# OpenVVC/OpenVVC

Hardware: AMD Instinct MI355X
Metric: decoded frames/sec, full rcn back-end decode step (H2D of the recorded picture + MC incl. BDOF/DMVR/affine-PROF/GPM/CIIP + LMCS + inverse transform + ordered intra pass + deblocking + SAO + ALF/CC-ALF + D2H of refined MVs + wait + per-picture digest + publication to the device DPB), 4K 10-bit RA rec (higher is better)
Workload: dtype u16 samples / int16 coefficients / int32 accumulate

## Files before the change

### include/ovvc_hip.h

```cpp
#ifndef OVVC_HIP_H
#define OVVC_HIP_H

#include <stddef.h>
#include <stdint.h>

#ifdef __cplusplus
extern "C" {
#endif

#define OVHIP_ABI_VERSION 9

#define OVHIP_OK        0
#define OVHIP_ENODEV   (-1)
#define OVHIP_ENOMEM   (-2)
#define OVHIP_EINVAL   (-3)
#define OVHIP_ELAUNCH  (-4)
#define OVHIP_EUNSUP   (-5)
#define OVHIP_EREF     (-6)

enum { OVHIP_DST_VII = 0, OVHIP_DCT_VIII = 1, OVHIP_DCT_II = 2 };

typedef struct ovhip_pic {
    uint16_t *y, *cb, *cr;
    int32_t   w, h;
// ... 814 lines not shown
int  ovhip_dpb_post_rows(ovhip_dpb *d, const void *key, int32_t rows, void *event, const volatile uint32_t *abort_word);
int  ovhip_dpb_rows_tag(ovhip_dpb *d, const void *key, uint64_t tag, int dev, int32_t need_rows, int block, int pin, ovhip_pic *pic, void **event);
int  ovhip_dpb_wait_copy(ovhip_dpb *d, int dev, void *event);
int  ovhip_dpb_unpin(ovhip_dpb *d, const void *key);
int  ovhip_dpb_release(ovhip_dpb *d, const void *key);
int  ovhip_dpb_lookup(ovhip_dpb *d, const void *key, int *home_dev, ovhip_pic *pic);
void ovhip_dpb_shutdown(ovhip_dpb *d);
int  ovhip_dpb_get_stats(ovhip_dpb *d, ovhip_dpb_stats *out);

typedef struct ovhip_frame ovhip_frame;

enum { OVHIP_OUT_NONE = 0,
       OVHIP_OUT_DIGEST = 1,
       OVHIP_OUT_PLANES = 2,
       OVHIP_OUT_PACKED = 3 };
typedef struct ovhip_frame_output {
    int32_t  mode;
    ovhip_window window;
    uint16_t *y, *cb, *cr; int32_t stride_y, stride_c;
    void    *packed;
    uint8_t  digest[16];
} ovhip_frame_output;

enum { OVHIP_FE_BEGIN = 1, OVHIP_FE_REF, OVHIP_FE_DMVR_ROWS, OVHIP_FE_DMVR_BEGIN, OVHIP_FE_DMVR_COLLECT, OVHIP_FE_SUBMIT, OVHIP_FE_FAIL,
       OVHIP_FE_BAND  };
typedef struct ovhip_frame_event {
    uint32_t op; int32_t frame;
    uint64_t key, tag;
    int64_t  a, b, result;
} ovhip_frame_event;
void ovhip_frame_set_trace(void (*sink)(void *user, const ovhip_frame_event *ev), void *user);

int  ovhip_frame_create(ovhip_dpb *dpb, int dev, int32_t w, int32_t h, ovhip_frame **out);
void ovhip_frame_destroy(ovhip_frame *f);
ovhip_ctx      *ovhip_frame_ctx(ovhip_frame *f);
ovhip_job      *ovhip_frame_job(ovhip_frame *f);
ovhip_recorder *ovhip_frame_recorder(ovhip_frame *f);
int  ovhip_frame_begin(ovhip_frame *f, const void *key);
int  ovhip_frame_ref(ovhip_frame *f, const void *ref_key);
int  ovhip_frame_begin_tag(ovhip_frame *f, const void *key, uint64_t tag);
int  ovhip_frame_ref_tag(ovhip_frame *f, const void *ref_key, uint64_t tag);
int  ovhip_frame_ref_at(ovhip_frame *f, int slot, const void *ref_key);
int64_t ovhip_frame_dmvr_rows(ovhip_frame *f);
int  ovhip_frame_refs_ready(ovhip_frame *f);
int64_t ovhip_frame_dmvr_rows_begin(ovhip_frame *f, int32_t log2_ctu_s);
int64_t ovhip_frame_dmvr_rows_begin_upto(ovhip_frame *f, int32_t log2_ctu_s, size_t upto_units);
int64_t ovhip_frame_dmvr_rows_collect(ovhip_frame *f);
int  ovhip_frame_submit(ovhip_frame *f, ovhip_job *job, const ovhip_pic *intra, const ovhip_job_params *params, ovhip_frame_output *out);
int  ovhip_frame_set_band_mode(ovhip_frame *f, int on);
int  ovhip_frame_band(ovhip_frame *f, const ovhip_job_params *params, int32_t row_end, int32_t last, ovhip_frame_output *out);
int  ovhip_frame_band_upto(ovhip_frame *f, const ovhip_job_params *params, int32_t row_end, const ovhip_band_counts *upto, int32_t block);
int  ovhip_frame_band_stats(const ovhip_frame *f, int32_t *n_bands, int32_t *n_deferred);
int  ovhip_frame_set_output_scale(ovhip_frame *f, int32_t out_w, int32_t out_h, const ovhip_scale_info *info);
int  ovhip_frame_set_film_grain(ovhip_frame *f, const ovhip_fg_params *params, int32_t poc);
int  ovhip_frame_set_picture_hash(ovhip_frame *f, int method, int n_planes, const ovhip_pic_hash_value *expected);
int  ovhip_frame_picture_hash(const ovhip_frame *f, ovhip_pic_hash_value *computed);
int  ovhip_frame_set_rgb_output(ovhip_frame *f, const ovhip_rgb_format *fmt, const ovhip_window *win, void *d_dst, size_t dst_bytes);
int  ovhip_frame_set_surface_output(ovhip_frame *f, const ovhip_surface_format *fmt, const ovhip_window *win, void *d_dst, size_t dst_bytes);
int  ovhip_frame_set_mvfield_output(ovhip_frame *f, const ovhip_mvfield_format *fmt, void *d_vec, size_t vec_bytes, void *d_info, size_t info_bytes);
int  ovhip_frame_fail(ovhip_frame *f, int status);
const char *ovhip_frame_last_error(const ovhip_frame *f);

typedef struct ovhip_calllog ovhip_calllog;
ovhip_calllog *ovhip_calllog_create(void);
void   ovhip_calllog_destroy(ovhip_calllog *log);
void   ovhip_calllog_reset(ovhip_calllog *log);
const void *ovhip_calllog_data(const ovhip_calllog *log, size_t *bytes);
void   ovhip_rec_set_calllog(ovhip_recorder *rec, ovhip_calllog *log);
int64_t ovhip_calllog_replay(const void *data, size_t bytes, ovhip_recorder *rec);

#define OVHIP_STREAM_MAX_REFS 8
typedef struct ovhip_stream_content {
    const void *calllog; size_t calllog_bytes;
    ovhip_job_params params;
    uint32_t n_ref_slots;
} ovhip_stream_content;

typedef struct ovhip_stream_pic {
    uint32_t content;
    uint32_t job;
    int32_t  poc;
    uint16_t device;
    uint16_t n_refs;
    uint32_t refs[OVHIP_STREAM_MAX_REFS];
    int32_t  owner;
    uint32_t send_mask;
} ovhip_stream_pic;

typedef struct ovhip_stream_xfer {
    void *user;
    int (*send)(void *user, uint32_t idx, const ovhip_pic *pic, int dst_rank);
    int (*recv)(void *user, uint32_t idx, const ovhip_pic *pic, int src_rank);
} ovhip_stream_xfer;

typedef struct ovhip_rccl ovhip_rccl;
int  ovhip_rccl_unique_id(uint8_t out[128]);
int  ovhip_rccl_create(ovhip_rccl **out, const uint8_t unique_id[128], int rank, int world, int hip_device);
void ovhip_rccl_destroy(ovhip_rccl *r);
const ovhip_stream_xfer *ovhip_rccl_xfer(ovhip_rccl *r);
const char *ovhip_rccl_last_error(const ovhip_rccl *r);
int  ovhip_rccl_stats(const ovhip_rccl *r, uint64_t out[4]);
int  ovhip_rccl_self_exchange(ovhip_rccl *r, const ovhip_pic *src, const ovhip_pic *dst);

enum { OVHIP_STREAM_RECORD = 1,
       OVHIP_STREAM_DIGESTS = 2,
       OVHIP_STREAM_RESIDENT = 4,
       OVHIP_STREAM_KEEP = 8,
       OVHIP_STREAM_HOLD_ALL = 32,
       OVHIP_STREAM_FILE_MD5 = 16 };

typedef struct ovhip_stream_cfg {
    int32_t w, h;
    uint32_t flags;
    int32_t threads_per_device;
    int32_t output;
    ovhip_window window;
    uint32_t extra_stages;
    int32_t rank;
    const ovhip_stream_xfer *xfer;
    int32_t intra_lookahead;
    int32_t ahead_own_queue;
} ovhip_stream_cfg;

typedef struct ovhip_stream_result {
    double   seconds;
    uint64_t n_decoded, n_second_passes, n_received, n_sent;
    uint64_t out_frames, out_bytes;
    uint8_t  out_md5[16];
    double   record_seconds;
    double   host_seconds[5];
    int32_t  status;
    char     error[192];
    double  *trace;
} ovhip_stream_result;

typedef struct ovhip_stream ovhip_stream;
int  ovhip_stream_create(ovhip_stream **out, ovhip_dpb *dpb, const ovhip_stream_cfg *cfg, const ovhip_stream_content *contents,
                         uint32_t n_contents, ovhip_job *const *jobs, uint32_t n_jobs);
void ovhip_stream_destroy(ovhip_stream *s);
int  ovhip_stream_run(ovhip_stream *s, const ovhip_stream_pic *pics, uint32_t n_total, uint32_t first, uint32_t n, uint32_t flags,
                      uint8_t *digests, ovhip_stream_result *res);
ovhip_frame *ovhip_stream_frame(ovhip_stream *s, int dev, int thread);
int  ovhip_stream_queue_info(const ovhip_stream *s, int *moved, int *sharing);
int  ovhip_stream_set_output_scale(ovhip_stream *s, int32_t out_w, int32_t out_h, const ovhip_scale_info *info);
int  ovhip_stream_set_film_grain(ovhip_stream *s, const ovhip_fg_params *params);
int  ovhip_stream_set_picture_hashes(ovhip_stream *s, int method, int n_planes, const ovhip_pic_hash_value *expected);
int  ovhip_stream_picture_hashes(const ovhip_stream *s, ovhip_pic_hash_value *computed, uint32_t *n_mismatch, int32_t *first_mismatch);
int  ovhip_stream_set_rgb_output(ovhip_stream *s, const ovhip_rgb_format *fmt, const ovhip_window *win, void *d_base, size_t bytes_per_picture, uint32_t n_slots);
int  ovhip_stream_set_surface_output(ovhip_stream *s, const ovhip_surface_format *fmt, const ovhip_window *win, void *d_base, size_t bytes_per_picture, uint32_t n_slots);
int  ovhip_stream_set_mvfield_output(ovhip_stream *s, const ovhip_mvfield_format *fmt, void *d_vec_base, size_t vec_bytes_per_picture,
                                     void *d_info_base, size_t info_bytes_per_picture, uint32_t n_slots);
const void *ovhip_stream_key(const ovhip_stream *s, uint32_t idx);
int  ovhip_job_test_abort_next_flow(ovhip_job *job);

#ifdef __cplusplus
}
#endif
#endif
```

### openvvc_amd/capi.py

```python
from __future__ import annotations

import ctypes as C
import os
from pathlib import Path

import numpy as np

_PKG = Path(__file__).resolve().parent
LIB_PATH = _PKG / os.environ.get("OVVC_HIP_LIB_NAME", "libovvc_hip.so")

OVHIP_ABI_VERSION = 9
OVHIP_OK, OVHIP_ENODEV, OVHIP_ENOMEM, OVHIP_EINVAL, OVHIP_ELAUNCH, OVHIP_EUNSUP, OVHIP_EREF = 0, -1, -2, -3, -4, -5, -6
DST_VII, DCT_VIII, DCT_II = 0, 1, 2
TB_TR, TB_DC, TB_TS, TB_TS_RAW = 0, 1, 2, 3
TB_FLAG_RASTER = 0x80
RES_ADD, RES_SUB, RES_ADD_HALF, RES_SUB_HALF, RES_SCALE = 0, 1, 2, 3, 4
MC_HPEL_FILT, MC_FILT_4x4, MC_NO_LUMA, MC_NO_CHROMA, MC_LMCS, MC_BDOF, MC_DMVR = 1, 2, 4, 8, 16, 32, 64
PU_BDOF, PU_DMVR, PU_GPM = 1, 2, 4
MC_GPM = 128


class Pic(C.Structure):
    _fields_ = [("y", C.c_void_p), ("cb", C.c_void_p), ("cr", C.c_void_p),
                ("w", C.c_int32), ("h", C.c_int32), ("stride_y", C.c_int32), ("stride_c", C.c_int32)]
# ... 489 lines not shown
    p = Path(path) if path else LIB_PATH
    if not p.exists():
        raise RuntimeError(f"{p} not built: run `python -c 'import __graft_entry__ as g; g.build()'` "
                           "(the HIP engine has no CPU fallback)")
    try:
        import torch
    except Exception:
        pass
    lib = C.CDLL(str(p))
    vp, u32, i32 = C.c_void_p, C.c_uint32, C.c_int32
    P = C.POINTER
    sigs = {
        "ovhip_abi_version": (C.c_int, []),
        "ovhip_rec_create": (vp, [i32, i32]),
        "ovhip_rec_destroy": (None, [vp]),
        "ovhip_rec_reset": (None, [vp]),
        "ovhip_rec_tu": (C.c_int, [vp, P(TuState), P(TuDesc)]),
        "ovhip_rec_pu": (C.c_int, [vp, P(PuDesc)]),
        "ovhip_rec_set_ref_scale": (C.c_int, [vp, i32, P(RefScale)]),
        "ovhip_rec_refusal": (C.c_char_p, [vp]),
        "ovhip_rec_rpr_units": (vp, [vp, P(C.c_size_t)]),
        "ovhip_mc_rpr_launch": (C.c_int, [vp, P(Pic), P(Pic), u32, vp, u32, vp, P(Pic)]),
        "ovhip_rec_set_rpr_tools": (C.c_int, [vp, u32]),
        "ovhip_rec_aff_rpr_units": (vp, [vp, P(C.c_size_t)]),
        "ovhip_mca_rpr_launch": (C.c_int, [vp, P(Pic), P(Pic), u32, vp, u32, vp, vp]),
        "ovhip_rec_dbf_ctu": (C.c_int, [vp, vp]),
        "ovhip_rec_dbf_row": (C.c_int, [vp, vp, C.c_size_t]),
        "ovhip_rec_dbf_mv_prepass_view": (C.c_int, [vp, vp, vp, vp]),
        "ovhip_rec_cu_inter": (C.c_int, [vp, vp, vp]),
        "ovhip_rec_dbf_planes": (C.c_int, [vp, P(DbfPlanes)]),
        "ovhip_dbf_launch": (C.c_int, [vp, P(Pic), P(DbfPlanes)]),
        "ovhip_sao_launch": (C.c_int, [vp, P(Pic), P(Pic), vp, i32]),
        "ovhip_alf_launch": (C.c_int, [vp, P(Pic), P(Pic), P(AlfPic)]),
        "ovhip_rec_tb_cmds": (vp, [vp, P(C.c_size_t)]),
        "ovhip_rec_coefs": (vp, [vp, P(C.c_size_t)]),
        "ovhip_rec_mc_units": (vp, [vp, P(C.c_size_t)]),
        "ovhip_rec_mcx_units": (vp, [vp, P(C.c_size_t)]),
        "ovhip_rec_affine_cu": (C.c_int, [vp, P(AffineDesc)]),
        "ovhip_rec_transform_tree": (C.c_int, [vp, P(TuState), P(TtDesc)]),
        "ovhip_rec_lmcs_region": (C.c_int, [vp, C.c_int32, C.c_int32, u32, u32]),
        "ovhip_dbf_compact": (C.c_int64, [P(DbfPlanes), C.c_int, vp, C.c_size_t]),
        "ovhip_rec_dbf_mv_prepass": (C.c_int, [vp, P(DbfMvCtx)]),
        "ovhip_dbf_launch_edges": (C.c_int, [vp, P(Pic), vp, u32, vp, u32, C.c_int32, C.c_int32]),
        "ovhip_rec_ciip": (C.c_int, [vp, C.c_int32, C.c_int32, C.c_int32, C.c_int32, C.c_int32, C.c_int32]),
        "ovhip_rec_ciip_units": (vp, [vp, P(C.c_size_t)]),
        "ovhip_ciip_launch": (C.c_int, [vp, P(Pic), P(Pic), vp, u32]),
        "ovhip_rec_lmcs_regions": (vp, [vp, P(C.c_size_t)]),
        "ovhip_rec_tb_cmds_split": (vp, [vp, C.c_size_t * 4, P(C.c_size_t)]),
        "ovhip_itx_launch_classes": (C.c_int, [vp, P(Pic), vp, u32, u32, vp, vp]),
        "ovhip_itx_launch_chroma_lmcs": (C.c_int, [vp, P(Pic), vp, u32, u32, vp, vp, vp]),
        "ovhip_lmcs_build": (C.c_int, [P(LmcsData), P(LmcsLuts)]),
        "ovhip_lmcs_scale_launch": (C.c_int, [vp, P(Pic), vp, u32, P(LmcsLuts), vp]),
        "ovhip_lmcs_inverse_launch": (C.c_int, [vp, P(Pic), vp]),
        "ovhip_rec_aff_units": (vp, [vp, P(C.c_size_t)]),
        "ovhip_rec_aff_side": (vp, [vp, P(C.c_size_t)]),
        "ovhip_ctx_create": (C.c_int, [P(vp), C.c_int, vp]),
        "ovhip_ctx_destroy": (None, [vp]),
        "ovhip_ctx_sync": (C.c_int, [vp]),
        "ovhip_ctx_shares_queue": (C.c_int, [vp, vp]),
        "ovhip_ctx_new_stream": (C.c_int, [vp]),
        "ovhip_ctx_fork": (C.c_int, [vp, C.c_int]),
        "ovhip_ctx_join": (C.c_int, [vp]),
        "ovhip_last_error": (C.c_char_p, [vp]),
        "ovhip_ctx_stream": (vp, [vp]),
        "ovhip_malloc": (C.c_int, [vp, C.c_size_t, P(vp)]),
        "ovhip_free": (C.c_int, [vp, vp]),
        "ovhip_h2d": (C.c_int, [vp, vp, vp, C.c_size_t]),
        "ovhip_d2h": (C.c_int, [vp, vp, vp, C.c_size_t]),
        "ovhip_pic_alloc": (C.c_int, [vp, i32, i32, P(Pic)]),
        "ovhip_pic_free": (C.c_int, [vp, P(Pic)]),
        "ovhip_pic_upload": (C.c_int, [vp, P(Pic), vp, vp, vp, i32, i32]),
        "ovhip_pic_download": (C.c_int, [vp, P(Pic), vp, vp, vp, i32, i32]),
        "ovhip_itx_launch": (C.c_int, [vp, P(Pic), vp, u32, vp, vp]),
        "ovhip_mc_launch": (C.c_int, [vp, P(Pic), P(Pic), u32, vp, u32, vp, P(Pic)]),
        "ovhip_ciip_weight": (C.c_int, [C.c_int32, C.c_int32]),
        "ovhip_mcx_launch": (C.c_int, [vp, P(Pic), P(Pic), u32, vp, u32, vp, vp]),
        "ovhip_mca_launch": (C.c_int, [vp, P(Pic), P(Pic), u32, vp, u32, vp, vp]),
        "ovhip_mcxa_launch": (C.c_int, [vp, P(Pic), P(Pic), u32, vp, u32, vp, vp, u32, vp, vp]),
        "ovhip_rec_create_ex": (vp, [i32, i32, vp]),
        "ovhip_rec_set_dense_dbf_planes": (None, [vp, C.c_int]),
        "ovhip_rec_dbf_edges": (vp, [vp, C.c_int, P(C.c_size_t), P(DbfOffsets)]),
        "ovhip_dbf_launch_edges_ex": (C.c_int, [vp, P(Pic), vp, u32, vp, u32, P(DbfOffsets)]),
        "ovhip_dmvr_search_launch": (C.c_int, [vp, P(Pic), P(Pic), u32, vp, u32, vp]),
        "ovhip_rec_append_raw": (C.c_int, [vp, C.c_int, vp, C.c_size_t]),
        "ovhip_itx_launch_classes_res": (C.c_int, [vp, P(Pic), P(Pic), vp, u32, u32, vp, vp]),
        "ovhip_intra_level_launch": (C.c_int, [vp, P(Pic), P(Pic), vp, u32, vp, vp, vp, i32, u32]),
        "ovhip_intra_level_geom": (u32, [vp, C.c_size_t]),
        "ovhip_intra_sync_words": (C.c_size_t, [i32, i32, i32]),
        "ovhip_intra_flow_words": (C.c_size_t, [i32, i32]),
        "ovhip_intra_flow_items": (C.c_size_t, [vp, C.c_size_t, vp, C.c_size_t]),
        "ovhip_intra_flow_launch": (C.c_int, [vp, P(Pic), P(Pic), vp, u32, vp, u32, vp, vp, vp, i32, vp, u32, vp, i32, i32]),
        "ovhip_intra_ctu_launch": (C.c_int, [vp, P(Pic), P(Pic), vp, vp, u32, vp, vp, vp, i32, vp, u32, vp]),
        "ovhip_rec_itask_levels": (u32, [vp]),
        "ovhip_rec_isp_cu": (C.c_int, [vp, vp, vp]),
        "ovhip_isp_geometry": (None, [i32, i32, i32, P(i32), P(i32), P(i32), P(i32)]),
        "ovhip_job_bind": (C.c_int, [vp, vp]),
        "ovhip_rec_set_ctu_size": (C.c_int, [vp, i32]),
        "ovhip_rec_itasks_by_ctu": (vp, [vp, i32, P(C.c_size_t), P(vp), P(C.c_size_t)]),
        "ovhip_rec_tu_intra": (C.c_int, [vp, P(TuState), P(TuDesc), P(ITask), P(ITask)]),
        "ovhip_rec_itasks": (vp, [vp, P(C.c_size_t)]),
        "ovhip_rec_ibc_check": (C.c_int, [vp, P(IbcDesc)]),
        "ovhip_rec_tu_ibc": (C.c_int, [vp, P(TuState), P(TuDesc), P(IbcDesc)]),
        "ovhip_rec_ibc_tasks": (C.c_size_t, [vp]),
        "ovhip_rec_itasks_sorted": (vp, [vp, P(C.c_size_t), P(P(C.c_uint32)), P(C.c_uint32)]),
        "ovhip_rec_set_dbf_offsets": (C.c_int, [vp, P(DbfOffsets), C.c_int]),
        "ovhip_job_create": (C.c_int, [vp, i32, i32, P(vp)]),
        "ovhip_job_destroy": (None, [vp]),
        "ovhip_job_recorder": (vp, [vp]),
        "ovhip_job_begin": (C.c_int, [vp]),
        "ovhip_job_flush": (C.c_int, [vp, P(Pic), P(Pic), u32, P(Pic), P(JobParams)]),
        "ovhip_frame_band": (C.c_int, [vp, P(JobParams), i32, i32, P(FrameOutput)]),
        "ovhip_frame_set_band_mode": (C.c_int, [vp, C.c_int]),
        "ovhip_frame_band_upto": (C.c_int, [vp, P(JobParams), i32, P(BandCounts), i32]),
        "ovhip_frame_dmvr_rows_begin_upto": (C.c_int64, [vp, i32, C.c_size_t]),
        "ovhip_job_dmvr_rows_begin_upto": (C.c_int64, [vp, P(Pic), u32, i32, C.c_size_t]),
        "ovhip_frame_band_stats": (C.c_int, [vp, P(i32), P(i32)]),
        "ovhip_dpb_post_rows": (C.c_int, [vp, vp, i32, vp, vp]),
        "ovhip_dpb_rows_tag": (C.c_int, [vp, vp, C.c_uint64, C.c_int, i32, C.c_int, C.c_int, P(Pic), P(vp)]),
        "ovhip_job_band": (C.c_int, [vp, P(Pic), P(Pic), u32, P(JobParams), P(BandCounts), i32, i32]),
        "ovhip_job_band_active": (C.c_int, [vp]),
        "ovhip_job_band_busy": (C.c_int, [vp]),
        "ovhip_job_band_progress": (C.c_int, [vp, P(i32), P(vp), P(vp)]),
        "ovhip_rec_counts": (None, [vp, P(BandCounts)]),
        "ovhip_sao_launch_rows": (C.c_int, [vp, P(Pic), P(Pic), vp, i32, i32, i32]),
        "ovhip_alf_launch_rows": (C.c_int, [vp, P(Pic), P(Pic), P(AlfPic), i32, i32]),
        "ovhip_job_wait": (C.c_int, [vp]),
        "ovhip_job_refined_mvs": (vp, [vp, P(C.c_size_t)]),
        "ovhip_job_dmvr_rows": (C.c_int64, [vp, P(Pic), u32]),
        "ovhip_job_dmvr_rows_begin": (C.c_int64, [vp, P(Pic), u32, i32]),
        "ovhip_job_dmvr_rows_collect": (C.c_int64, [vp]),
        "ovhip_job_last_stats": (C.c_int, [vp, P(JobStats)]),
        "ovhip_job_time_stage": (C.c_int, [vp, C.c_int]),
        "ovhip_job_stage_time": (C.c_int, [vp, P(C.c_double), P(C.c_uint64)]),
        "ovhip_lmcs_scale_prepare_launch": (C.c_int, [vp, P(Pic), vp, u32, vp, vp, vp, u32, vp, u32]),
        "ovhip_lmcs_inverse_untag_launch": (C.c_int, [vp, P(Pic), vp, vp, u32]),
        "ovhip_intra_flow_untag_launch": (C.c_int, [vp, P(Pic), vp, u32, i32]),
        "ovhip_tmvp_cells_launch": (C.c_int, [vp, vp, u32, vp, i32, i32, vp]),
        "ovhip_job_tmvp_cells": (vp, [vp, P(C.c_size_t)]),
        "ovhip_output_bytes": (C.c_size_t, [i32, i32, P(Window)]),
        "ovhip_output_rows": (C.c_size_t, [i32, i32, P(Window)]),
        "ovhip_output_pack_launch": (C.c_int, [vp, P(Pic), P(Window), vp]),
        "ovhip_output_row_md5_launch": (C.c_int, [vp, P(Pic), P(Window), vp]),
        "ovhip_output_bands": (C.c_size_t, [i32, i32, P(Window)]),
        "ovhip_output_tree_md5_launch": (C.c_int, [vp, P(Pic), P(Window), vp]),
        "ovhip_pic_output": (C.c_int, [vp, P(Pic), P(Window), vp]),
        "ovhip_pic_digest": (C.c_int, [vp, P(Pic), P(Window), vp]),
        "ovhip_md5_init": (None, [P(Md5State)]),
        "ovhip_md5_update": (None, [P(Md5State), vp, C.c_size_t]),
        "ovhip_md5_final": (None, [P(Md5State), vp]),
        "ovhip_d2d": (C.c_int, [vp, vp, vp, C.c_size_t]),
        "ovhip_host_alloc": (vp, [C.c_size_t]),
        "ovhip_host_free": (None, [vp]),
        "ovhip_job_test_abort_next_flow": (C.c_int, [vp]),
        "ovhip_dpb_create": (C.c_int, [P(vp), P(C.c_int), C.c_int]),
        "ovhip_dpb_create_ex": (C.c_int, [P(vp), C.c_int, P(DpbOps)]),
        "ovhip_dpb_destroy": (None, [vp]),
        "ovhip_dpb_n_devices": (C.c_int, [vp]),
        "ovhip_dpb_device": (C.c_int, [vp, C.c_int]),
        "ovhip_dpb_begin": (C.c_int, [vp, vp, C.c_int, i32, i32, P(Pic)]),
        "ovhip_dpb_want": (C.c_int, [vp, vp, C.c_int]),
        "ovhip_dpb_begin_tag": (C.c_int, [vp, vp, C.c_uint64, C.c_int, i32, i32, P(Pic)]),
        "ovhip_dpb_want_tag": (C.c_int, [vp, vp, C.c_uint64, C.c_int]),
        "ovhip_dpb_acquire_tag": (C.c_int, [vp, vp, C.c_uint64, C.c_int, P(Pic), P(vp)]),
        "ovhip_dpb_publish": (C.c_int, [vp, vp, C.c_int]),
        "ovhip_dpb_acquire": (C.c_int, [vp, vp, C.c_int, P(Pic), P(vp)]),
        "ovhip_dpb_wait_copy": (C.c_int, [vp, C.c_int, vp]),
        "ovhip_dpb_poll_tag": (C.c_int, [vp, vp, C.c_uint64]),
        "ovhip_frame_refs_ready": (C.c_int, [vp]),
        "ovhip_dpb_set_unknown_key_timeout": (None, [vp, C.c_int]),
        "ovhip_dpb_unpin": (C.c_int, [vp, vp]),
        "ovhip_dpb_release": (C.c_int, [vp, vp]),
        "ovhip_dpb_lookup": (C.c_int, [vp, vp, P(C.c_int), P(Pic)]),
        "ovhip_dpb_shutdown": (None, [vp]),
        "ovhip_dpb_get_stats": (C.c_int, [vp, P(DpbStats)]),
        "ovhip_frame_create": (C.c_int, [vp, C.c_int, i32, i32, P(vp)]),
        "ovhip_frame_destroy": (None, [vp]),
        "ovhip_frame_ctx": (vp, [vp]),
        "ovhip_frame_job": (vp, [vp]),
        "ovhip_frame_recorder": (vp, [vp]),
        "ovhip_frame_begin": (C.c_int, [vp, vp]),
        "ovhip_frame_ref": (C.c_int, [vp, vp]),
        "ovhip_frame_set_trace": (None, [vp, vp]),
        "ovhip_rccl_unique_id": (C.c_int, [vp]),
        "ovhip_rccl_create": (C.c_int, [P(vp), vp, C.c_int, C.c_int, C.c_int]),
        "ovhip_rccl_destroy": (None, [vp]),
        "ovhip_rccl_xfer": (vp, [vp]),
        "ovhip_rccl_last_error": (C.c_char_p, [vp]),
        "ovhip_rccl_stats": (C.c_int, [vp, P(C.c_uint64)]),
        "ovhip_rccl_self_exchange": (C.c_int, [vp, P(Pic), P(Pic)]),
        "ovhip_frame_begin_tag": (C.c_int, [vp, vp, C.c_uint64]),
        "ovhip_frame_ref_tag": (C.c_int, [vp, vp, C.c_uint64]),
        "ovhip_frame_ref_at": (C.c_int, [vp, C.c_int, vp]),
        "ovhip_frame_dmvr_rows": (C.c_int64, [vp]),
        "ovhip_frame_dmvr_rows_begin": (C.c_int64, [vp, i32]),
        "ovhip_frame_dmvr_rows_collect": (C.c_int64, [vp]),
        "ovhip_frame_submit": (C.c_int, [vp, vp, P(Pic), P(JobParams), P(FrameOutput)]),
        "ovhip_frame_fail": (C.c_int, [vp, C.c_int]),
        "ovhip_frame_last_error": (C.c_char_p, [vp]),
        "ovhip_calllog_create": (vp, []),
        "ovhip_calllog_destroy": (None, [vp]),
        "ovhip_calllog_reset": (None, [vp]),
        "ovhip_calllog_data": (vp, [vp, P(C.c_size_t)]),
        "ovhip_rec_set_calllog": (None, [vp, vp]),
        "ovhip_calllog_replay": (C.c_int64, [vp, C.c_size_t, vp]),
        "ovhip_stream_create": (C.c_int, [P(vp), vp, P(StreamCfg), P(StreamContent), u32, P(vp), u32]),
        "ovhip_stream_destroy": (None, [vp]),
        "ovhip_stream_run": (C.c_int, [vp, P(StreamPic), u32, u32, u32, u32, vp, P(StreamResult)]),
        "ovhip_stream_frame": (vp, [vp, C.c_int, C.c_int]),
        "ovhip_stream_queue_info": (C.c_int, [vp, P(C.c_int), P(C.c_int)]),
        "ovhip_stream_key": (vp, [vp, u32]),
        "ovhip_output_scale_check": (C.c_int, [i32, i32, P(ScaleInfo), i32, i32, P(i32 * 4)]),
        "ovhip_output_scale_launch": (C.c_int, [vp, P(Pic), P(ScaleInfo), P(Pic)]),
        "ovhip_pic_output_scaled": (C.c_int, [vp, P(Pic), P(ScaleInfo), i32, i32, P(Window), vp]),
        "ovhip_pic_digest_scaled": (C.c_int, [vp, P(Pic), P(ScaleInfo), i32, i32, P(Window), vp]),
        "ovhip_ctx_scratch_bytes": (C.c_size_t, [vp]),
        "ovhip_frame_set_output_scale": (C.c_int, [vp, i32, i32, P(ScaleInfo)]),
        "ovhip_stream_set_output_scale": (C.c_int, [vp, i32, i32, P(ScaleInfo)]),
        "ovhip_frame_set_film_grain": (C.c_int, [vp, P(FgParams), i32]),
        "ovhip_stream_set_film_grain": (C.c_int, [vp, P(FgParams)]),
        "ovhip_fg_derive": (C.c_int, [P(FgParams), P(FgModel), P(FgParams)]),
        "ovhip_fg_database": (vp, []),
        "ovhip_fg_seed": (u32, [i32, i32, C.c_int]),
        "ovhip_fg_prng": (u32, [u32]),
        "ovhip_fg_stripe_seeds": (None, [u32, i32, i32, P(u32)]),
        "ovhip_film_grain_launch": (C.c_int, [vp, P(Pic), P(FgModel), i32, i32, P(Pic)]),
        "ovhip_pic_output_grain": (C.c_int, [vp, P(Pic), P(FgModel), i32, P(Window), vp]),
        "ovhip_pic_digest_grain": (C.c_int, [vp, P(Pic), P(FgModel), i32, P(Window), vp]),
        "ovhip_pic_hash_host": (C.c_int, [C.c_int, C.c_int, vp, vp, vp, i32, i32, i32, i32, P(PicHashValue)]),
        "ovhip_pic_hash_parse_sei": (C.c_int, [vp, C.c_size_t, P(PicHashValue)]),
        "ovhip_pic_hash_equal": (C.c_int, [P(PicHashValue), P(PicHashValue)]),
        "ovhip_pic_hash_launch": (C.c_int, [vp, P(Pic), C.c_int, C.c_int, vp]),
        "ovhip_pic_hash": (C.c_int, [vp, P(Pic), C.c_int, C.c_int, P(PicHashValue)]),
        "ovhip_frame_set_picture_hash": (C.c_int, [vp, C.c_int, C.c_int, P(PicHashValue)]),
        "ovhip_frame_picture_hash": (C.c_int, [vp, P(PicHashValue)]),
        "ovhip_stream_set_picture_hashes": (C.c_int, [vp, C.c_int, C.c_int, P(PicHashValue)]),
        "ovhip_stream_picture_hashes": (C.c_int, [vp, P(PicHashValue), P(u32), P(i32)]),
        "ovhip_rgb_bytes": (C.c_size_t, [i32, i32, P(Window), P(RgbFormat)]),
        "ovhip_rgb_coefs": (C.c_int, [P(RgbFormat), P(i32), P(i32)]),
        "ovhip_rgb_host": (C.c_int, [vp, vp, vp, i32, i32, i32, i32, P(Window), P(RgbFormat), vp, C.c_size_t]),
        "ovhip_rgb_launch": (C.c_int, [vp, P(Pic), P(Window), P(RgbFormat), vp, C.c_size_t]),
        "ovhip_pic_output_rgb": (C.c_int, [vp, P(Pic), P(Window), P(RgbFormat), vp, C.c_size_t]),
        "ovhip_frame_set_rgb_output": (C.c_int, [vp, P(RgbFormat), P(Window), vp, C.c_size_t]),
        "ovhip_stream_set_rgb_output": (C.c_int, [vp, P(RgbFormat), P(Window), vp, C.c_size_t, u32]),
        "ovhip_surface_bytes": (C.c_size_t, [i32, i32, P(Window), P(SurfaceFormat)]),
        "ovhip_surface_host": (C.c_int, [vp, vp, vp, i32, i32, i32, i32, P(Window), P(SurfaceFormat), vp, C.c_size_t]),
        "ovhip_surface_launch": (C.c_int, [vp, P(Pic), P(Window), P(SurfaceFormat), vp, C.c_size_t]),
        "ovhip_pic_output_surface": (C.c_int, [vp, P(Pic), P(Window), P(SurfaceFormat), vp, C.c_size_t]),
        "ovhip_frame_set_surface_output": (C.c_int, [vp, P(SurfaceFormat), P(Window), vp, C.c_size_t]),
        "ovhip_stream_set_surface_output": (C.c_int, [vp, P(SurfaceFormat), P(Window), vp, C.c_size_t, u32]),
        "ovhip_mvfield_bytes": (C.c_size_t, [i32, i32, P(MvfieldFormat), P(C.c_size_t)]),
        "ovhip_mvfield_host": (C.c_int, [i32, i32, P(MvfieldSrc), P(MvfieldFormat), vp, C.c_size_t, vp, C.c_size_t]),
        "ovhip_mvfield_launch": (C.c_int, [vp, i32, i32, P(MvfieldSrc), P(MvfieldFormat), vp, C.c_size_t, vp, C.c_size_t]),
        "ovhip_job_mvfield": (C.c_int, [vp, P(MvfieldFormat), vp, C.c_size_t, vp, C.c_size_t]),
        "ovhip_frame_set_mvfield_output": (C.c_int, [vp, P(MvfieldFormat), vp, C.c_size_t, vp, C.c_size_t]),
        "ovhip_stream_set_mvfield_output": (C.c_int, [vp, P(MvfieldFormat), vp, C.c_size_t, vp, C.c_size_t, u32]),
    }
    ab_build = "OVVC_HIP_LIB_NAME" in os.environ
    for name, (res, args) in sigs.items():
        if ab_build and not hasattr(lib, name):
            continue
        fn = getattr(lib, name)
        fn.restype, fn.argtypes = res, args
    if lib.ovhip_abi_version() != OVHIP_ABI_VERSION and not ab_build:
        raise RuntimeError("libovvc_hip.so ABI version mismatch")
    if path is None:
        _lib = lib
    return lib


EXPORTED_SYMBOLS = [
    "ovhip_abi_version", "ovhip_rec_create", "ovhip_rec_destroy", "ovhip_rec_reset", "ovhip_rec_tu",
    "ovhip_rec_pu", "ovhip_rec_cu_inter", "ovhip_rec_dbf_row", "ovhip_rec_dbf_mv_prepass_view", "ovhip_rec_dbf_ctu", "ovhip_rec_dbf_planes", "ovhip_dbf_launch", "ovhip_sao_launch", "ovhip_alf_launch", "ovhip_rec_tb_cmds", "ovhip_rec_coefs", "ovhip_rec_mc_units", "ovhip_rec_mcx_units", "ovhip_mcx_launch", "ovhip_rec_affine_cu", "ovhip_rec_transform_tree", "ovhip_rec_lmcs_region", "ovhip_dbf_compact", "ovhip_rec_dbf_mv_prepass", "ovhip_dbf_launch_edges", "ovhip_rec_ciip", "ovhip_ciip_weight", "ovhip_rec_ciip_units", "ovhip_ciip_launch", "ovhip_rec_lmcs_regions", "ovhip_rec_tb_cmds_split", "ovhip_itx_launch_classes", "ovhip_itx_launch_chroma_lmcs", "ovhip_lmcs_build", "ovhip_lmcs_scale_launch", "ovhip_lmcs_inverse_launch", "ovhip_rec_aff_units", "ovhip_rec_aff_side", "ovhip_mca_launch", "ovhip_mcxa_launch", "ovhip_ctx_create",
    "ovhip_ctx_destroy", "ovhip_ctx_sync", "ovhip_ctx_shares_queue", "ovhip_ctx_new_stream", "ovhip_ctx_fork", "ovhip_ctx_join", "ovhip_last_error", "ovhip_ctx_stream", "ovhip_malloc",
    "ovhip_free", "ovhip_h2d", "ovhip_d2h", "ovhip_pic_alloc", "ovhip_pic_free", "ovhip_pic_upload",
    "ovhip_pic_download", "ovhip_itx_launch", "ovhip_mc_launch",
    "ovhip_rec_set_ref_scale", "ovhip_rec_refusal", "ovhip_rec_rpr_units", "ovhip_mc_rpr_launch",
    "ovhip_rec_set_rpr_tools", "ovhip_rec_aff_rpr_units", "ovhip_mca_rpr_launch",
    "ovhip_rec_create_ex", "ovhip_rec_set_dense_dbf_planes", "ovhip_rec_dbf_edges", "ovhip_dbf_launch_edges_ex",
    "ovhip_dmvr_search_launch", "ovhip_rec_append_raw", "ovhip_rec_set_dbf_offsets", "ovhip_rec_tu_intra", "ovhip_rec_itasks", "ovhip_rec_itasks_sorted", "ovhip_itx_launch_classes_res", "ovhip_intra_level_launch", "ovhip_intra_level_geom", "ovhip_intra_sync_words", "ovhip_intra_ctu_launch", "ovhip_intra_flow_words", "ovhip_intra_flow_items", "ovhip_intra_flow_launch",
    "ovhip_rec_itask_levels", "ovhip_rec_isp_cu", "ovhip_isp_geometry", "ovhip_rec_itasks_by_ctu", "ovhip_rec_set_ctu_size", "ovhip_job_bind", "ovhip_job_create", "ovhip_job_destroy", "ovhip_job_recorder", "ovhip_job_begin",
    "ovhip_frame_band", "ovhip_frame_band_upto", "ovhip_frame_dmvr_rows_begin_upto", "ovhip_job_dmvr_rows_begin_upto", "ovhip_frame_set_band_mode", "ovhip_frame_band_stats", "ovhip_dpb_post_rows", "ovhip_dpb_rows_tag",
    "ovhip_job_band", "ovhip_job_band_active", "ovhip_job_band_busy", "ovhip_job_band_reserve", "ovhip_job_reserve_for_picture", "ovhip_rec_reserve_for_picture", "ovhip_job_band_progress", "ovhip_rec_counts", "ovhip_sao_launch_rows", "ovhip_alf_launch_rows",
    "ovhip_job_flush", "ovhip_job_wait", "ovhip_job_refined_mvs", "ovhip_job_dmvr_rows", "ovhip_job_dmvr_rows_begin", "ovhip_job_dmvr_rows_collect", "ovhip_job_last_stats", "ovhip_job_time_stage", "ovhip_job_stage_time",
    "ovhip_output_bytes", "ovhip_output_rows", "ovhip_output_pack_launch", "ovhip_output_row_md5_launch", "ovhip_output_bands", "ovhip_output_tree_md5_launch", "ovhip_pic_output", "ovhip_pic_digest",
    "ovhip_md5_init", "ovhip_md5_update", "ovhip_md5_final", "ovhip_tmvp_cells_launch", "ovhip_job_tmvp_cells", "ovhip_intra_flow_untag_launch", "ovhip_lmcs_inverse_untag_launch", "ovhip_lmcs_scale_prepare_launch",
    "ovhip_host_alloc", "ovhip_host_free", "ovhip_d2d", "ovhip_job_test_abort_next_flow",
    "ovhip_dpb_create", "ovhip_dpb_create_ex", "ovhip_dpb_destroy", "ovhip_dpb_n_devices", "ovhip_dpb_device", "ovhip_dpb_begin", "ovhip_dpb_want",
    "ovhip_dpb_publish", "ovhip_dpb_acquire", "ovhip_dpb_wait_copy", "ovhip_dpb_poll_tag", "ovhip_frame_refs_ready", "ovhip_dpb_set_unknown_key_timeout", "ovhip_dpb_unpin", "ovhip_dpb_release", "ovhip_dpb_lookup", "ovhip_dpb_shutdown",
    "ovhip_dpb_get_stats", "ovhip_dpb_begin_tag", "ovhip_dpb_want_tag", "ovhip_dpb_acquire_tag", "ovhip_frame_begin_tag", "ovhip_frame_ref_tag", "ovhip_frame_set_trace",
    "ovhip_rccl_unique_id", "ovhip_rccl_create", "ovhip_rccl_destroy", "ovhip_rccl_xfer", "ovhip_rccl_last_error", "ovhip_rccl_stats", "ovhip_rccl_self_exchange",
    "ovhip_frame_create", "ovhip_frame_destroy", "ovhip_frame_ctx", "ovhip_frame_job", "ovhip_frame_recorder", "ovhip_frame_begin", "ovhip_frame_ref",
    "ovhip_frame_ref_at", "ovhip_frame_dmvr_rows", "ovhip_frame_dmvr_rows_begin", "ovhip_frame_dmvr_rows_collect", "ovhip_frame_submit", "ovhip_frame_fail", "ovhip_frame_last_error",
    "ovhip_calllog_create", "ovhip_calllog_destroy", "ovhip_calllog_reset", "ovhip_calllog_data", "ovhip_rec_set_calllog", "ovhip_calllog_replay",
    "ovhip_stream_create", "ovhip_stream_destroy", "ovhip_stream_run", "ovhip_stream_frame", "ovhip_stream_key", "ovhip_stream_queue_info",
    "ovhip_output_scale_check", "ovhip_output_scale_launch", "ovhip_pic_output_scaled", "ovhip_pic_digest_scaled",
    "ovhip_frame_set_output_scale", "ovhip_stream_set_output_scale", "ovhip_ctx_scratch_bytes",
    "ovhip_rec_ibc_check", "ovhip_rec_tu_ibc", "ovhip_rec_ibc_tasks",
    "ovhip_frame_set_film_grain", "ovhip_stream_set_film_grain", "ovhip_fg_derive", "ovhip_fg_database", "ovhip_fg_seed", "ovhip_fg_prng", "ovhip_fg_stripe_seeds", "ovhip_film_grain_launch", "ovhip_pic_output_grain", "ovhip_pic_digest_grain",
    "ovhip_pic_hash_host", "ovhip_pic_hash_parse_sei", "ovhip_pic_hash_equal", "ovhip_pic_hash_launch", "ovhip_pic_hash",
    "ovhip_frame_set_picture_hash", "ovhip_frame_picture_hash", "ovhip_stream_set_picture_hashes", "ovhip_stream_picture_hashes",
    "ovhip_rgb_bytes", "ovhip_rgb_coefs", "ovhip_rgb_host", "ovhip_rgb_launch", "ovhip_pic_output_rgb", "ovhip_frame_set_rgb_output", "ovhip_stream_set_rgb_output",
    "ovhip_surface_bytes", "ovhip_surface_host", "ovhip_surface_launch", "ovhip_pic_output_surface", "ovhip_frame_set_surface_output", "ovhip_stream_set_surface_output",
    "ovhip_mvfield_bytes", "ovhip_mvfield_host", "ovhip_mvfield_launch", "ovhip_job_mvfield", "ovhip_frame_set_mvfield_output", "ovhip_stream_set_mvfield_output",
]


def rpr_units(lib, rec) -> list:
    n = C.c_size_t(0)
    ptr = lib.ovhip_rec_rpr_units(rec, C.byref(n))
    if not ptr or not n.value:
        return []
    raw = C.string_at(ptr, n.value * C.sizeof(RprUnit))
    return [RprUnit.from_buffer_copy(raw, i * C.sizeof(RprUnit)) for i in range(n.value)]


def aff_rpr_units(lib, rec) -> list:
    n = C.c_size_t(0)
    ptr = lib.ovhip_rec_aff_rpr_units(rec, C.byref(n))
    if not ptr or not n.value:
        return []
    raw = C.string_at(ptr, n.value * C.sizeof(AffRprUnit))
    return [AffRprUnit.from_buffer_copy(raw, i * C.sizeof(AffRprUnit)) for i in range(n.value)]


def set_ref_scale(lib, rec, slot: int, scale_hor: int | None = None, scale_ver: int | None = None, ref_w: int = 0, ref_h: int = 0,
                  col_hor: int = 0, col_ver: int = 0) -> int:
    if scale_hor is None:
        return lib.ovhip_rec_set_ref_scale(rec, slot, None)
    sc = RefScale(scale_hor, scale_ver if scale_ver is not None else scale_hor, ref_w, ref_h, col_hor, col_ver)
    return lib.ovhip_rec_set_ref_scale(rec, slot, C.byref(sc))


class Recorder:

    def __init__(self, pic_w: int, pic_h: int):
        self.lib = load()
        self.h = self.lib.ovhip_rec_create(pic_w, pic_h)
        if not self.h:
            raise MemoryError("ovhip_rec_create")
        self._keep = []

    def close(self):
        if self.h:
            self.lib.ovhip_rec_destroy(self.h)
            self.h = None

    def __del__(self):
        try:
            self.close()
        except Exception:
            pass

    def reset(self):
        self.lib.ovhip_rec_reset(self.h)

    def start_calllog(self):
        self._log = self.lib.ovhip_calllog_create()
        self.lib.ovhip_rec_set_calllog(self.h, self._log)

    def take_calllog(self) -> np.ndarray:
        n = C.c_size_t()
        p = self.lib.ovhip_calllog_data(self._log, C.byref(n))
        if not p and n.value:
            raise MemoryError("call log")
        out = np.frombuffer((C.c_char * n.value).from_address(p), dtype=np.uint8).copy() if n.value else np.zeros(0, np.uint8)
        self.lib.ovhip_rec_set_calllog(self.h, None)
        self.lib.ovhip_calllog_destroy(self._log)
        self._log = None
        return out

    def replay(self, log: np.ndarray) -> int:
        n = self.lib.ovhip_calllog_replay(log.ctypes.data, log.nbytes, self.h)
        if n < 0:
            raise ValueError(f"ovhip_calllog_replay -> {n}")
        return int(n)

    def tu(self, st: TuState, d: TuDesc) -> int:
        r = self.lib.ovhip_rec_tu(self.h, C.byref(st), C.byref(d))
        if r < 0:
            raise ValueError(f"ovhip_rec_tu -> {r}")
        return r

    def tu_intra(self, st: TuState, d: TuDesc, task_l: "ITask | None", task_c: "ITask | None") -> int:
        r = self.lib.ovhip_rec_tu_intra(self.h, C.byref(st), C.byref(d), C.byref(task_l) if task_l is not None else None,
                                        C.byref(task_c) if task_c is not None else None)
        if r < 0:
            raise ValueError(f"ovhip_rec_tu_intra -> {r}")
        return r

    def ibc_check(self, cu: IbcDesc) -> int:
        return self.lib.ovhip_rec_ibc_check(self.h, C.byref(cu))

    def tu_ibc(self, st: TuState, d: TuDesc, cu: IbcDesc) -> int:
        return self.lib.ovhip_rec_tu_ibc(self.h, C.byref(st), C.byref(d), C.byref(cu))

    def ibc_tasks(self) -> int:
        return int(self.lib.ovhip_rec_ibc_tasks(self.h))

    def refusal(self) -> str:
        return (self.lib.ovhip_rec_refusal(self.h) or b"").decode()

    def itasks(self) -> np.ndarray:
        return self._arr(self.lib.ovhip_rec_itasks, ITASK_DTYPE)

    def itasks_sorted(self):
        n, nl, ls = C.c_size_t(), C.c_uint32(), C.POINTER(C.c_uint32)()
        p = self.lib.ovhip_rec_itasks_sorted(self.h, C.byref(n), C.byref(ls), C.byref(nl))
        if not n.value:
            return np.zeros(0, ITASK_DTYPE), np.zeros(1, np.uint32)
        t = np.frombuffer((C.c_char * (n.value * 32)).from_address(p), dtype=ITASK_DTYPE).copy()
        return t, np.array([ls[i] for i in range(nl.value + 1)], np.uint32)

    def itasks_by_ctu(self, log2_ctu: int = 7):
        n, nc, cp = C.c_size_t(), C.c_size_t(), C.c_void_p()
        p = self.lib.ovhip_rec_itasks_by_ctu(self.h, log2_ctu, C.byref(n), C.byref(cp), C.byref(nc))
        if not n.value:
            return np.zeros(0, ITASK_DTYPE), np.zeros(0, ICTU_DTYPE)
        t = np.frombuffer((C.c_char * (n.value * 32)).from_address(p), dtype=ITASK_DTYPE).copy()
        c = np.frombuffer((C.c_char * (nc.value * 16)).from_address(cp.value), dtype=ICTU_DTYPE).copy()
        return t, c

    def transform_tree(self, st: "TuState", d: TtDesc, infos: bytes, res_cb: np.ndarray, res_cr: np.ndarray, res_y: np.ndarray) -> int:
        ib = (C.c_char * len(infos)).from_buffer_copy(infos)
        keep = [np.ascontiguousarray(a, dtype=np.int16) for a in (res_cb, res_cr, res_y)]
        d.tu_info = C.addressof(ib)
        for k in range(3):
            d.residual[k] = keep[k].ctypes.data
        r = self.lib.ovhip_rec_transform_tree(self.h, C.byref(st), C.byref(d))
        d.tu_info = None
        if r < 0:
            raise ValueError(f"ovhip_rec_transform_tree -> {r}")
        return r

    def isp_cu(self, st: TuState, d: IspDesc) -> int:
        r = self.lib.ovhip_rec_isp_cu(self.h, C.byref(st), C.byref(d))
        if r < 0:
            raise ValueError(f"ovhip_rec_isp_cu -> {r}")
        return r

# ... 126 lines not shown
```

### openvvc_amd/csrc/kernels_itx.hip

```cpp
#include "ovvc_common.hip.h"
#include <stdlib.h>
#define OVT_ATTR __device__
#include "vvc_tables.h"

#ifndef OV_WPE_ITX
#define OV_WPE_ITX 8
#endif
#if OV_WPE_ITX > 0
#define OV_OCC_ITX __attribute__((amdgpu_waves_per_eu(OV_WPE_ITX)))
#else
#define OV_OCC_ITX
#endif

namespace {

constexpr int core_ks(int log2n)   { const int n = 1 << log2n, K = n < 32 ? n : 32; return K < 8 ? 8 : K; }
constexpr int core_size(int log2n) { return (1 << log2n) * core_ks(log2n); }
constexpr int core_off(int type, int log2n)
{
    int off = 0;
    for (int t = 0; t < 3; ++t)
        for (int l = (t == 2 ? 1 : 2); l <= (t == 2 ? 6 : 5); ++l) {
            if (t == type && l == log2n) return off;
            off += core_size(l);
        }
    return off;
}
constexpr int CORE_TOTAL = core_off(3, 0);
struct CoreT16 { int16_t v[CORE_TOTAL]; };
constexpr CoreT16 build_cores()
{
    CoreT16 t{};
    const int8_t *const tabs[3][7] = {
        { nullptr, nullptr, ovt_dst7_4, ovt_dst7_8, ovt_dst7_16, ovt_dst7_32, nullptr },
        { nullptr, nullptr, ovt_dct8_4, ovt_dct8_8, ovt_dct8_16, ovt_dct8_32, nullptr },
        { nullptr, ovt_dct2_2, ovt_dct2_4, ovt_dct2_8, ovt_dct2_16, ovt_dct2_32, ovt_dct2_64 } };
    for (int ty = 0; ty < 3; ++ty)
        for (int l = 1; l <= 6; ++l) {
            if (!tabs[ty][l]) continue;
            const int n = 1 << l, K = n < 32 ? n : 32, KS = core_ks(l), off = core_off(ty, l);
            for (int j = 0; j < n; ++j)
                for (int k = 0; k < K; ++k) t.v[off + j * KS + k] = tabs[ty][l][k * n + j];
        }
    return t;
}
__device__ const CoreT16 __attribute__((aligned(16))) g_cores = build_cores();

constexpr uint64_t core_lut(int type)
{
    uint64_t v = 0;
    for (int l = (type == 2 ? 1 : 2); l <= (type == 2 ? 6 : 5); ++l)
        v |= (uint64_t)((core_off(type, l) - core_off(type, type == 2 ? 1 : 2)) / 16) << (8 * l);
    return v;
}
static_assert(core_lut(0) == core_lut(1) && (core_off(2, 6) - core_off(2, 1)) / 16 < 256 && core_off(1, 2) % 16 == 0 && core_off(2, 1) % 16 == 0,
              "core offsets must fit the byte table");
__device__ __forceinline__ const int16_t *tr_core(int type, int log2n)
{
    const uint64_t lut = type == 2 ? core_lut(2) : core_lut(0);
    const int base = type == 2 ? core_off(2, 1) : type == 1 ? core_off(1, 2) : 0;
    return g_cores.v + base + 16 * (int)((lut >> (8 * log2n)) & 0xff);
}
__device__ __forceinline__ int tile_stride(int K) { return K < 8 ? 8 : K + (K >= 16 ? 4 : 0); }
constexpr int tile_stride_c(int K) { return K < 8 ? 8 : K + (K >= 16 ? 4 : 0); }

__device__ __forceinline__ int dequant1(int c, int scale, int shift, int neg)
{
    if (neg) return ov_clip3((int)((uint32_t)c * (uint32_t)(scale << shift)), -32767, 32767);
    return ov_clip3(((int)((uint32_t)c * (uint32_t)scale) + ((1 << shift) >> 1)) >> shift, -32767, 32767);
}

__device__ __forceinline__ int nb_rows_of(uint64_t map)
{
    uint32_t m = (uint32_t)map | (uint32_t)(map >> 32);
    m |= m >> 16; m |= m >> 8;
    m = (m & 0xff) | 1;
    return (32 - __clz((int)m)) << 2;
}
__device__ __forceinline__ int nb_cols_of(uint64_t map)
{
    return (8 - (__clzll((long long)(map | 1)) >> 3)) << 2;
}

__device__ __forceinline__ int residual1(int pix, int r, int mode, int scale)
{
    const int neg = -(mode & 1);
    int v = ((r ^ neg) - neg) >> ((mode >> 1) & 1);
    if (mode & OVHIP_RES_STORE) return ov_clip16(v) & 0xffff;
    if (mode & OVHIP_RES_SCALE) {
        int sign = v & (1 << 15);
        int a = ov_clip_bd(abs(v));
        a = (a * scale + (1 << 10)) >> 11;
        v = ov_clip3(sign ? -a : a, -(1 << 15), 1 << 15);
    }
    return ov_clip_bd(pix + v);
}

struct ResDelta { long long d[3]; };

struct ResidualSink {
    uint16_t *dst; int stride; int mode;
    uint16_t *dst2; int stride2; int mode2;
    int scale;
};
typedef short short2v __attribute__((ext_vector_type(2)));

template <bool FINAL, int NT, int NK4>
__device__ __forceinline__ void tr_pass_lds_n(const int16_t *src, int sstride, const int16_t *core, int cstride, int log2n,
                                               int kmax, int lines, int shift, int16_t *dst, int dstride, int lane,
                                               const ResidualSink &sink)
{
    const int n = 1 << log2n;
    const int ntask = lines << log2n;
    const int rnd = 1 << (shift - 1);
    const int nk4 = (kmax + 3) >> 2;
    for (int t = lane; t < ntask; t += NT) {
        const int j = t & (n - 1), i = t >> log2n;
        int old = 0, old2 = 0;
        if (FINAL) {
            old = sink.dst[i * sink.stride + j];
            if (sink.dst2) old2 = sink.dst2[i * sink.stride2 + j];
        }
        const int2 *sp = reinterpret_cast<const int2 *>(src + i * sstride);
        const int2 *cp = reinterpret_cast<const int2 *>(core + j * cstride);
        int acc = 0;
        if (NK4 > 0) {
            int2 a[NK4 > 0 ? NK4 : 1], m[NK4 > 0 ? NK4 : 1];
#pragma unroll
            for (int k4 = 0; k4 < NK4; ++k4) { a[k4] = sp[k4]; m[k4] = cp[k4]; }
#pragma unroll
            for (int k4 = 0; k4 < NK4; ++k4) {
                acc = __builtin_amdgcn_sdot2(__builtin_bit_cast(short2v, a[k4].x), __builtin_bit_cast(short2v, m[k4].x), acc, false);
                acc = __builtin_amdgcn_sdot2(__builtin_bit_cast(short2v, a[k4].y), __builtin_bit_cast(short2v, m[k4].y), acc, false);
            }
        } else
        for (int k4 = 0; k4 < nk4; ++k4) {
            const int2 a = sp[k4], m = cp[k4];
            acc = __builtin_amdgcn_sdot2(__builtin_bit_cast(short2v, a.x), __builtin_bit_cast(short2v, m.x), acc, false);
            acc = __builtin_amdgcn_sdot2(__builtin_bit_cast(short2v, a.y), __builtin_bit_cast(short2v, m.y), acc, false);
        }
        const int r = ov_clip16((acc + rnd) >> shift);
        if (!FINAL) {
            dst[j * dstride + i] = (int16_t)r;
        } else {
            sink.dst[i * sink.stride + j] = (uint16_t)residual1(old, r, sink.mode, sink.scale);
            if (sink.dst2) sink.dst2[i * sink.stride2 + j] = (uint16_t)residual1(old2, r, sink.mode2, sink.scale);
        }
    }
}

template <bool FINAL, int NT>
__device__ __forceinline__ void tr_pass_lds(const int16_t *src, int sstride, const int16_t *core, int cstride, int log2n,
                                             int kmax, int lines, int shift, int16_t *dst, int dstride, int lane,
                                             const ResidualSink &sink)
{
    const int nk4 = (kmax + 3) >> 2;
    if (nk4 == 1)      tr_pass_lds_n<FINAL, NT, 1>(src, sstride, core, cstride, log2n, kmax, lines, shift, dst, dstride, lane, sink);
    else if (nk4 == 2) tr_pass_lds_n<FINAL, NT, 2>(src, sstride, core, cstride, log2n, kmax, lines, shift, dst, dstride, lane, sink);
    else if (nk4 == 4) tr_pass_lds_n<FINAL, NT, 4>(src, sstride, core, cstride, log2n, kmax, lines, shift, dst, dstride, lane, sink);
    else               tr_pass_lds_n<FINAL, NT, 0>(src, sstride, core, cstride, log2n, kmax, lines, shift, dst, dstride, lane, sink);
}

template <int NT>
__device__ __forceinline__ void lmcs_inverse_rows(const ovhip_pic &pic, const uint16_t *__restrict__ lut, uint32_t e, uint32_t n_extra,
                                                  uint16_t *s_lut)
{
    for (int i = threadIdx.x; i < 512; i += NT) reinterpret_cast<uint32_t *>(s_lut)[i] = reinterpret_cast<const uint32_t *>(lut)[i];
    __syncthreads();
    const int nvx = pic.w >> 3, tail = pic.w & 7;
    for (int y = (int)e; y < pic.h; y += (int)n_extra) {
        uint16_t *row = pic.y + (size_t)y * pic.stride_y;
        for (int v = threadIdx.x; v < nvx; v += NT) {
            uint4 q = *reinterpret_cast<uint4 *>(row + 8 * v);
            uint32_t *d = reinterpret_cast<uint32_t *>(&q);
#pragma unroll
            for (int k = 0; k < 4; ++k) d[k] = s_lut[d[k] & 1023] | ((uint32_t)s_lut[(d[k] >> 16) & 1023] << 16);
            *reinterpret_cast<uint4 *>(row + 8 * v) = q;
        }
        if ((int)threadIdx.x < tail) row[8 * nvx + threadIdx.x] = s_lut[row[8 * nvx + threadIdx.x] & 1023];
    }
}

#define ITX_LDS_BIG   8064
#define ITX_LDS_SLICE 2048

__device__ __forceinline__ ResidualSink make_sink(const ovhip_pic &pic, const ResDelta &rd, const ovhip_tb_cmd &c, const int16_t *__restrict__ lmcs_scales)
{
    ResidualSink sink;
    sink.dst = ov_plane(pic, c.plane, sink.stride) + c.y * sink.stride + c.x;
    sink.mode = c.res_mode;
    sink.dst2 = nullptr; sink.stride2 = 0; sink.mode2 = c.res_mode2;
    if (c.plane2 != 0xff) sink.dst2 = ov_plane(pic, c.plane2, sink.stride2) + c.y * sink.stride2 + c.x;
    if (c.res_mode & OVHIP_RES_STORE) {
        const long long d1 = c.plane == 0 ? rd.d[0] : (c.plane == 1 ? rd.d[1] : rd.d[2]);
        sink.dst = reinterpret_cast<uint16_t *>(reinterpret_cast<char *>(sink.dst) + d1);
        if (sink.dst2) {
            const long long d2 = c.plane2 == 0 ? rd.d[0] : (c.plane2 == 1 ? rd.d[1] : rd.d[2]);
            sink.dst2 = reinterpret_cast<uint16_t *>(reinterpret_cast<char *>(sink.dst2) + d2);
        }
    }
    sink.scale = (c.res_mode & OVHIP_RES_SCALE_IDX) ? lmcs_scales[c.c_scale] : c.c_scale;
    return sink;
}

template <int NT>
__device__ __forceinline__ void block_sync()
{
    if (NT == 64) {
        __builtin_amdgcn_fence(__ATOMIC_RELEASE, "wavefront");
        __builtin_amdgcn_wave_barrier();
        __builtin_amdgcn_fence(__ATOMIC_ACQUIRE, "wavefront");
    } else __syncthreads();
}

template <int NT, int LW = -1, int LH = -1, bool PLAIN = false>
__device__ __forceinline__ void itx_block(const ovhip_pic &pic, const ResDelta &rd, const ovhip_tb_cmd &c, bool valid, const int16_t *__restrict__ arena,
                                          const int16_t *__restrict__ lmcs_scales, int ablate, int lane, int16_t *lds)
{
    const int log2_w = LW >= 0 ? LW : c.log2_w, log2_h = LH >= 0 ? LH : c.log2_h;
    const int tb_w = 1 << log2_w, tb_h = 1 << log2_h;
    const int kind = PLAIN ? (int)OVHIP_TB_TR : (c.kind & 0x3f);
    const bool raster = PLAIN ? false : (bool)(c.kind & OVHIP_TB_FLAG_RASTER), bdpcm = PLAIN ? false : (bool)(c.kind & OVHIP_TB_FLAG_BDPCM);
    if (PLAIN) ablate = 0;
    const int cw = min(tb_w, 32), ch = min(tb_h, 32);
    const int16_t *src = arena + c.coef_off;

    if (NT == 64 && kind == OVHIP_TB_DC && !ablate) {
        if (!valid) return;
        const bool have = raster || (c.sig_sb_map & 1);
        const int lvl = have ? (int)src[0] : 0;
        const int c0 = (!have || bdpcm) ? lvl : dequant1(lvl, c.dq_scale, c.dq_shift, c.dq_neg);
        const int flat_val = ov_clip16(((((int)(int16_t)c0 + 1) >> 1) + (1 << (14 - OV_BD - 1))) >> (14 - OV_BD));
        const ResidualSink sink = make_sink(pic, rd, c, lmcs_scales);
        for (int i0 = lane; i0 < tb_w * tb_h; i0 += 4 * NT) {
            int old[4], old2[4];
#pragma unroll
            for (int q = 0; q < 4; ++q) {
                const int i = i0 + NT * q;
                if (i < tb_w * tb_h) {
                    const int x = i & (tb_w - 1), y = i >> log2_w;
                    old[q] = sink.dst[y * sink.stride + x];
                    old2[q] = sink.dst2 ? (int)sink.dst2[y * sink.stride2 + x] : 0;
                }
            }
#pragma unroll
            for (int q = 0; q < 4; ++q) {
                const int i = i0 + NT * q;
                if (i < tb_w * tb_h) {
                    const int x = i & (tb_w - 1), y = i >> log2_w;
                    sink.dst[y * sink.stride + x] = (uint16_t)residual1(old[q], flat_val, sink.mode, sink.scale);
                    if (sink.dst2) sink.dst2[y * sink.stride2 + x] = (uint16_t)residual1(old2[q], flat_val, sink.mode2, sink.scale);
                }
            }
        }
        return;
    }

    const int l2nx = max(min(log2_w, 5) - 2, 0), nx = 1 << l2nx, ny = ch >> 2;
    const int sx = lane & (nx - 1), sy = lane >> l2nx, bit = sy * 8 + sx;
    const bool descan = !raster && !(ablate & 2) && cw >= 4 && lane < nx * ny;
    const bool sig = descan && ((c.sig_sb_map >> bit) & 1);
    int4 v0 = make_int4(0, 0, 0, 0), v1 = v0;
    if (valid && sig) {
        const int rank = __popcll(c.sig_sb_map & ((1ull << bit) - 1));
        const int4 *p = reinterpret_cast<const int4 *>(src + rank * 16);
        v0 = p[0]; v1 = p[1];
    }
    const int kv = min(tb_h, 32), kh = min(tb_w, 32);
    const bool one_d = kind == OVHIP_TB_TR && (log2_w == 0 || log2_h == 0);
    const bool is_tr = kind == OVHIP_TB_TR && !one_d;
    const int cs = tile_stride(ch);
    const int msv = tile_stride(kv), msh = tile_stride(kh);
    const int n_coef = (max(cw * cs, is_tr ? 0 : tb_w * tb_h) + 7) & ~7, n_tmp = (tb_h * msh + 7) & ~7, n_mv = (tb_h * msv + 7) & ~7;
    int16_t *const s_coef = lds, *const s_tmp = lds + n_coef, *const s_mv = s_tmp + n_tmp, *const s_mh = s_mv + n_mv;
    if (valid && is_tr && !(ablate & 1)) {
        const int l2cv = kv >= 32 ? 2 : kv >= 16 ? 1 : 0, l2ch = kh >= 32 ? 2 : kh >= 16 ? 1 : 0;
        const int nv = tb_h << l2cv, nh = tb_w << l2ch;
        const uint4 *mv4 = reinterpret_cast<const uint4 *>(tr_core(c.tr_v, log2_h));
        const uint4 *mh4 = reinterpret_cast<const uint4 *>(tr_core(c.tr_h, log2_w));
        for (int i = lane; i < max(nv, nh); i += NT) {
            uint4 a = make_uint4(0, 0, 0, 0), b = a;
            if (i < nv) a = mv4[i];
            if (i < nh) b = mh4[i];
            if (i < nv) {
                uint2 *d = reinterpret_cast<uint2 *>(s_mv + (i >> l2cv) * msv + ((i & ((1 << l2cv) - 1)) << 3));
                d[0] = make_uint2(a.x, a.y); d[1] = make_uint2(a.z, a.w);
            }
            if (i < nh) {
                uint2 *d = reinterpret_cast<uint2 *>(s_mh + (i >> l2ch) * msh + ((i & ((1 << l2ch) - 1)) << 3));
                d[0] = make_uint2(b.x, b.y); d[1] = make_uint2(b.z, b.w);
            }
        }
    }

    if (!valid || (ablate & 2)) {
    } else if (raster) {
        if (is_tr) {
            for (int i = lane; i < tb_w * tb_h; i += NT) {
                const int x = i & (tb_w - 1), y = i >> log2_w;
                if (y < ch && x < cw) s_coef[x * cs + y] = (int16_t)dequant1(src[i], c.dq_scale, c.dq_shift, c.dq_neg);
                if (tb_h < 4 && y == 0 && x < cw) { s_coef[x * cs + 2] = 0; s_coef[x * cs + 3] = 0; }
            }
        } else {
            for (int i = lane; i < tb_w * tb_h; i += NT)
                s_coef[i] = (kind == OVHIP_TB_TS_RAW || bdpcm) ? src[i] : (int16_t)dequant1(src[i], c.dq_scale, c.dq_shift, c.dq_neg);
        }
    } else if (descan) {
        const int w[8] = { v0.x, v0.y, v0.z, v0.w, v1.x, v1.y, v1.z, v1.w };
        int o[4][4];
#pragma unroll
        for (int r = 0; r < 4; ++r)
#pragma unroll
            for (int q = 0; q < 4; ++q) {
                const int word = w[r * 2 + (q >> 1)];
                const int cv = (q & 1) ? (word >> 16) : (int)(int16_t)(word & 0xffff);
                o[r][q] = (bdpcm || !sig) ? cv : dequant1(cv, c.dq_scale, c.dq_shift, c.dq_neg);
            }
#pragma unroll
        for (int a = 0; a < 4; ++a) {
            uint2 pk;
            if (is_tr) {
                pk.x = (uint32_t)(o[0][a] & 0xffff) | ((uint32_t)o[1][a] << 16);
                pk.y = (uint32_t)(o[2][a] & 0xffff) | ((uint32_t)o[3][a] << 16);
                *reinterpret_cast<uint2 *>(s_coef + (sx * 4 + a) * cs + sy * 4) = pk;
            } else {
                pk.x = (uint32_t)(o[a][0] & 0xffff) | ((uint32_t)o[a][1] << 16);
                pk.y = (uint32_t)(o[a][2] & 0xffff) | ((uint32_t)o[a][3] << 16);
                *reinterpret_cast<uint2 *>(s_coef + (sy * 4 + a) * cw + sx * 4) = pk;
            }
        }
    }
    block_sync<NT>();

    const ResidualSink sink = make_sink(pic, rd, c, lmcs_scales);

    if (ablate & 4) valid = false;
    const bool tr = valid && is_tr, lf = !PLAIN && tr && (c.lfnst & 1), bd = valid && !is_tr && bdpcm;
    int nb_row = 0, nb_col = 0;
    if (tr) {
        if (raster) {
            const int l2sw = log2_w > 2 ? 3 : 1;
            nb_col = kv;
            nb_row = (nb_rows_of(c.sig_sb_map) >> 2) << l2sw;
        } else {
            nb_row = nb_rows_of(c.sig_sb_map);
            nb_col = nb_cols_of(c.sig_sb_map);
        }
    }
    const bool is8 = log2_w >= 3 && log2_h >= 3;
    const int nout = is8 ? 48 : 16;
    int out = 0;
    if (lf) {
        const int set = (c.lfnst >> 1) & 3, idx = (c.lfnst >> 3) & 1;
        const int8_t *m = is8 ? ovt_lfnst_8x8[set][idx] : ovt_lfnst_4x4[set][idx];
        const int nin = is8 ? 16 : (min(log2_w, 5) == min(log2_h, 5) ? 8 : 16);
        if (lane < nout) {
            const uint64_t scan = 0xfbe7ad369c258140ull;
            int s = 0;
            for (int j = 0; j < nin; ++j) {
                const int pos = (int)((scan >> (4 * j)) & 0xf);
                s += (int)s_coef[(pos & 3) * cs + (pos >> 2)] * (int)m[lane + j * nout];
            }
            out = ov_clip3((s + 64) >> 7, -(1 << 15), 1 << 15);
        }
    } else if (bd) {
        if (c.tr_h == 0) {
            if (lane < tb_h) {
                int acc = s_coef[lane * tb_w];
                for (int x = 1; x < tb_w; ++x) { acc = ov_clip3(acc + s_coef[lane * tb_w + x], -(1 << 15), (1 << 15) - 1); s_coef[lane * tb_w + x] = (int16_t)acc; }
            }
        } else if (lane < tb_w) {
            int acc = s_coef[lane];
            for (int y = 1; y < tb_h; ++y) { acc = ov_clip3(acc + s_coef[y * tb_w + lane], -(1 << 15), (1 << 15) - 1); s_coef[y * tb_w + lane] = (int16_t)acc; }
        }
    }
    if (!PLAIN) block_sync<NT>();
    if (lf) {
        const int tr_flag = (c.lfnst >> 4) & 1;
        if (lane < nout) {
            int r, q;
            if (!is8)           { r = lane >> 2; q = lane & 3; }
            else if (lane < 32) { r = lane >> 3; q = lane & 7; }
            else                { r = 4 + ((lane - 32) >> 2); q = lane & 3; }
            if (tr_flag) { int t = r; r = q; q = t; }
            s_coef[q * cs + r] = (int16_t)out;
        }
        nb_row = 4 << (int)is8;
        nb_col = max(nb_col, nb_row);
    } else if (bd && kind == OVHIP_TB_TS) {
        for (int i = lane; i < tb_w * tb_h; i += NT) s_coef[i] = (int16_t)dequant1(s_coef[i], c.dq_scale, c.dq_shift, c.dq_neg);
    }
    if (!PLAIN) block_sync<NT>();
    const int ts = tile_stride(kh);
    if (tr) {
        nb_row = min(nb_row, tb_w);
        const int k1 = min(nb_col, kv);
        if ((nb_row & 3) && lane < tb_h)
            for (int e = nb_row; e < ((nb_row + 3) & ~3); ++e) s_tmp[lane * ts + e] = 0;
        tr_pass_lds<false, NT>(s_coef, cs, s_mv, msv, log2_h, k1, nb_row, 7, s_tmp, ts, lane, sink);
    }
    if (valid && one_d) {
        const int l2n = log2_w == 0 ? log2_h : log2_w, n = 1 << l2n, kmax = min(n, 32), ks = core_ks(l2n);
        const int16_t *core = tr_core(log2_w == 0 ? c.tr_v : c.tr_h, l2n);
        if (lane < n) {
            int acc = 0;
            for (int k = 0; k < kmax; ++k) acc += (int)s_coef[k] * (int)core[lane * ks + k];
            s_tmp[lane] = (int16_t)ov_clip16((acc + (1 << (20 - OV_BD))) >> (20 - OV_BD + 1));
        }
    }
    block_sync<NT>();
    if (tr) {
        const int k2 = min(nb_row, kh);
        tr_pass_lds<true, NT>(s_tmp, ts, s_mh, msh, log2_w, k2, tb_h, 20 - OV_BD, nullptr, 0, lane, sink);
        return;
    }
    if (!valid) return;

    const bool flat = kind == OVHIP_TB_DC;
    const int flat_val = ov_clip16(((((int)s_coef[0] + 1) >> 1) + (1 << (14 - OV_BD - 1))) >> (14 - OV_BD));
    for (int i0 = lane; i0 < tb_w * tb_h; i0 += 4 * NT) {
        int old[4], old2[4];
#pragma unroll
        for (int q = 0; q < 4; ++q) {
            const int i = i0 + NT * q;
            if (i < tb_w * tb_h) {
                const int x = i & (tb_w - 1), y = i >> log2_w;
                old[q] = sink.dst[y * sink.stride + x];
                old2[q] = sink.dst2 ? (int)sink.dst2[y * sink.stride2 + x] : 0;
            }
        }
#pragma unroll
        for (int q = 0; q < 4; ++q) {
            const int i = i0 + NT * q;
            if (i < tb_w * tb_h) {
                const int x = i & (tb_w - 1), y = i >> log2_w;
                const int r = flat ? flat_val : one_d ? (int)s_tmp[i] : (int)s_coef[y * tb_w + x];
                sink.dst[y * sink.stride + x] = (uint16_t)residual1(old[q], r, sink.mode, sink.scale);
                if (sink.dst2) sink.dst2[y * sink.stride2 + x] = (uint16_t)residual1(old2[q], r, sink.mode2, sink.scale);
            }
        }
    }
}

template <int K>
__device__ __forceinline__ int itx_dot(const int16_t *a, const int16_t *b, int kmax)
{
    int acc = 0;
    if (K == 4) {
        const uint2 x = *reinterpret_cast<const uint2 *>(a), y = *reinterpret_cast<const uint2 *>(b);
        acc = __builtin_amdgcn_sdot2(__builtin_bit_cast(short2v, x.x), __builtin_bit_cast(short2v, y.x), acc, false);
        acc = __builtin_amdgcn_sdot2(__builtin_bit_cast(short2v, x.y), __builtin_bit_cast(short2v, y.y), acc, false);
    } else {
#pragma unroll
        for (int k = 0; k < K; k += 8) {
            if (k < kmax) {
                const uint4 x = *reinterpret_cast<const uint4 *>(a + k), y = *reinterpret_cast<const uint4 *>(b + k);
                acc = __builtin_amdgcn_sdot2(__builtin_bit_cast(short2v, x.x), __builtin_bit_cast(short2v, y.x), acc, false);
                acc = __builtin_amdgcn_sdot2(__builtin_bit_cast(short2v, x.y), __builtin_bit_cast(short2v, y.y), acc, false);
                acc = __builtin_amdgcn_sdot2(__builtin_bit_cast(short2v, x.z), __builtin_bit_cast(short2v, y.z), acc, false);
                acc = __builtin_amdgcn_sdot2(__builtin_bit_cast(short2v, x.w), __builtin_bit_cast(short2v, y.w), acc, false);
            }
        }
    }
    return acc;
}

template <int LW, int LH>
__device__ __forceinline__ void itx_tiny(const ovhip_pic &pic, const ResDelta &rd, const ovhip_tb_cmd *__restrict__ cmds, uint32_t i, bool valid,
                                         const int16_t *__restrict__ arena, const int16_t *__restrict__ lmcs_scales, int16_t *s , int l)
{
    constexpr int W = 1 << LW, H = 1 << LH, N = W * H;
    static_assert(N <= 64 && W <= 8 && H <= 8, "a block is at most one wave: its fences are the wave's (tried with 16-point shapes behind workgroup barriers: slower)");
    const ovhip_tb_cmd c = cmds[valid ? i : 0];
    const int r = l >> LW, q = l & (W - 1);
    const int bit = (r >> 2) * 8 + (q >> 2);
    const bool sig = (c.sig_sb_map >> bit) & 1;
    const int rank = __popcll(c.sig_sb_map & ((1ull << bit) - 1));
    const int16_t *src = arena + c.coef_off + rank * 16 + (r & 3) * 4 + (q & 3);
    const int co = sig ? dequant1((int)src[0], c.dq_scale, c.dq_shift, c.dq_neg) : 0;
    s[q * H + r] = (int16_t)co;
    block_sync<64>();
    int acc = itx_dot<H>(s + q * H, tr_core(c.tr_v, LH) + r * 8, H);
    s[N + r * W + q] = (int16_t)ov_clip16((acc + 64) >> 7);
    block_sync<64>();
    acc = itx_dot<W>(s + N + r * W, tr_core(c.tr_h, LW) + q * 8, W);
    int res = ov_clip16((acc + (1 << (20 - OV_BD - 1))) >> (20 - OV_BD));
    if (c.kind == OVHIP_TB_DC) {
        res = ov_clip16(((((int)s[0] + 1) >> 1) + (1 << (14 - OV_BD - 1))) >> (14 - OV_BD));
    }
    if (!valid) return;
    const ResidualSink sink = make_sink(pic, rd, c, lmcs_scales);
    const int old = sink.dst[r * sink.stride + q];
    const int old2 = sink.dst2 ? (int)sink.dst2[r * sink.stride2 + q] : 0;
    sink.dst[r * sink.stride + q] = (uint16_t)residual1(old, res, sink.mode, sink.scale);
    if (sink.dst2) sink.dst2[r * sink.stride2 + q] = (uint16_t)residual1(old2, res, sink.mode2, sink.scale);
}

struct TinyCounts { uint32_t n[4]; };

__global__ __launch_bounds__(256) OV_OCC_ITX void k_itx_all(ovhip_pic pic, const ovhip_tb_cmd *__restrict__ cmds, uint32_t n_large,
                                                  uint32_t n_small, const int16_t *__restrict__ arena,
                                                  const int16_t *__restrict__ lmcs_scales, int ablate,
                                                  const uint16_t *__restrict__ lmcs_inv_lut, uint32_t n_extra, ResDelta rd, TinyCounts tc)
{
    __shared__ __attribute__((aligned(16))) int16_t lds[ITX_LDS_BIG > 4 * ITX_LDS_SLICE ? ITX_LDS_BIG : 4 * ITX_LDS_SLICE];
    const uint32_t n_tiny = tc.n[0] + tc.n[1] + tc.n[2] + tc.n[3];
    const uint32_t gq = (tc.n[0] + 3) >> 2, g0 = (tc.n[1] + 7) >> 3, g1 = (tc.n[2] + 7) >> 3, g2 = (tc.n[3] + 15) >> 4, n_tg = gq + g0 + g1 + g2;
    const uint32_t n_wave = n_small - n_tiny;
    const uint32_t b = blockIdx.x, n_quads = (n_wave + 3) >> 2;
    if (b < n_large) {
        itx_block<256>(pic, rd, cmds[ov_xcd_slot(b, n_large)], true, arena, lmcs_scales, ablate, threadIdx.x, lds);
    } else if (b < n_large + n_quads) {
        const int w = __builtin_amdgcn_readfirstlane(threadIdx.x >> 6);
        const uint32_t i = ov_xcd_slot(b - n_large, n_quads) * 4 + w;
        const bool valid = i < n_wave;
        const ovhip_tb_cmd &c = cmds[n_large + (valid ? i : 0)];
        int16_t *const slice = lds + w * ITX_LDS_SLICE;
        const int lane = threadIdx.x & 63;
        const bool plain = valid && !ablate && (c.kind & 0x3f) == OVHIP_TB_TR && !(c.kind & (OVHIP_TB_FLAG_RASTER | OVHIP_TB_FLAG_BDPCM)) && !(c.lfnst & 1);
        const int shape = plain ? (c.log2_w << 3 | c.log2_h) : -1;
#define ITX_SHAPE(lw, lh) case (lw) << 3 | (lh): itx_block<64, lw, lh, true>(pic, rd, c, true, arena, lmcs_scales, 0, lane, slice); break;
        switch (shape) {
        ITX_SHAPE(2, 2) ITX_SHAPE(3, 2) ITX_SHAPE(2, 3) ITX_SHAPE(3, 3) ITX_SHAPE(4, 2) ITX_SHAPE(2, 4) ITX_SHAPE(4, 3) ITX_SHAPE(3, 4)
        ITX_SHAPE(4, 4) ITX_SHAPE(5, 2) ITX_SHAPE(2, 5) ITX_SHAPE(5, 3) ITX_SHAPE(3, 5)
        default: itx_block<64>(pic, rd, c, valid, arena, lmcs_scales, ablate, lane, slice);
        }
#undef ITX_SHAPE
    } else if (b < n_large + n_quads + n_tg) {
        uint32_t g = b - n_large - n_quads;
        const ovhip_tb_cmd *base = cmds + n_large + n_wave;
        if (g < gq) {
            const uint32_t blk = threadIdx.x >> 6, i = ov_xcd_slot(g, gq) * 4 + blk;
            itx_tiny<3, 3>(pic, rd, base, i, i < tc.n[0], arena, lmcs_scales, lds + 128 * blk, (int)(threadIdx.x & 63));
        } else if ((g -= gq) < g0) {
            const uint32_t blk = threadIdx.x >> 5, i = ov_xcd_slot(g, g0) * 8 + blk;
            itx_tiny<2, 3>(pic, rd, base + tc.n[0], i, i < tc.n[1], arena, lmcs_scales, lds + 64 * blk, (int)(threadIdx.x & 31));
        } else if ((g -= g0) < g1) {
            const uint32_t blk = threadIdx.x >> 5, i = ov_xcd_slot(g, g1) * 8 + blk;
            itx_tiny<3, 2>(pic, rd, base + tc.n[0] + tc.n[1], i, i < tc.n[2], arena, lmcs_scales, lds + 64 * blk, (int)(threadIdx.x & 31));
        } else {
            g -= g1;
            const uint32_t blk = threadIdx.x >> 4, i = ov_xcd_slot(g, g2) * 16 + blk;
            itx_tiny<2, 2>(pic, rd, base + tc.n[0] + tc.n[1] + tc.n[2], i, i < tc.n[3], arena, lmcs_scales, lds + 32 * blk, (int)(threadIdx.x & 15));
        }
    } else {
        lmcs_inverse_rows<256>(pic, lmcs_inv_lut, b - n_large - n_quads - n_tg, n_extra, reinterpret_cast<uint16_t *>(lds));
    }
}

}

static int itx_ablate()
{
    static int cfg_ablate = -1;
#ifdef OVHIP_TUNING
    if (cfg_ablate < 0) { const char *a = getenv("OVHIP_ITX_ABLATE"); cfg_ablate = a ? atoi(a) : 0; }
#else
    cfg_ablate = 0;
#endif
    return cfg_ablate;
}

static int itx_launch(ovhip_ctx *ctx, const ovhip_pic *dst, const ovhip_tb_cmd *d_cmds, uint32_t n_large, uint32_t n_small,
                      const int16_t *d_coefs, const int16_t *d_lmcs_scales, const uint16_t *d_bwd_lut, const ovhip_pic *res = nullptr,
                      const uint32_t *tiny3 = nullptr)
{
    TinyCounts tc = { { tiny3 ? tiny3[0] : 0u, tiny3 ? tiny3[1] : 0u, tiny3 ? tiny3[2] : 0u, tiny3 ? tiny3[3] : 0u } };
    if ((uint64_t)tc.n[0] + tc.n[1] + tc.n[2] + tc.n[3] > n_small) return ov_fail(ctx, OVHIP_EINVAL, "itx launch: more tiny blocks than small ones", hipSuccess);
    ResDelta rd = { { 0, 0, 0 } };
    if (res) {
        if (res->w != dst->w || res->h != dst->h || res->stride_y != dst->stride_y || res->stride_c != dst->stride_c)
            return ov_fail(ctx, OVHIP_EINVAL, "itx launch: the residual picture must have the picture's geometry", hipSuccess);
        rd.d[0] = (char *)res->y - (char *)dst->y; rd.d[1] = (char *)res->cb - (char *)dst->cb; rd.d[2] = (char *)res->cr - (char *)dst->cr;
    }
    const uint32_t n_extra = d_bwd_lut ? (uint32_t)(dst->h + 3) / 4 : 0;
    if (itx_ablate()) tc.n[0] = tc.n[1] = tc.n[2] = tc.n[3] = 0;
    const uint32_t n_tiny = tc.n[0] + tc.n[1] + tc.n[2] + tc.n[3];
    const uint32_t grid = n_large + (n_small - n_tiny + 3) / 4 + (tc.n[0] + 3) / 4 + (tc.n[1] + 7) / 8 + (tc.n[2] + 7) / 8 + (tc.n[3] + 15) / 16 + n_extra;
    if (!grid) return OVHIP_OK;
    hipLaunchKernelGGL(k_itx_all, dim3(grid), dim3(256), 0, ctx->stream, *dst, d_cmds, n_large, n_small, d_coefs,
                       d_lmcs_scales, itx_ablate(), d_bwd_lut, n_extra, rd, tc);
    OV_LAUNCH_CHECK(ctx, "k_itx_all");
    return OVHIP_OK;
}

extern "C" int ovhip_itx_launch_classes(ovhip_ctx *ctx, const ovhip_pic *dst, const ovhip_tb_cmd *d_cmds,
                                        uint32_t n_large, uint32_t n_small, const int16_t *d_coefs,
                                        const int16_t *d_lmcs_scales)
{
    if (!ctx || !dst) return OVHIP_EINVAL;
    OV_DEVICE(ctx);
    if (!n_large && !n_small) return OVHIP_OK;
    if (!d_cmds || !d_coefs) return ov_fail(ctx, OVHIP_EINVAL, "ovhip_itx_launch: null buffer", hipSuccess);
    return itx_launch(ctx, dst, d_cmds, n_large, n_small, d_coefs, d_lmcs_scales, nullptr);
}

extern "C" int ovhip_itx_launch_classes_res(ovhip_ctx *ctx, const ovhip_pic *dst, const ovhip_pic *res, const ovhip_tb_cmd *d_cmds,
                                            uint32_t n_large, uint32_t n_small, const int16_t *d_coefs,
                                            const int16_t *d_lmcs_scales)
{
    if (!ctx || !dst || !res) return OVHIP_EINVAL;
    OV_DEVICE(ctx);
    if ((n_large + n_small) && (!d_cmds || !d_coefs))
        return ov_fail(ctx, OVHIP_EINVAL, "ovhip_itx_launch_classes_res: null commands / coefficients", hipSuccess);
    return itx_launch(ctx, dst, d_cmds, n_large, n_small, d_coefs, d_lmcs_scales, nullptr, res);
}

extern "C" int ovhip_itx_launch_chroma_lmcs(ovhip_ctx *ctx, const ovhip_pic *dst, const ovhip_tb_cmd *d_cmds,
                                            uint32_t n_large, uint32_t n_small, const int16_t *d_coefs,
                                            const int16_t *d_lmcs_scales, const uint16_t *d_bwd_lut)
{
    if (!ctx || !dst || !d_bwd_lut) return OVHIP_EINVAL;
    OV_DEVICE(ctx);
    if ((n_large || n_small) && (!d_cmds || !d_coefs)) return ov_fail(ctx, OVHIP_EINVAL, "ovhip_itx_launch_chroma_lmcs: null buffer", hipSuccess);
    if ((dst->stride_y & 7) || ((uintptr_t)dst->y & 15))
        return ov_fail(ctx, OVHIP_EINVAL, "ovhip_itx_launch_chroma_lmcs: luma plane must be 16-byte aligned with stride % 8 == 0", hipSuccess);
    return itx_launch(ctx, dst, d_cmds, n_large, n_small, d_coefs, d_lmcs_scales, d_bwd_lut);
}

extern "C" int ovhip_itx_launch_ex_(ovhip_ctx *ctx, const ovhip_pic *dst, const ovhip_pic *res, const ovhip_tb_cmd *d_cmds,
                                    uint32_t n_large, uint32_t n_small, const uint32_t tiny3[4], const int16_t *d_coefs,
                                    const int16_t *d_lmcs_scales, const uint16_t *d_bwd_lut)
{
    if (!ctx || !dst) return OVHIP_EINVAL;
    OV_DEVICE(ctx);
    if (!n_large && !n_small && !d_bwd_lut) return OVHIP_OK;
    if ((n_large || n_small) && (!d_cmds || !d_coefs)) return ov_fail(ctx, OVHIP_EINVAL, "ovhip_itx_launch_ex_: null buffer", hipSuccess);
    if (d_bwd_lut && ((dst->stride_y & 7) || ((uintptr_t)dst->y & 15)))
        return ov_fail(ctx, OVHIP_EINVAL, "ovhip_itx_launch_ex_: luma plane must be 16-byte aligned with stride % 8 == 0", hipSuccess);
    return itx_launch(ctx, dst, d_cmds, n_large, n_small, d_coefs, d_lmcs_scales, d_bwd_lut, res, tiny3);
}

extern "C" int ovhip_itx_launch(ovhip_ctx *ctx, const ovhip_pic *dst, const ovhip_tb_cmd *d_cmds,
                                uint32_t n_cmds, const int16_t *d_coefs, const int16_t *d_lmcs_scales)
{
    return ovhip_itx_launch_classes(ctx, dst, d_cmds, n_cmds, 0, d_coefs, d_lmcs_scales);
}
```

### openvvc_amd/csrc/kernels_lmcs.hip

```cpp
#include "ovvc_common.hip.h"
#include "flow_state.hip.h"
#include "lmcs_wnd.hip.h"

namespace {

#ifndef LMCS_ROWS
#define LMCS_ROWS 4
#endif

__global__ __launch_bounds__(64) void k_lmcs_scale(ovhip_pic pic, const ovhip_lmcs_region *__restrict__ regs, uint32_t n,
                                                   LmcsWnd wnd, int16_t *__restrict__ scales, const ovhip_itask *__restrict__ tasks,
                                                   uint32_t n_tasks, FlowState fs, unsigned epoch)
{
    const uint32_t bid = blockIdx.x;
    if (bid >= n) {
        const uint32_t ti = (bid - n) * 4 + (threadIdx.x >> 4);
        if (ti < n_tasks) flow_prepare_task(tasks[ti], fs, epoch, threadIdx.x & 15);
        return;
    }
    const ovhip_lmcs_region g = regs[bid];
    if (g.ordered) return;
    const int lane = threadIdx.x;
    const uint16_t *src = pic.y + (size_t)g.y * pic.stride_y + g.x;
    const int na = 4 * g.n_abv, nl = 4 * g.n_lft;
    const long oa = g.n_abv ? (long)min(lane, na - 1) - pic.stride_y : 0;
    const long ol = g.n_lft ? (long)min(lane, nl - 1) * pic.stride_y - 1 : 0;
    const int va = src[oa], vl = src[ol];
    int sum = (g.n_abv ? va : 0) + (g.n_lft ? vl : 0);
#pragma unroll
    for (int m = 32; m; m >>= 1) sum += __shfl_xor(sum, m);
    if (lane == 0) scales[bid] = (int16_t)lmcs_scale_of_sum(wnd, sum, g.n_abv, g.n_lft);
}

typedef uint32_t lm_u2 __attribute__((ext_vector_type(2), aligned(4)));

#define UNTAG_TASKS_PER_WG 4
__device__ __forceinline__ void untag_chroma_tasks(const ovhip_pic &pic, const ovhip_itask *__restrict__ tasks, uint32_t n, uint32_t wg)
{
    const uint32_t ti = wg * UNTAG_TASKS_PER_WG + (threadIdx.x >> 6);
    if (ti >= n) return;
    const ovhip_itask t = tasks[ti];
    if (t.kind == OVHIP_IT_REGION || t.kind == OVHIP_IT_LUMA || t.kind == OVHIP_IT_IBC_L) return;
    const int lane = threadIdx.x & 63;
    const int l2w = t.log2_w, w = 1 << l2w, npx = w << t.log2_h, stride = pic.stride_c;
    const bool res_only = t.kind == OVHIP_IT_RES_C;
    const bool on0 = !res_only || (t.flags & OVHIP_IF_RES_CB), on1 = !res_only || (t.flags & OVHIP_IF_RES_CR);
    uint16_t *const d0 = pic.cb + t.y * stride + t.x, *const d1 = pic.cr + t.y * stride + t.x;
    if (w >= 4) {
        for (int base = 0; base < npx; base += 1024) {
            lm_u2 v0[4], v1[4];
#pragma unroll
            for (int k = 0; k < 4; ++k) {
                const int p = base + 4 * lane + 256 * k;
                const int o = (p >> l2w) * stride + (p & (w - 1));
                if (p < npx && on0) v0[k] = *reinterpret_cast<const lm_u2 *>(d0 + o);
                if (p < npx && on1) v1[k] = *reinterpret_cast<const lm_u2 *>(d1 + o);
            }
#pragma unroll
            for (int k = 0; k < 4; ++k) {
                const int p = base + 4 * lane + 256 * k;
                const int o = (p >> l2w) * stride + (p & (w - 1));
                if (p < npx && on0) { lm_u2 v = v0[k]; v[0] &= 0x03ff03ffu; v[1] &= 0x03ff03ffu; *reinterpret_cast<lm_u2 *>(d0 + o) = v; }
                if (p < npx && on1) { lm_u2 v = v1[k]; v[0] &= 0x03ff03ffu; v[1] &= 0x03ff03ffu; *reinterpret_cast<lm_u2 *>(d1 + o) = v; }
            }
        }
    } else if (w == 2) {
        for (int p = 2 * lane; p < npx; p += 128) {
            const int o = (p >> l2w) * stride + (p & (w - 1));
            uint32_t a = 0, b = 0;
            if (on0) a = *reinterpret_cast<const uint32_t *>(d0 + o);
            if (on1) b = *reinterpret_cast<const uint32_t *>(d1 + o);
            if (on0) *reinterpret_cast<uint32_t *>(d0 + o) = a & 0x03ff03ffu;
            if (on1) *reinterpret_cast<uint32_t *>(d1 + o) = b & 0x03ff03ffu;
        }
    } else {
        for (int p = lane; p < npx; p += 64) {
            const int o = (p >> l2w) * stride + (p & (w - 1));
            if (on0) d0[o] = d0[o] & 0x3ff;
            if (on1) d1[o] = d1[o] & 0x3ff;
        }
    }
}

__global__ __launch_bounds__(256) void k_lmcs_inverse(ovhip_pic pic, const uint16_t *__restrict__ lut, uint32_t rows_y,
                                                      const ovhip_itask *__restrict__ tasks, uint32_t n_tasks)
{
    const uint32_t untag_y = gridDim.y - rows_y;
    if (blockIdx.y < untag_y) { untag_chroma_tasks(pic, tasks, n_tasks, blockIdx.y * gridDim.x + blockIdx.x); return; }
    const uint32_t by = blockIdx.y - untag_y;

    __shared__ uint16_t s_lut[1024];
    const int nvx = pic.w >> 3;
    const int tail = pic.w & 7;
    const int y00 = (int)by * LMCS_ROWS, v00 = blockIdx.x * 256 + threadIdx.x;
    uint4 q0[LMCS_ROWS];
    const bool first = y00 < pic.h && v00 < nvx;
    if (first) {
#pragma unroll
        for (int r = 0; r < LMCS_ROWS; ++r) q0[r] = *reinterpret_cast<const uint4 *>(pic.y + (size_t)min(y00 + r, pic.h - 1) * pic.stride_y + 8 * v00);
    }
    for (int i = threadIdx.x; i < 512; i += 256) reinterpret_cast<uint32_t *>(s_lut)[i] = reinterpret_cast<const uint32_t *>(lut)[i];
    __syncthreads();
    for (int y0 = y00; y0 < pic.h; y0 += rows_y * LMCS_ROWS) {
        for (int v = v00; v < nvx; v += gridDim.x * 256) {
            uint4 q[LMCS_ROWS];
            if (y0 == y00 && v == v00) {
#pragma unroll
                for (int r = 0; r < LMCS_ROWS; ++r) q[r] = q0[r];
            } else {
#pragma unroll
                for (int r = 0; r < LMCS_ROWS; ++r) q[r] = *reinterpret_cast<const uint4 *>(pic.y + (size_t)min(y0 + r, pic.h - 1) * pic.stride_y + 8 * v);
            }
#pragma unroll
            for (int r = 0; r < LMCS_ROWS; ++r) {
                if (y0 + r >= pic.h) break;
                uint32_t *d = reinterpret_cast<uint32_t *>(&q[r]);
#pragma unroll
                for (int k = 0; k < 4; ++k) d[k] = s_lut[d[k] & 1023] | ((uint32_t)s_lut[(d[k] >> 16) & 1023] << 16);
                *reinterpret_cast<uint4 *>(pic.y + (size_t)(y0 + r) * pic.stride_y + 8 * v) = q[r];
            }
        }
        if (tail && blockIdx.x == 0 && threadIdx.x < tail)
            for (int r = 0; r < LMCS_ROWS && y0 + r < pic.h; ++r) {
                uint16_t *row = pic.y + (size_t)(y0 + r) * pic.stride_y;
                row[8 * nvx + threadIdx.x] = s_lut[row[8 * nvx + threadIdx.x] & 1023];
            }
    }
}

}

static int lmcs_scale_launch(ovhip_ctx *ctx, const ovhip_pic *pic, const ovhip_lmcs_region *d_regions, uint32_t n_regions, const ovhip_lmcs_luts *luts,
                             int16_t *d_scales, const ovhip_itask *d_tasks, uint32_t n_tasks, uint32_t *d_state, uint32_t epoch)
{
    if (!ctx || !pic || !luts) return OVHIP_EINVAL;
    OV_DEVICE(ctx);
    if (!n_regions && !n_tasks) return OVHIP_OK;
    if (n_regions && (!d_regions || !d_scales)) return ov_fail(ctx, OVHIP_EINVAL, "ovhip_lmcs_scale_launch: null buffer", hipSuccess);
    if (n_tasks && (!d_tasks || !d_state || !epoch)) return ov_fail(ctx, OVHIP_EINVAL, "ovhip_lmcs_scale_prepare_launch: bad arguments", hipSuccess);
    const LmcsWnd w = lmcs_wnd_of(luts);
    FlowState fs;
    memset(&fs, 0, sizeof(fs));
    if (n_tasks) fs = flow_state_of(d_state, pic->w, pic->h);
    hipLaunchKernelGGL(k_lmcs_scale, dim3(n_regions + (n_tasks + 3) / 4), dim3(64), 0, ctx->stream, *pic, d_regions, n_regions, w, d_scales, d_tasks, n_tasks, fs, epoch);
    OV_LAUNCH_CHECK(ctx, n_tasks ? "k_lmcs_scale (+ flow state words)" : "k_lmcs_scale");
    return OVHIP_OK;
}

extern "C" int ovhip_lmcs_scale_launch(ovhip_ctx *ctx, const ovhip_pic *pic, const ovhip_lmcs_region *d_regions,
                                       uint32_t n_regions, const ovhip_lmcs_luts *luts, int16_t *d_scales)
{
    return lmcs_scale_launch(ctx, pic, d_regions, n_regions, luts, d_scales, nullptr, 0, nullptr, 0);
}

extern "C" int ovhip_lmcs_scale_prepare_launch(ovhip_ctx *ctx, const ovhip_pic *pic, const ovhip_lmcs_region *d_regions, uint32_t n_regions,
                                               const ovhip_lmcs_luts *luts, int16_t *d_scales, const ovhip_itask *d_tasks, uint32_t n_tasks,
                                               uint32_t *d_state, uint32_t epoch)
{
    return lmcs_scale_launch(ctx, pic, d_regions, n_regions, luts, d_scales, d_tasks, n_tasks, d_state, epoch);
}

static int lmcs_inverse_launch(ovhip_ctx *ctx, const ovhip_pic *pic, const uint16_t *d_bwd_lut, const ovhip_itask *d_tasks, uint32_t n_tasks, const char *who)
{
    if (!ctx || !pic || !d_bwd_lut) return OVHIP_EINVAL;
    OV_DEVICE(ctx);
    if ((pic->stride_y & 7) || ((uintptr_t)pic->y & 15))
        return ov_fail(ctx, OVHIP_EINVAL, "ovhip_lmcs_inverse_launch: luma plane must be 16-byte aligned with stride % 8 == 0", hipSuccess);
    const int nvx = pic->w >> 3;
    const int row_groups = (pic->h + LMCS_ROWS - 1) / LMCS_ROWS;
    const uint32_t gx = (nvx + 255) / 256 > 0 ? (nvx + 255) / 256 : 1, rows_y = row_groups < 4096 ? row_groups : 4096;
    const uint32_t untag_wgs = d_tasks ? (n_tasks + UNTAG_TASKS_PER_WG - 1) / UNTAG_TASKS_PER_WG : 0;
    hipLaunchKernelGGL(k_lmcs_inverse, dim3(gx, rows_y + (untag_wgs + gx - 1) / gx), dim3(256), 0, ctx->stream, *pic, d_bwd_lut, rows_y, d_tasks, d_tasks ? n_tasks : 0u);
    OV_LAUNCH_CHECK(ctx, who);
    return OVHIP_OK;
}

extern "C" int ovhip_lmcs_inverse_launch(ovhip_ctx *ctx, const ovhip_pic *pic, const uint16_t *d_bwd_lut)
{
    return lmcs_inverse_launch(ctx, pic, d_bwd_lut, nullptr, 0, "k_lmcs_inverse");
}

extern "C" int ovhip_lmcs_inverse_untag_launch(ovhip_ctx *ctx, const ovhip_pic *pic, const uint16_t *d_bwd_lut, const ovhip_itask *d_tasks, uint32_t n_tasks)
{
    if (n_tasks && !d_tasks) return OVHIP_EINVAL;
// ... 3 lines not shown
```

### openvvc_amd/csrc/lmcs_wnd.hip.h

```cpp
#pragma once
#include "ovvc_common.hip.h"

struct LmcsWnd { uint16_t bnd[17]; int min_idx, max_idx, crs_offset; };

static inline LmcsWnd lmcs_wnd_of(const ovhip_lmcs_luts *luts)
{
    LmcsWnd wnd;
    memset(&wnd, 0, sizeof(wnd));
    if (luts) { memcpy(wnd.bnd, luts->wnd_bnd, sizeof(wnd.bnd)); wnd.min_idx = luts->min_idx; wnd.max_idx = luts->max_idx; wnd.crs_offset = luts->crs_offset; }
    return wnd;
}

__device__ __forceinline__ int lmcs_scale_of_sum(const LmcsWnd &wnd, int sum, bool has_abv, bool has_lft)
{
    const int nb_units = (has_abv ? 16 : 0) + (has_lft ? 16 : 0);
    int log2_nb = 0;
    for (int v = nb_units; v; v >>= 1) ++log2_nb;
    const int avg = log2_nb ? (sum + (1 << log2_nb)) >> (log2_nb + 1) : 512;
    int idx = wnd.min_idx;
    for (; idx < wnd.max_idx; ++idx)
        if (avg < wnd.bnd[idx + 1]) break;
    idx = min(idx, 15);
    const int wnd_sz = (int)wnd.bnd[idx + 1] - (int)wnd.bnd[idx];
    return wnd_sz == 0 ? 1 << 11 : (1 << (OV_BD - 4 + 11)) / (wnd_sz + wnd.crs_offset);
}
```

### openvvc_amd/csrc/ovvc_picture.hip

```cpp
#include "ovvc_job.hip.h"

extern "C" int ovhip_dmvr_search_launch(ovhip_ctx *ctx, const ovhip_pic *geom, const ovhip_pic *refs, uint32_t n_refs,
                                        const ovhip_mc_unit *d_units, uint32_t n_units, int32_t *d_mv_out);

namespace {

static const ovhip_pic *same_size_refs(const ovhip_pic *geom, const ovhip_pic *refs, uint32_t n_refs, ovhip_pic *out)
{
    if (!refs || n_refs > 16) return refs;
    bool any = false;
    for (uint32_t i = 0; i < n_refs; ++i) {
        const bool same = refs[i].w == geom->w && refs[i].h == geom->h && refs[i].stride_y == geom->stride_y && refs[i].stride_c == geom->stride_c;
        out[i] = same ? refs[i] : *geom;
        any |= !same;
    }
    return any ? out : refs;
}

__global__ __launch_bounds__(256) void k_store_host(uint4 *__restrict__ dst, const uint4 *__restrict__ src, size_t n)
{
    const size_t i = (size_t)blockIdx.x * 256 + threadIdx.x;
    if (i < n) dst[i] = src[i];
}

int store_host(ovhip_ctx *ctx, void *dst_host, const void *src_dev, size_t bytes)
{
    const size_t n = (bytes + 15) / 16;
    if (!n) return OVHIP_OK;
    hipLaunchKernelGGL(k_store_host, dim3((unsigned)((n + 255) / 256)), dim3(256), 0, ctx->stream, (uint4 *)dst_host, (const uint4 *)src_dev, n);
    OV_LAUNCH_CHECK(ctx, "k_store_host");
    return OVHIP_OK;
}

double host_now_us()
{
    timespec t;
    clock_gettime(CLOCK_MONOTONIC, &t);
    return 1e6 * (double)t.tv_sec + 1e-3 * (double)t.tv_nsec;
}

int grow_trace() { static int on = -1; if (on < 0) on = getenv("OVVC_HIP_GROW_TRACE") != nullptr; return on; }

int h2d(ovhip_job *j, hipStream_t st, int k, const void *host, size_t bytes)
{
    if (!bytes) return OVHIP_OK;
    if (j->resident) return j->dev[k].cap >= bytes ? OVHIP_OK : ov_fail(j->ctx, OVHIP_EINVAL, "resident flush before a full one", hipSuccess);
    int r = dev_reserve(j, k, bytes);
    if (r) return r;
    OV_HIP(j->ctx, hipMemcpyAsync(j->dev[k].p, host, bytes, hipMemcpyHostToDevice, st));
    j->st.h2d_bytes += bytes; j->st.n_h2d++;
    return OVHIP_OK;
}

extern "C" const ovhip_tb_cmd *ovhip_rec_tb_cmds_split_tiny_(ovhip_recorder *r, size_t counts[4], size_t tiny[4][4], size_t *n);
extern "C" int ovhip_itx_launch_ex_(ovhip_ctx *ctx, const ovhip_pic *dst, const ovhip_pic *res, const ovhip_tb_cmd *d_cmds, uint32_t n_large,
                                    uint32_t n_small, const uint32_t tiny3[4], const int16_t *d_coefs, const int16_t *d_lmcs_scales, const uint16_t *d_bwd_lut);

extern "C" int ovhip_sao_launch_rows(ovhip_ctx *ctx, const ovhip_pic *dst, const ovhip_pic *src, const ovhip_sao_ctu *d_params, int32_t log2_ctu_s, int32_t row0, int32_t row1);
extern "C" int ovhip_alf_launch_rows(ovhip_ctx *ctx, const ovhip_pic *dst, const ovhip_pic *src, const ovhip_alf_pic *alf, int32_t row0, int32_t row1);

#ifndef OVHIP_PACK_LIMIT
#define OVHIP_PACK_LIMIT (1 << 20)
#endif

int t_collect(ovhip_job *j, int k)
{
    if (!j->t_pending[k]) return OVHIP_OK;
    float ms = 0.f;
    OV_HIP(j->ctx, hipEventSynchronize(j->t_ev[k][1]));
    OV_HIP(j->ctx, hipEventElapsedTime(&ms, j->t_ev[k][0], j->t_ev[k][1]));
    j->t_sum_ms += ms; j->t_count++;
    j->t_pending[k] = 0;
    return OVHIP_OK;
}

struct StageTimer {
    ovhip_job *j; int k;
    StageTimer(ovhip_job *job, int stage) : j(job), k(-1)
    {
        if (!j || j->t_stage != stage) return;
        k = j->t_next; j->t_next = (j->t_next + 1) % 32;
        if (t_collect(j, k) != OVHIP_OK || hipEventRecord(j->t_ev[k][0], j->ctx->stream) != hipSuccess) k = -1;
    }
    ~StageTimer()
    {
        if (k >= 0 && hipEventRecord(j->t_ev[k][1], j->ctx->stream) == hipSuccess) j->t_pending[k] = 1;
    }
};

int copy_rows(ovhip_ctx *ctx, const ovhip_pic *d, const ovhip_pic *s, int32_t r0, int32_t r1)
{
    uint16_t *dp[3] = { d->y, d->cb, d->cr };
    uint16_t *sp[3] = { s->y, s->cb, s->cr };
    for (int p = 0; p < 3; ++p) {
        const size_t ds = p ? d->stride_c : d->stride_y, ss = p ? s->stride_c : s->stride_y;
        const int32_t a = p ? r0 / 2 : r0, b = p ? r1 / 2 : r1;
        OV_HIP(ctx, hipMemcpy2DAsync(dp[p] + a * ds, ds * 2, sp[p] + a * ss, ss * 2, (size_t)(p ? d->w / 2 : d->w) * 2, b - a,
                                     hipMemcpyDeviceToDevice, ctx->stream));
    }
    return OVHIP_OK;
}

int tmvp_cells(ovhip_job *j, const ovhip_mc_unit *d_units, const int32_t *d_mv, size_t first, size_t n, int log2_ctu)
{
    ovhip_tmvp_cell *d_cells = (ovhip_tmvp_cell *)j->dev[B_TMVP].p + 4 * first;
    CHK(ovhip_tmvp_cells_launch(j->ctx, d_units, (uint32_t)(n - first), d_mv, log2_ctu, (j->w + (1 << log2_ctu) - 1) >> log2_ctu, d_cells));
    CHK(store_host(j->ctx, j->tmvp_host + 4 * first, d_cells, 4 * (n - first) * sizeof(ovhip_tmvp_cell)));
    j->n_tmvp = 4 * n;
    return OVHIP_OK;
}

}

enum { UP_DEVS = 64, UP_MAX = 8 };
static pthread_mutex_t g_up_mtx = PTHREAD_MUTEX_INITIALIZER;
static hipStream_t g_up[UP_DEVS][UP_MAX];
static unsigned g_up_next[UP_DEVS];
static int g_up_n = -1;
static int upload_stream_count();
static hipStream_t upload_stream_for(ovhip_job *j)
{
    const int n = upload_stream_count(), dev = j->ctx->device;
    if (n <= 0 || dev < 0 || dev >= UP_DEVS || j->t_stage >= 0) return nullptr;
    pthread_mutex_lock(&g_up_mtx);
    const unsigned k = g_up_next[dev]++ % (unsigned)n;
    if (!g_up[dev][k] && hipStreamCreateWithFlags(&g_up[dev][k], hipStreamNonBlocking) != hipSuccess) g_up[dev][k] = nullptr;
    hipStream_t st = g_up[dev][k];
    pthread_mutex_unlock(&g_up_mtx);
    return st;
}

static int upload_stream_count()
{
    if (__atomic_load_n(&g_up_n, __ATOMIC_RELAXED) < 0) {
        const char *e = getenv("OVVC_HIP_UPLOAD_STREAMS"); const int n = e ? atoi(e) : 2;
        __atomic_store_n(&g_up_n, n < 0 ? 0 : n > UP_MAX ? UP_MAX : n, __ATOMIC_RELAXED);
    }
    return __atomic_load_n(&g_up_n, __ATOMIC_RELAXED);
}

extern "C" int ovhip_upload_streams_clear_of_(ovhip_ctx *keep_clear)
{
    if (!keep_clear) return OVHIP_EINVAL;
    const int n = upload_stream_count(), dev = keep_clear->device;
    if (n <= 0 || dev < 0 || dev >= UP_DEVS) return 0;
    OV_DEVICE(keep_clear);
    int sharing = 0;
    for (int k = 0; k < n; ++k) {
        pthread_mutex_lock(&g_up_mtx);
        if (!g_up[dev][k] && hipStreamCreateWithFlags(&g_up[dev][k], hipStreamNonBlocking) != hipSuccess) g_up[dev][k] = nullptr;
        hipStream_t st = g_up[dev][k];
        pthread_mutex_unlock(&g_up_mtx);
        if (!st) continue;
        for (int tries = 0; tries < 12; ++tries) {
            ovhip_ctx tmp; memset(&tmp, 0, sizeof(tmp)); tmp.device = dev; tmp.stream = st;
            const int q = ovhip_ctx_shares_queue(keep_clear, &tmp);
            if (q != 1) { st = q == 0 ? st : nullptr; break; }
            hipStream_t fresh = nullptr;
            if (hipStreamCreateWithFlags(&fresh, hipStreamNonBlocking) != hipSuccess) { st = nullptr; break; }
            st = fresh;
            if (tries == 11) st = nullptr;
        }
        if (!st) { ++sharing; continue; }
        pthread_mutex_lock(&g_up_mtx);
        g_up[dev][k] = st;
        pthread_mutex_unlock(&g_up_mtx);
    }
    return sharing;
}

void *pinned_alloc(void *user, size_t bytes)
{
    (void)user;
    void *p = nullptr;
    const double t0 = grow_trace() ? host_now_us() : 0.0;
    const bool ok = hipHostMalloc(&p, bytes ? bytes : 16, hipHostMallocDefault) == hipSuccess;
    if (grow_trace()) fprintf(stderr, "grow: pinned %zu bytes at %.3f ms, took %.3f ms\n", bytes, 1e-3 * t0, 1e-3 * (host_now_us() - t0));
    return ok ? p : nullptr;
}
void pinned_free(void *user, void *p) { (void)user; if (p) (void)hipHostFree(p); }

int dev_reserve(ovhip_job *j, int k, size_t bytes)
{
    DevBuf &b = j->dev[k];
    if (bytes <= b.cap) return OVHIP_OK;
    size_t nc = b.cap ? b.cap : (size_t)1 << 16;
    while (nc < bytes) nc *= 2;
    const double t0 = grow_trace() ? host_now_us() : 0.0;
    if (b.p) OV_HIP(j->ctx, hipFree(b.p));
    b.p = nullptr; b.cap = 0;
    hipError_t e = hipMalloc(&b.p, nc);
    if (grow_trace()) fprintf(stderr, "grow: device buffer %d to %zu bytes at %.3f ms, took %.3f ms\n", k, nc, 1e-3 * t0, 1e-3 * (host_now_us() - t0));
    if (e != hipSuccess) return ov_fail(j->ctx, OVHIP_ENOMEM, "hipMalloc(job buffer)", e);
    b.cap = nc;
    return OVHIP_OK;
}

int pinned_reserve(ovhip_job *j, void **p, size_t *cap, size_t bytes)
{
    if (bytes <= *cap) return OVHIP_OK;
    size_t nc = *cap ? *cap : 4096;
    while (nc < bytes) nc *= 2;
    void *q = pinned_alloc(nullptr, nc);
    if (!q) return ov_fail(j->ctx, OVHIP_ENOMEM, "hipHostMalloc", hipSuccess);
    if (*p) { memcpy(q, *p, *cap); pinned_free(nullptr, *p); }
    *p = q; *cap = nc;
    return OVHIP_OK;
}

int state_words(ovhip_job *j, uint32_t **words, size_t n)
{
    if (*words) return OVHIP_OK;
    OV_HIP(j->ctx, hipMalloc((void **)words, n * sizeof(uint32_t)));
    OV_HIP(j->ctx, hipMemsetAsync(*words, 0, n * sizeof(uint32_t), j->ctx->stream));
    return OVHIP_OK;
}

int ordered_arm(ovhip_job *j, uint32_t **words, size_t n)
{
    CHK(state_words(j, words, n));
    if (!j->abort_host) {
        j->abort_host = (uint32_t *)pinned_alloc(nullptr, 64);
        if (!j->abort_host) return ov_fail(j->ctx, OVHIP_ENOMEM, "pinned abort word", hipSuccess);
        *j->abort_host = 0;
    }
    if (++j->epoch >= 0x7ffffff0u) j->epoch = 1;
    return OVHIP_OK;
}

int flow_widest(const ovhip_itask *sorted, const uint32_t *items, size_t n_items)
{
    size_t widest = 0, run = 0;
    for (size_t q = 0; q < n_items; ++q) {
        run = (q && sorted[flow_item_unpack(items[q]).task].level == sorted[flow_item_unpack(items[q - 1]).task].level) ? run + 1 : 1;
        if (run > widest) widest = run;
    }
    return (int)((2 * widest + 63) & ~(size_t)63);
}


enum { FLOW_DEVS = 64, FLOW_DECAY = 512 };
static int g_flow_shift[FLOW_DEVS], g_flow_clean[FLOW_DEVS];
int flow_shift_of(int device)
{
    const int s = __atomic_load_n(&g_flow_shift[device & (FLOW_DEVS - 1)], __ATOMIC_RELAXED);
    return s < 0 ? 0 : s > 4 ? 4 : s;
}

int flow_worker_count(const ovhip_ctx *ctx, uint32_t asked, const ovhip_itask *sorted, const uint32_t *items, size_t n_items, bool in_band)
{
    const int most = (6 * ctx->num_cus) >> flow_shift_of(ctx->device);
    int n = asked ? (int)asked : flow_widest(sorted, items, n_items);
    if (in_band || !asked) n = n >= most ? most : (n < 64 ? 64 : n);
    if (in_band) return ((n < 64 ? 64 : n) + 63) & ~63;
    return n < 1 ? 1 : n;
}

void flow_launch_abandoned(ovhip_job *j)
{
    const int fd = j->ctx->device & (FLOW_DEVS - 1);
    if (!j->test_abort_seen) {
        if (__atomic_load_n(&g_flow_shift[fd], __ATOMIC_RELAXED) < 4) __atomic_fetch_add(&g_flow_shift[fd], 1, __ATOMIC_RELAXED);
        __atomic_store_n(&g_flow_clean[fd], 0, __ATOMIC_RELAXED);
    }
    j->test_abort_seen = 0;
    j->flow_launched = 0;
}

void flow_launch_clean(ovhip_job *j)
{
    if (!j->flow_launched) return;
    const int fd = j->ctx->device & (FLOW_DEVS - 1);
    j->flow_launched = 0;
    if (__atomic_load_n(&g_flow_shift[fd], __ATOMIC_RELAXED) > 0 && __atomic_add_fetch(&g_flow_clean[fd], 1, __ATOMIC_RELAXED) == FLOW_DECAY) {
        __atomic_store_n(&g_flow_clean[fd], 0, __ATOMIC_RELAXED);
        int cur = __atomic_load_n(&g_flow_shift[fd], __ATOMIC_RELAXED);
        while (cur > 0 && !__atomic_compare_exchange_n(&g_flow_shift[fd], &cur, cur - 1, true, __ATOMIC_RELAXED, __ATOMIC_RELAXED)) {}
    }
}

static int g_band_flow_inflight[FLOW_DEVS];
int band_flow_take(ovhip_ctx *ctx, int want)
{
    const int fd = ctx->device & (FLOW_DEVS - 1), cap = 12 * ctx->num_cus;
    int cur = __atomic_load_n(&g_band_flow_inflight[fd], __ATOMIC_RELAXED);
    for (;;) {
        int give = cap - cur < want ? cap - cur : want;
        give &= ~63;
        if (give < 64) return 0;
        if (__atomic_compare_exchange_n(&g_band_flow_inflight[fd], &cur, cur + give, true, __ATOMIC_RELAXED, __ATOMIC_RELAXED)) return give;
    }
}
void band_flow_give(ovhip_ctx *ctx, int n) { if (n) __atomic_fetch_sub(&g_band_flow_inflight[ctx->device & (FLOW_DEVS - 1)], n, __ATOMIC_RELAXED); }

int band_flow_reclaim(ovhip_ctx *ctx, int *charge, hipEvent_t ev_recon, int wait)
{
    if (!*charge) return 1;
    if (wait) (void)hipEventSynchronize(ev_recon);
    else if (hipEventQuery(ev_recon) != hipSuccess) { (void)hipGetLastError(); return 0; }
    band_flow_give(ctx, *charge);
    *charge = 0;
    return 1;
}

void chain_bind(Chain &c, const Placement &p, const ovhip_band_counts &first, const ovhip_band_counts &n, uint32_t n_rpr, uint32_t n_affr)
{
    c.d_mc = (const ovhip_mc_unit *)p.at[B_MC]; c.n_mc = n.n_mc; c.d_mcx = (const ovhip_mc_unit *)p.at[B_MCX]; c.n_mcx = n.n_mcx;
    c.d_aff = (const ovhip_aff_unit *)p.at[B_AFF]; c.n_aff = n.n_aff; c.d_side = (const int32_t *)p.at[B_SIDE] - first.n_side;
    c.d_rpr = (const ovhip_rpr_unit *)p.at[B_RPR]; c.n_rpr = n_rpr; c.d_affr = (const ovhip_aff_rpr_unit *)p.at[B_AFFR]; c.n_affr = n_affr;
    c.d_tb = (const ovhip_tb_cmd *)p.at[B_TB]; c.d_coef = (const int16_t *)p.at[B_COEF] - first.n_coef;
    c.d_reg = (const ovhip_lmcs_region *)p.at[B_REG] - first.n_reg; c.reg0 = first.n_reg; c.n_reg = n.n_reg;
    c.d_it = (const ovhip_itask *)p.at[B_ITASK]; c.n_it = n.n_itask; c.d_items = (const uint32_t *)p.at[B_IITEM];
}

int chain_predict(const Chain &c, const ovhip_pic *refs_same, const ovhip_pic *refs, uint32_t n_refs, const ovhip_pic *intra, int32_t *d_mv)
{
    ovhip_job *j = c.j;
    {
        StageTimer t_(c.timer, OVHIP_TIME_MC);
        CHK(ovhip_mc_launch(j->ctx, c.dst, refs_same, n_refs, c.d_mc, c.n_mc, c.d_fwd, intra));
        if (c.n_rpr) CHK(ovhip_mc_rpr_launch(j->ctx, c.dst, refs, n_refs, c.d_rpr, c.n_rpr, c.d_fwd, intra));
    }
    j->st.n_launches += (c.n_mc != 0) + (c.n_rpr != 0);
    if (c.n_mcx || c.n_aff) {
        StageTimer t_(c.timer, OVHIP_TIME_MCXA);
        CHK(ovhip_mcxa_launch(j->ctx, c.dst, refs_same, n_refs, c.d_mcx, c.n_mcx, d_mv, c.d_aff, c.n_aff, c.d_side, c.d_fwd));
        j->st.n_launches++;
    }
    if (c.n_affr) {
        StageTimer t_(c.timer, OVHIP_TIME_MCXA);
        CHK(ovhip_mca_rpr_launch(j->ctx, c.dst, refs, n_refs, c.d_affr, c.n_affr, c.d_side, c.d_fwd));
        j->st.n_launches++;
    }
    return OVHIP_OK;
}

int chain_residual(Chain &c, const uint16_t *d_bwd)
{
    ovhip_job *j = c.j;
    ovhip_ctx *ctx = j->ctx;
    const uint32_t t_luma[4] = { (uint32_t)c.tiny[1][0], (uint32_t)c.tiny[1][1], (uint32_t)c.tiny[1][2], (uint32_t)c.tiny[1][3] };
    const uint32_t t_chroma[4] = { (uint32_t)c.tiny[3][0], (uint32_t)c.tiny[3][1], (uint32_t)c.tiny[3][2], (uint32_t)c.tiny[3][3] };
    if (c.cls[0] + c.cls[1]) {
        StageTimer t_(c.timer, OVHIP_TIME_ITX_LUMA);
        CHK(ovhip_itx_launch_ex_(ctx, c.dst, c.res, c.d_tb, (uint32_t)c.cls[0], (uint32_t)c.cls[1], t_luma, c.d_coef, nullptr, nullptr));
        j->st.n_launches++;
    }
    if (c.n_reg) {
        if (!c.luts) return ov_fail(ctx, OVHIP_EINVAL, "chroma-scale regions recorded without LMCS tables", hipSuccess);
        StageTimer t_(c.timer, OVHIP_TIME_LMCS_SCALE);
        if (c.n_items) {
            CHK(ovhip_lmcs_scale_prepare_launch(ctx, c.dst, c.d_reg + c.reg0, c.n_reg, c.luts, c.d_scales + c.reg0, c.d_it, c.n_it, j->d_flow, j->epoch));
            c.prepared = 1;
        } else CHK(ovhip_lmcs_scale_launch(ctx, c.dst, c.d_reg + c.reg0, c.n_reg, c.luts, c.d_scales + c.reg0));
        j->st.n_launches++;
    }
    const ovhip_tb_cmd *d_tbc = c.d_tb + c.cls[0] + c.cls[1];
    StageTimer t_(c.timer, OVHIP_TIME_ITX_CHROMA);
    if (d_bwd && c.cls[3]) {
        CHK(ovhip_itx_launch_ex_(ctx, c.dst, nullptr, d_tbc, (uint32_t)c.cls[2], (uint32_t)c.cls[3], t_chroma, c.d_coef, c.d_scales, d_bwd));
        j->st.n_launches++;
        return OVHIP_OK;
    }
    if (c.cls[2] + c.cls[3]) {
        CHK(ovhip_itx_launch_ex_(ctx, c.dst, c.res, d_tbc, (uint32_t)c.cls[2], (uint32_t)c.cls[3], t_chroma, c.d_coef, c.d_scales, nullptr));
        j->st.n_launches++;
    }
    if (d_bwd) { CHK(ovhip_lmcs_inverse_launch(ctx, c.dst, d_bwd)); j->st.n_launches++; }
    return OVHIP_OK;
}

int chain_ordered(const Chain &c, int n_workers)
{
    ovhip_job *j = c.j;
    if (c.n_items) {
        CHK(ovhip_intra_flow_launch(j->ctx, c.dst, c.res, c.d_it, c.n_it, c.d_items, c.n_items, c.d_reg, c.luts, c.d_scales, c.log2_ctu,
                                    j->d_flow, j->epoch, j->abort_host, (c.prepared ? 0 : 1) | (c.ibc ? OVHIP_FLOW_IBC : 0), n_workers));
        j->st.n_launches += 1 + !c.prepared;
        return OVHIP_OK;
    }
    for (uint32_t l = 0; l < c.n_lv; ++l) {
        const uint32_t a = c.lv_start[l], b = c.lv_start[l + 1];
        if (b > a) {
            CHK(ovhip_intra_level_launch(j->ctx, c.dst, c.res, c.d_it + a, b - a, c.d_reg, c.luts, c.d_scales, c.log2_ctu,
                                         ovhip_intra_level_geom(c.h_it + a, b - a)));
            j->st.n_launches++;
        }
    }
    return OVHIP_OK;
}

int chain_unmap(ovhip_job *j, const ovhip_pic *dst, int32_t row0, int32_t row1, const uint16_t *d_bwd, const ovhip_itask *d_it, uint32_t n_tagged)
{
    if (d_bwd) {
        ovhip_pic view = *dst;
        view.y = dst->y + (size_t)row0 * dst->stride_y; view.h = row1 - row0;
        CHK(ovhip_lmcs_inverse_untag_launch(j->ctx, &view, d_bwd, d_it, n_tagged));
    } else if (n_tagged) CHK(ovhip_intra_flow_untag_launch(j->ctx, dst, d_it, n_tagged, 1));
    else return OVHIP_OK;
    j->st.n_launches++;
    return OVHIP_OK;
}

int chain_deblock(const Chain &c, const ovhip_dbf_edge *d_ev, uint32_t n_ev, const ovhip_dbf_edge *d_eh, uint32_t n_eh, const ovhip_dbf_offsets *offs)
{
    StageTimer t_(c.timer, OVHIP_TIME_DBF);
    CHK(ovhip_dbf_launch_edges_ex(c.j->ctx, c.dst, d_ev, n_ev, d_eh, n_eh, offs));
    c.j->st.n_launches += (n_ev != 0) + (n_eh != 0);
    return OVHIP_OK;
}

int chain_filters(const Chain &c, const ovhip_sao_ctu *d_sao, const ovhip_alf_pic *alf, int32_t s0, int32_t s1, int32_t a0, int32_t a1)
{
    ovhip_job *j = c.j;
    if (s1 > s0) {
        if (d_sao) {
            StageTimer t_(c.timer, OVHIP_TIME_SAO);
            CHK(ovhip_sao_launch_rows(j->ctx, &j->tmp, c.dst, d_sao, c.log2_ctu, s0, s1));
            j->st.n_launches++;
        } else if (alf) CHK(copy_rows(j->ctx, &j->tmp, c.dst, s0, s1));
    }
    if (a1 > a0) {
        if (alf) {
            StageTimer t_(c.timer, OVHIP_TIME_ALF);
            CHK(ovhip_alf_launch_rows(j->ctx, c.dst, &j->tmp, alf, a0, a1));
            j->st.n_launches++;
        } else if (d_sao) CHK(copy_rows(j->ctx, c.dst, &j->tmp, a0, a1));
    }
    return OVHIP_OK;
}

namespace {

struct Gathered {
    Switches sw; size_t n_ctu;
    double t0;
    const ovhip_tb_cmd *tb; size_t cls[4], tiny[4][4];
    const int16_t *coef; const ovhip_mc_unit *mc, *mcx; const ovhip_aff_unit *aff; const int32_t *side; const ovhip_lmcs_region *reg;
    const ovhip_ciip_unit *ciip; const ovhip_rpr_unit *rpr; const ovhip_aff_rpr_unit *affr;
    const ovhip_itask *it; const ovhip_ictu *ictu; const uint32_t *lv_start; uint32_t n_lv;
    const ovhip_dbf_edge *ev, *eh; ovhip_dbf_offsets offs;
    ovhip_band_counts n;
    size_t n_ciip, n_rpr, n_affr, n_ictu;
    size_t n_items;
    bool ibc;
    int by_ctu; bool ordered, flow;
};

int flush_gather(ovhip_job *j, const ovhip_pic *dst, const ovhip_pic *intra, const ovhip_job_params *pr, Gathered &g)
{
    ovhip_ctx *ctx = j->ctx;
    if ((dst->w != j->w || dst->h != j->h)) return ov_fail(ctx, OVHIP_EINVAL, "ovhip_job_flush: picture size differs from the job's", hipSuccess);
    { const int64_t c_ = ovhip_job_dmvr_rows_collect(j); if (c_ < 0) return (int)c_; }
    g = Gathered{};
    g.sw = switches_of(pr);
    const uint32_t stages = g.sw.stages;
    const int log2_ctu = g.sw.log2_ctu;
    if (log2_ctu < 5 || log2_ctu > 7) return ov_fail(ctx, OVHIP_EINVAL, "ovhip_job_flush: log2_ctu_s", hipSuccess);
    g.n_ctu = (size_t)((j->w + (1 << log2_ctu) - 1) >> log2_ctu) * ((j->h + (1 << log2_ctu) - 1) >> log2_ctu);
    memset(&j->st, 0, sizeof(j->st));
    j->st.n_ordered_retries = j->n_retries;
    g.t0 = host_now_us();
    j->resident = (stages & OVHIP_STAGE_RESIDENT) && pr->stages;
    ovhip_recorder *rec = j->rec;

    size_t n_tb = 0, n_coef = 0, n_mc = 0, n_mcx = 0, n_aff = 0, n_side = 0, n_reg = 0, n_ev = 0, n_eh = 0;
    g.tb = ovhip_rec_tb_cmds_split_tiny_(rec, g.cls, g.tiny, &n_tb);
    if (!g.tb && n_tb) return ov_fail(ctx, OVHIP_ENOMEM, "ovhip_rec_tb_cmds_split", hipSuccess);
    g.coef = ovhip_rec_coefs(rec, &n_coef);
    g.mc = ovhip_rec_mc_units(rec, &n_mc);
    g.mcx = ovhip_rec_mcx_units(rec, &n_mcx);
    g.aff = ovhip_rec_aff_units(rec, &n_aff);
    g.side = ovhip_rec_aff_side(rec, &n_side);
    g.reg = ovhip_rec_lmcs_regions(rec, &n_reg);
    g.ciip = ovhip_rec_ciip_units(rec, &g.n_ciip);
    if (g.n_ciip && !intra)
        return ov_fail(ctx, OVHIP_EUNSUP, "ovhip_job_flush: CIIP blend units recorded but no picture with their intra prediction", hipSuccess);
    g.rpr = ovhip_rec_rpr_units(rec, &g.n_rpr);
    g.affr = ovhip_rec_aff_rpr_units(rec, &g.n_affr);
    size_t n_it = 0;
    const int want_ctu = pr->stages && (stages & OVHIP_STAGE_INTRA_CTU);
    g.ibc = ovhip_rec_ibc_tasks(rec) != 0;
    g.by_ctu = want_ctu && !g.ibc;
    int by_flow = !want_ctu && !(pr->stages && (stages & OVHIP_STAGE_INTRA_LEVELS));
    if (j->resident && by_flow && !j->flow_on_device) by_flow = 0;
    g.it = !g.by_ctu ? ovhip_rec_itasks_sorted(rec, &n_it, &g.lv_start, &g.n_lv)
                     : ovhip_rec_itasks_by_ctu(rec, log2_ctu, &n_it, &g.ictu, &g.n_ictu);
    if (by_flow && n_it) {
        g.n_items = ovhip_intra_flow_items_(g.it, n_it, j->items_host, j->items_cap / sizeof(uint32_t));
        if (g.n_items > j->items_cap / sizeof(uint32_t)) {
            CHK(pinned_reserve(j, (void **)&j->items_host, &j->items_cap, g.n_items * sizeof(uint32_t)));
            g.n_items = ovhip_intra_flow_items_(g.it, n_it, j->items_host, g.n_items);
        }
    }
    if (!g.it && ovhip_rec_itask_levels(rec)) return ov_fail(ctx, OVHIP_ENOMEM, "ovhip_job_flush: sorting the ordered tasks", hipSuccess);
    if (g.by_ctu) g.n_lv = ovhip_rec_itask_levels(rec);
    if (!(stages & OVHIP_STAGE_INTRA)) { n_it = 0; g.n_lv = 0; g.n_ictu = 0; }
    g.ordered = n_it != 0;
    g.flow = (stages & OVHIP_STAGE_INTRA) && g.n_items;
    if (g.ordered && !j->res.y) CHK(ovhip_pic_alloc(ctx, j->w, j->h, &j->res));
    if (g.ordered && (dst->stride_y != j->res.stride_y || dst->stride_c != j->res.stride_c))
        return ov_fail(ctx, OVHIP_EUNSUP, "ovhip_job_flush: pictures with ordered tasks need tight planes (stride = width)", hipSuccess);
    g.ev = ovhip_rec_dbf_edges(rec, 0, &n_ev, &g.offs);
    g.eh = ovhip_rec_dbf_edges(rec, 1, &n_eh, nullptr);
    g.n = ovhip_band_counts{ (uint32_t)n_tb, (uint32_t)n_coef, (uint32_t)n_mc, (uint32_t)n_mcx, (uint32_t)n_aff, (uint32_t)n_side, (uint32_t)n_reg,
                             (uint32_t)n_it, (uint32_t)n_ev, (uint32_t)n_eh };
    j->st.n_itasks = g.n.n_itask; j->st.n_ilevels = g.n_lv;
    j->st.n_tb = g.n.n_tb; j->st.n_mc = g.n.n_mc; j->st.n_mcx = g.n.n_mcx; j->st.n_aff = g.n.n_aff;
    j->st.n_edges_v = g.n.n_edge_v; j->st.n_edges_h = g.n.n_edge_h; j->st.n_regions = g.n.n_reg;
    if (g.sw.alf_on && alf_tables_missing(pr)) return ov_fail(ctx, OVHIP_EINVAL, "ovhip_job_flush: ALF tables missing", hipSuccess);
    return OVHIP_OK;
}

struct Small { const void *host; size_t bytes; int buf; size_t at; };

int stage_uploads(ovhip_job *j, hipStream_t ust, const Gathered &g, size_t block_bytes, const Small *small, size_t n_small, const void **packed)
{
// ... 286 lines not shown
    if (!j || !n_units) return nullptr;
    *n_units = j->n_mv;
    return j->mv_host;
}

const ovhip_tmvp_cell *ovhip_job_tmvp_cells(ovhip_job *j, size_t *n_entries)
{
    if (!j || !n_entries) return nullptr;
    *n_entries = j->n_tmvp;
    return j->tmvp_host;
}

int ovhip_job_last_stats(const ovhip_job *j, ovhip_job_stats *out)
{
    if (!j || !out) return OVHIP_EINVAL;
    *out = j->st;
    return OVHIP_OK;
}

int ovhip_job_time_stage(ovhip_job *j, int stage)
{
    if (!j || stage < -1 || stage >= OVHIP_TIME_COUNT) return OVHIP_EINVAL;
    OV_DEVICE(j->ctx);
    for (int k = 0; k < 32; ++k) {
        CHK(t_collect(j, k));
        for (int q = 0; q < 2 && stage >= 0; ++q)
            if (!j->t_ev[k][q]) OV_HIP(j->ctx, hipEventCreate(&j->t_ev[k][q]));
    }
    j->t_stage = stage; j->t_sum_ms = 0.0; j->t_count = 0;
    return OVHIP_OK;
}

int ovhip_job_stage_time(ovhip_job *j, double *sum_ms, uint64_t *count)
{
    if (!j || !sum_ms || !count) return OVHIP_EINVAL;
    OV_DEVICE(j->ctx);
    for (int k = 0; k < 32; ++k) CHK(t_collect(j, k));
    *sum_ms = j->t_sum_ms; *count = j->t_count;
    return OVHIP_OK;
}

int64_t ovhip_job_dmvr_rows_collect(ovhip_job *j)
{
    if (!j) return OVHIP_EINVAL;
    if (j->rows_pending) {
        ovhip_ctx *ctx = j->ctx;
        OV_DEVICE(ctx);
        hipError_t e = hipEventSynchronize(j->ev_rows);
        j->rows_pending = 0;
        if (e != hipSuccess) return ov_fail(ctx, OVHIP_ELAUNCH, "hipEventSynchronize(dmvr rows)", e);
        if (j->rows_end > j->n_mv) j->n_mv = j->rows_end;
    }
    return (int64_t)j->rows_end;
}

int64_t ovhip_job_dmvr_rows_begin_upto(ovhip_job *j, const ovhip_pic *refs, uint32_t n_refs, int32_t log2_ctu_s, size_t upto);
int64_t ovhip_job_dmvr_rows_begin(ovhip_job *j, const ovhip_pic *refs, uint32_t n_refs, int32_t log2_ctu_s)
{
    return ovhip_job_dmvr_rows_begin_upto(j, refs, n_refs, log2_ctu_s, (size_t)-1);
}

int64_t ovhip_job_dmvr_rows_begin_upto(ovhip_job *j, const ovhip_pic *refs, uint32_t n_refs, int32_t log2_ctu_s, size_t upto)
{
    if (!j) return OVHIP_EINVAL;
    const int64_t c = ovhip_job_dmvr_rows_collect(j);
    if (c < 0) return c;
    ovhip_ctx *ctx = j->ctx;
    OV_DEVICE(ctx);
    size_t n = 0;
    const ovhip_mc_unit *u = ovhip_rec_mcx_units(j->rec, &n);
    if (n > upto) n = upto;
    const size_t first = j->dmvr_first;
    if (n <= first) return (int64_t)first;
    int any = 0;
    for (size_t i = first; i < n && !any; ++i) any = (u[i].flags & OVHIP_MC_DMVR) != 0;
    if (any) {
        CHK(pinned_reserve(j, (void **)&j->mv_host, &j->mv_cap, n * 16));
        if (log2_ctu_s) CHK(pinned_reserve(j, (void **)&j->tmvp_host, &j->tmvp_cap, 4 * n * sizeof(ovhip_tmvp_cell)));
        if (j->dev[B_MCX].cap < n * sizeof(ovhip_mc_unit) || j->dev[B_MV].cap < n * 16 ||
            (log2_ctu_s && j->dev[B_TMVP].cap < 4 * n * sizeof(ovhip_tmvp_cell))) {
            const size_t ub = (size_t)((j->w + 7) / 8) * ((j->h + 7) / 8);
            CHK(dev_reserve(j, B_MCX, (ub > n ? ub : n) * sizeof(ovhip_mc_unit)));
            CHK(dev_reserve(j, B_MV, (ub > n ? ub : n) * 16));
            if (log2_ctu_s) CHK(dev_reserve(j, B_TMVP, 4 * (ub > n ? ub : n) * sizeof(ovhip_tmvp_cell)));
        }
        char *d_units = (char *)j->dev[B_MCX].p + first * sizeof(ovhip_mc_unit);
        int32_t *d_mv = (int32_t *)j->dev[B_MV].p + 4 * first;
        OV_HIP(ctx, hipMemcpyAsync(d_units, u + first, (n - first) * sizeof(ovhip_mc_unit), hipMemcpyHostToDevice, ctx->stream));
        ovhip_pic geom = j->tmp, same[16];
        CHK(ovhip_dmvr_search_launch(ctx, &geom, same_size_refs(&geom, refs, n_refs, same), n_refs, (const ovhip_mc_unit *)d_units,
                                     (uint32_t)(n - first), d_mv));
        CHK(store_host(ctx, j->mv_host + 4 * first, d_mv, (n - first) * 16));
        if (log2_ctu_s) CHK(tmvp_cells(j, (const ovhip_mc_unit *)d_units, d_mv, first, n, log2_ctu_s));
        OV_HIP(ctx, hipEventRecord(j->ev_rows, ctx->stream));
        j->rows_pending = 1;
    }
    else if (log2_ctu_s) {
        CHK(pinned_reserve(j, (void **)&j->tmvp_host, &j->tmvp_cap, 4 * n * sizeof(ovhip_tmvp_cell)));
        for (size_t i = 4 * first; i < 4 * n; ++i) { j->tmvp_host[i] = ovhip_tmvp_cell{}; j->tmvp_host[i].cell = OVHIP_TMVP_NONE; }
        j->n_tmvp = 4 * n;
    }
    j->dmvr_first = n;
    j->rows_end = n;
    return (int64_t)n;
}

int64_t ovhip_job_dmvr_rows(ovhip_job *j, const ovhip_pic *refs, uint32_t n_refs)
{
    const int64_t n = ovhip_job_dmvr_rows_begin(j, refs, n_refs, 0);
    return n < 0 ? n : ovhip_job_dmvr_rows_collect(j);
}

int ovhip_job_flush(ovhip_job *j, const ovhip_pic *dst, const ovhip_pic *refs, uint32_t n_refs, const ovhip_pic *intra,
                    const ovhip_job_params *pr)
{
    if (!j || !dst || !pr) return OVHIP_EINVAL;
    j->again.valid = 0;
    j->n_retries = 0;
    j->mvf.valid = 0;
    const int r = job_flush_impl(j, dst, refs, n_refs, intra, pr);
    j->mvf.valid = r == OVHIP_OK;
    j->again.valid = r == OVHIP_OK && n_refs <= 16;
    j->again.dst = *dst;
    for (uint32_t i = 0; i < n_refs && i < 16; ++i) j->again.refs[i] = refs[i];
    j->again.n_refs = n_refs;
    j->again.has_intra = intra != nullptr;
    if (intra) j->again.intra = *intra;
    j->again.pr = *pr;
    return r;
}

int ovhip_job_mvfield(ovhip_job *j, const ovhip_mvfield_format *fmt, void *d_vec, size_t vec_bytes, void *d_info, size_t info_bytes)
{
    if (!j) return OVHIP_EINVAL;
    if (band_active(j)) return ov_fail(j->ctx, OVHIP_EUNSUP, "ovhip_job_mvfield: the picture was submitted band-wise (its arrays live in band arenas)", hipSuccess);
    if (!j->mvf.valid) return ov_fail(j->ctx, OVHIP_EINVAL, "ovhip_job_mvfield: no whole-picture flush since ovhip_job_begin", hipSuccess);
    return ovhip_mvfield_launch(j->ctx, j->w, j->h, &j->mvf.src, fmt, d_vec, vec_bytes, d_info, info_bytes);
}

int ovhip_job_mvfield_done_(ovhip_job *j, const ovhip_mvfield_format *fmt, void *d_vec, size_t vec_bytes, void *d_info, size_t info_bytes)
{
    int r = ovhip_job_mvfield(j, fmt, d_vec, vec_bytes, d_info, info_bytes);
    if (r == OVHIP_OK && ov_sync_stream(j->ctx) != hipSuccess) r = ov_fail(j->ctx, OVHIP_ELAUNCH, "motion field output", hipGetLastError());
    return r;
}

int ovhip_job_test_abort_next_flow(ovhip_job *j)
{
    if (!j) return OVHIP_EINVAL;
    j->test_abort = 1;
    return OVHIP_OK;
}

static int job_flush_impl(ovhip_job *j, const ovhip_pic *dst, const ovhip_pic *refs, uint32_t n_refs, const ovhip_pic *intra,
                          const ovhip_job_params *pr)
{
    OV_DEVICE(j->ctx);
    Gathered g;
    Placement p;
    CHK(flush_gather(j, dst, intra, pr, g));
    CHK(flush_stage(j, pr, g, p));
    const double t3 = host_now_us();
    CHK(flush_launch(j, dst, refs, n_refs, intra, pr, g, p));
    j->st.host_us_launch = (uint32_t)(host_now_us() - t3);
    return OVHIP_OK;
}

}
```

### openvvc_amd/engine.py

```python
from __future__ import annotations

import ctypes as C

import numpy as np

from . import capi


class EngineError(RuntimeError):
    pass


def rgb_format(matrix: int = 1, full_range: int = 0, chroma_loc: int = 0, dtype: int = capi.RGB_U8, layout: int = capi.RGB_PLANAR) -> capi.RgbFormat:
    return capi.RgbFormat(matrix, full_range, chroma_loc, dtype, layout)


def rgb_shape(fmt: capi.RgbFormat, w: int, h: int, window=(0, 0, 0, 0)) -> tuple:
    W, H = w - 2 * (window[0] + window[1]), h - 2 * (window[2] + window[3])
    return (3, H, W) if fmt.layout == capi.RGB_PLANAR else (H, W, 3)


def _device_tensor(tensor, what: str, dtypes: tuple, shape: "tuple | None" = None, need: "int | None" = None, slots: bool = False) -> "tuple[int, int, int]":
    import torch
    if not isinstance(tensor, torch.Tensor) or not tensor.is_cuda:
# ... 601 lines not shown
        elif name == "dbf":
            c.dbf_edges(self.dst, self.dbf_v, self.dbf_h, self.wl.dbf_planes["beta_offset"], self.wl.dbf_planes["tc_offset"])
        elif name == "sao":
            c.sao(self.tmp, self.dst, self.sao_params, self.log2_ctu)
        elif name == "alf":
            c.alf(self.dst, self.tmp, self.alf)
        else:
            raise ValueError(name)

    def decode(self, stages=STAGES):
        for s in stages:
            self.run_stage(s)

    def result(self):
        self.ctx.sync()
        return self.dst.download()

    def refined_mvs(self) -> np.ndarray:
        self.ctx.sync()
        return self.mv_out.download(np.int32).reshape(-1, 4) if self.mv_out else np.zeros((0, 4), np.int32)

    def free(self):
        for b in self.bufs + [self.dbf_planes, self.alf]:
            b.free()
        for p in self.refs + [self.dst, self.tmp] + ([self.intra] if self.intra else []):
            p.free()


class Job:

    def __init__(self, ctx: Context, w: int, h: int):
        self.ctx, self.lib, self.w, self.h = ctx, ctx.lib, w, h
        j = C.c_void_p()
        ctx._chk(self.lib.ovhip_job_create(ctx.h, w, h, C.byref(j)), "job_create")
        self.j = j
        self.rec = capi.Recorder.__new__(capi.Recorder)
        self.rec.lib, self.rec.h, self.rec._keep = self.lib, self.lib.ovhip_job_recorder(j), []
        self._keep = {}

    def close(self):
        if self.j:
            self.rec.h = None
            self.lib.ovhip_job_destroy(self.j)
            self.j = None

    def begin(self):
        self.ctx._chk(self.lib.ovhip_job_begin(self.j), "job_begin")

    def load_workload(self, wl):
        self.begin()
        r = self.rec
        for which, arr in ((capi.REC_COEF, wl.coefs), (capi.REC_TB, wl.tb_cmds), (capi.REC_MC, wl.mc_units),
                           (capi.REC_MCX, wl.mcx_units), (capi.REC_AFF, wl.aff_units), (capi.REC_SIDE, wl.aff_side),
                           (capi.REC_REGION, wl.lmcs_regions), (capi.REC_CIIP, wl.ciip_units), (capi.REC_ITASK, wl.itasks),
                           (capi.REC_EDGE_V, wl.dbf_edges[0]), (capi.REC_EDGE_H, wl.dbf_edges[1])):
            if arr is not None and len(arr):
                r.append_raw(which, arr)
        offs = capi.DbfOffsets()
        for i in range(8):
            offs.beta[i], offs.tc[i] = wl.dbf_planes["beta_offset"], wl.dbf_planes["tc_offset"]
        self.ctx._chk(self.lib.ovhip_rec_set_dbf_offsets(r.h, C.byref(offs), 1), "set_dbf_offsets")
        self.params = self.make_params(wl)

    def make_params(self, wl, log2_ctu: int = 7, stages: int = 0) -> "capi.JobParams":
        keep = self._keep
        keep["sao"] = np.ascontiguousarray(wl.sao_params)
        keep["alf"] = {k: np.ascontiguousarray(wl.alf[k], dtype=dt) for k, dt in capi.ALF_TABLES}
        keep["lmcs"] = wl.lmcs
        a = keep["alf"]
        p = capi.JobParams()
        p.lmcs = C.addressof(wl.lmcs) if wl.lmcs is not None else None
        p.sao = keep["sao"].ctypes.data
        p.alf_ctus = a["ctus"].ctypes.data
        p.alf_luma_coeff, p.alf_luma_clip = a["luma_coeff"].ctypes.data, a["luma_clip"].ctypes.data
        p.alf_chroma_coeff, p.alf_chroma_clip = a["chroma_coeff"].ctypes.data, a["chroma_clip"].ctypes.data
        p.alf_cc_coeff = a["cc_coeff"].ctypes.data
        p.log2_ctu_s, p.stages = log2_ctu, stages
        return p

    def flush(self, dst: "DevPic", refs: list, intra: "DevPic | None" = None, params=None):
        arr = (capi.Pic * max(len(refs), 1))(*[r.s for r in refs])
        self.ctx._chk(self.lib.ovhip_job_flush(self.j, C.byref(dst.s), arr, len(refs), C.byref(intra.s) if intra else None,
                                               C.byref(params if params is not None else self.params)), "job_flush")

    def wait(self):
        self.ctx._chk(self.lib.ovhip_job_wait(self.j), "job_wait")

    def band(self, dst: "DevPic", refs: list, row_end: int, last: bool = False, upto: "capi.BandCounts | None" = None, params=None):
        arr = (capi.Pic * max(len(refs), 1))(*[r.s for r in refs])
        self.ctx._chk(self.lib.ovhip_job_band(self.j, C.byref(dst.s), arr, len(refs), C.byref(params if params is not None else self.params),
                                              C.byref(upto) if upto is not None else None, row_end, int(last)), "job_band")

    def band_progress(self) -> int:
        rows = C.c_int32()
        self.ctx._chk(self.lib.ovhip_job_band_progress(self.j, C.byref(rows), None, None), "job_band_progress")
        return rows.value

    def flush_in_bands(self, wl, dst: "DevPic", refs: list, ctu_rows_per_band: int = 1, log2_ctu: int = 7, params=None):
        rows = list(range(ctu_rows_per_band << log2_ctu, self.h, ctu_rows_per_band << log2_ctu))
        cuts = band_counts(wl, rows, log2_ctu)
        for r, c in zip(rows, cuts):
            self.band(dst, refs, r, False, c, params)
        self.band(dst, refs, self.h, True, None, params)

    def bind(self, ctx: "Context"):
        self.ctx._chk(self.lib.ovhip_job_bind(self.j, ctx.h), "job_bind")
        self.ctx = ctx

    def dmvr_rows(self, refs: list) -> int:
        arr = (capi.Pic * max(len(refs), 1))(*[r.s for r in refs])
        n = self.lib.ovhip_job_dmvr_rows(self.j, arr, len(refs))
        if n < 0:
            self.ctx._chk(int(n), "job_dmvr_rows")
        return int(n)

    def dmvr_rows_begin(self, refs: list, log2_ctu: int = 0) -> int:
        arr = (capi.Pic * max(len(refs), 1))(*[r.s for r in refs])
        n = self.lib.ovhip_job_dmvr_rows_begin(self.j, arr, len(refs), log2_ctu)
        if n < 0:
            self.ctx._chk(int(n), "job_dmvr_rows_begin")
        return int(n)

    def dmvr_rows_collect(self) -> int:
        n = self.lib.ovhip_job_dmvr_rows_collect(self.j)
        if n < 0:
            self.ctx._chk(int(n), "job_dmvr_rows_collect")
        return int(n)

    def refined_mvs(self) -> np.ndarray:
        n = C.c_size_t()
        p = self.lib.ovhip_job_refined_mvs(self.j, C.byref(n))
        if not n.value:
            return np.zeros((0, 4), np.int32)
        return np.frombuffer((C.c_int32 * (4 * n.value)).from_address(p), dtype=np.int32).reshape(-1, 4).copy()

    def mvfield(self, fmt: "capi.MvfieldFormat | None", vec=None, info=None, vec_bytes: "int | None" = None, info_bytes: "int | None" = None,
                check: bool = True) -> int:
        vp, vb, ip, ib, _n = _mvfield_dsts(vec, info, fmt, self.w, self.h, vec_bytes, info_bytes) if fmt is not None else (vec or 0, vec_bytes or 0, info or 0, info_bytes or 0, None)
        r = self.lib.ovhip_job_mvfield(self.j, C.byref(fmt) if fmt is not None else None, C.c_void_p(vp) if vp else None, vb, C.c_void_p(ip) if ip else None, ib)
        if check:
            self.ctx._chk(r, "job_mvfield")
        return r

    def tmvp_cells(self) -> np.ndarray:
        n = C.c_size_t()
        p = self.lib.ovhip_job_tmvp_cells(self.j, C.byref(n))
        if not n.value:
            return np.zeros(0, capi.TMVP_CELL_DTYPE)
        return np.ctypeslib.as_array(C.cast(p, C.POINTER(C.c_uint8)), (n.value * capi.TMVP_CELL_DTYPE.itemsize,)).view(capi.TMVP_CELL_DTYPE).copy()

    def test_abort_next_flow(self):
        self.ctx._chk(self.lib.ovhip_job_test_abort_next_flow(self.j), "job_test_abort_next_flow")

    def stats(self) -> "capi.JobStats":
        s = capi.JobStats()
        self.lib.ovhip_job_last_stats(self.j, C.byref(s))
        return s

    def time_stage(self, name: "str | None"):
        self.ctx._chk(self.lib.ovhip_job_time_stage(self.j, capi.TIME_STAGES.index(name) if name else -1), "job_time_stage")

    def stage_time(self):
        s, n = C.c_double(), C.c_uint64()
        self.ctx._chk(self.lib.ovhip_job_stage_time(self.j, C.byref(s), C.byref(n)), "job_stage_time")
        return s.value * 1e-3, n.value


def band_counts(wl, rows, log2_ctu: int = 7) -> list:
    def cut(ctu_row, what):
        ctu_row = np.asarray(ctu_row, np.int64)
        if len(ctu_row) > 1 and (np.diff(ctu_row) < 0).any():
            raise EngineError(f"band_counts: {what} are not in CTU-row order")
        return [int(np.searchsorted(ctu_row, r >> log2_ctu, side="left")) for r in rows]

    def arr(a, dt):
        return np.zeros(0, dt) if a is None or not len(a) else np.asarray(a).view(dt).reshape(-1)

    tb, mc, mcx = arr(wl.tb_cmds, capi.TB_CMD_DTYPE), arr(wl.mc_units, capi.MC_UNIT_DTYPE), arr(wl.mcx_units, capi.MC_UNIT_DTYPE)
    aff, reg, it = arr(wl.aff_units, capi.AFF_UNIT_DTYPE), arr(wl.lmcs_regions, capi.LMCS_REGION_DTYPE), arr(wl.itasks, capi.ITASK_DTYPE)
    ev, eh = arr(wl.dbf_edges[0], capi.DBF_EDGE_DTYPE), arr(wl.dbf_edges[1], capi.DBF_EDGE_DTYPE)
    n_coef = 0 if wl.coefs is None else len(wl.coefs)
    n_side = 0 if wl.aff_side is None else len(wl.aff_side)
    tb_row = (tb["y"].astype(np.int64) << (tb["plane"] != 0)) >> log2_ctu
    it_chroma = (it["kind"] == capi.IT_CHROMA) | (it["kind"] == capi.IT_RES_C)
    it_row = (it["y"].astype(np.int64) << it_chroma) >> log2_ctu
    k_tb, k_mc, k_mcx = cut(tb_row, "transform blocks"), cut(mc["y"] >> log2_ctu, "MC units"), cut(mcx["y"] >> log2_ctu, "refined units")
    k_aff, k_reg, k_it = cut(aff["y"] >> log2_ctu, "affine units"), cut(reg["y"] >> log2_ctu, "regions"), cut(it_row, "ordered tasks")
    k_ev = cut((ev["uy"].astype(np.int64) << 2) >> log2_ctu, "vertical edges")
    k_eh = cut((eh["uy"].astype(np.int64) << 2) >> log2_ctu, "horizontal edges")
    out = []
    for i in range(len(rows)):
        c = capi.BandCounts()
        c.n_tb, c.n_mc, c.n_mcx, c.n_aff, c.n_reg, c.n_itask, c.n_edge_v, c.n_edge_h = k_tb[i], k_mc[i], k_mcx[i], k_aff[i], k_reg[i], k_it[i], k_ev[i], k_eh[i]
        later = tb["coef_off"][k_tb[i]:]
        c.n_coef = int(later.min()) if len(later) else n_coef
        la = aff[k_aff[i]:]
        c.n_side = int(min(la["side_off"].min(), la["prof_off"][(la["flags"] & 1) != 0].min(initial=0xffffffff))) if len(la) else n_side
        out.append(c)
    return out


class Dpb:

    def __init__(self, devices=(0,), ops: "capi.DpbOps | None" = None, n_devices: int | None = None):
        self.lib = capi.load()
        h = C.c_void_p()
        if ops is not None:
            self._ops = ops
            r = self.lib.ovhip_dpb_create_ex(C.byref(h), n_devices or 1, C.byref(ops))
        else:
            arr = (C.c_int * len(devices))(*devices)
            r = self.lib.ovhip_dpb_create(C.byref(h), arr, len(devices))
        if r != 0:
            raise EngineError(f"ovhip_dpb_create: {r} (no HIP device? the DPB has no CPU back-end outside the tests' own)")
        self.h = h

    def close(self):
        if self.h:
            self.lib.ovhip_dpb_destroy(self.h)
            self.h = None

    def stats(self) -> "capi.DpbStats":
        st = capi.DpbStats()
        self.lib.ovhip_dpb_get_stats(self.h, C.byref(st))
        return st

    def begin(self, key: int, dev: int, w: int, h: int, tag: int = 0) -> "capi.Pic":
        pic = capi.Pic()
        r = self.lib.ovhip_dpb_begin_tag(self.h, C.c_void_p(key), tag, dev, w, h, C.byref(pic))
        if r != 0:
            raise EngineError(f"ovhip_dpb_begin: {r}")
        return pic

    def lookup(self, key: int) -> "tuple[int, capi.Pic]":
        pic, dev = capi.Pic(), C.c_int()
        r = self.lib.ovhip_dpb_lookup(self.h, C.c_void_p(key), C.byref(dev), C.byref(pic))
        if r != 0:
            raise EngineError(f"ovhip_dpb_lookup: {r}")
        return dev.value, pic


class Frame:

    def __init__(self, dpb: Dpb, dev: int, w: int, h: int):
        self.lib, self.dpb, self.w, self.h = dpb.lib, dpb, w, h
        f = C.c_void_p()
        r = self.lib.ovhip_frame_create(dpb.h, dev, w, h, C.byref(f))
        if r != 0:
            raise EngineError(f"ovhip_frame_create: {r}")
        self.f = f

    def _chk(self, r, what):
        if r < 0:
            raise EngineError(f"{what}: {r}: {self.lib.ovhip_frame_last_error(self.f).decode()}")
        return r

    def close(self):
        if self.f:
            self.lib.ovhip_frame_destroy(self.f)
            self.f = None

    def begin(self, key: int, tag: int = 0):
        self._chk(self.lib.ovhip_frame_begin_tag(self.f, C.c_void_p(key), tag), "frame_begin")

    def ref(self, key: int, tag: int = 0) -> int:
        return self._chk(self.lib.ovhip_frame_ref_tag(self.f, C.c_void_p(key), tag), "frame_ref")

    def ref_at(self, slot: int, key: int) -> int:
        return self._chk(self.lib.ovhip_frame_ref_at(self.f, slot, C.c_void_p(key)), "frame_ref_at")

    def recorder(self) -> "capi.Recorder":
        r = capi.Recorder.__new__(capi.Recorder)
        r.lib, r.h, r._keep = self.lib, self.lib.ovhip_frame_recorder(self.f), []
        if not r.h:
            raise EngineError("ovhip_frame_recorder")
        r.close = lambda: None
        return r

    def dmvr_rows(self) -> int:
        return int(self._chk(self.lib.ovhip_frame_dmvr_rows(self.f), "frame_dmvr_rows"))

    def dmvr_rows_begin(self, log2_ctu: int = 7) -> int:
        return int(self._chk(self.lib.ovhip_frame_dmvr_rows_begin(self.f, log2_ctu), "frame_dmvr_rows_begin"))

    def dmvr_rows_collect(self) -> int:
        return int(self._chk(self.lib.ovhip_frame_dmvr_rows_collect(self.f), "frame_dmvr_rows_collect"))

    def submit(self, params: "capi.JobParams", job: "Job | None" = None, out: "capi.FrameOutput | None" = None, check: bool = True) -> int:
        r = self.lib.ovhip_frame_submit(self.f, job.j if job is not None else None, None, C.byref(params), C.byref(out) if out is not None else None)
        return self._chk(r, "frame_submit") if check else r

    def fail(self, status: int = -3):
        self.lib.ovhip_frame_fail(self.f, status)

    def set_film_grain(self, params, poc: int = 0, check: bool = True) -> int:
        r = self.lib.ovhip_frame_set_film_grain(self.f, C.byref(params) if params is not None else None, poc)
        if check and r:
            raise EngineError(f"frame_set_film_grain: {r}")
        return r

    def set_picture_hash(self, method: int, n_planes: int = 3, expected: "capi.PicHashValue | None" = None, check: bool = True) -> int:
        r = self.lib.ovhip_frame_set_picture_hash(self.f, method, n_planes, C.byref(expected) if expected is not None else None)
        if check and r:
            raise EngineError(f"frame_set_picture_hash: {r}")
        return r

# ... 180 lines not shown
```

Baseline: 3613.

## Fold LMCS chroma-scale derivation into the chroma inverse-transform launch

The chroma residual scale is now derived inside the chroma ITX kernel instead of in a separate scale-prepare launch. Extra leading workgroups compute region scales and flow-task preparation. Each transform block reloads its neighbour luma and derives the scale itself when its region is unordered. Scale lookup in the window table is unrolled to stay in registers. This removes one kernel launch and its serialization per picture, at the cost of duplicated neighbour loads and reductions in every chroma block, plus higher register pressure. A test hook that reads back the scales is also added.

Result: no change. 3645 (median of 2 runs) (+0.9%).

```diff
diff --git a/include/ovvc_hip.h b/include/ovvc_hip.h
--- a/include/ovvc_hip.h
+++ b/include/ovvc_hip.h
@@ -990,6 +990,7 @@
                                      void *d_info_base, size_t info_bytes_per_picture, uint32_t n_slots);
 const void *ovhip_stream_key(const ovhip_stream *s, uint32_t idx);
 int  ovhip_job_test_abort_next_flow(ovhip_job *job);
+int  ovhip_job_test_scales(ovhip_job *job, int16_t *out, size_t n);
 
 #ifdef __cplusplus
 }
diff --git a/openvvc_amd/capi.py b/openvvc_amd/capi.py
--- a/openvvc_amd/capi.py
+++ b/openvvc_amd/capi.py
@@ -665,6 +665,7 @@
         "ovhip_host_alloc": (vp, [C.c_size_t]),
         "ovhip_host_free": (None, [vp]),
         "ovhip_job_test_abort_next_flow": (C.c_int, [vp]),
+        "ovhip_job_test_scales": (C.c_int, [vp, vp, C.c_size_t]),
         "ovhip_dpb_create": (C.c_int, [P(vp), P(C.c_int), C.c_int]),
         "ovhip_dpb_create_ex": (C.c_int, [P(vp), C.c_int, P(DpbOps)]),
         "ovhip_dpb_destroy": (None, [vp]),
@@ -797,7 +798,7 @@
     "ovhip_job_flush", "ovhip_job_wait", "ovhip_job_refined_mvs", "ovhip_job_dmvr_rows", "ovhip_job_dmvr_rows_begin", "ovhip_job_dmvr_rows_collect", "ovhip_job_last_stats", "ovhip_job_time_stage", "ovhip_job_stage_time",
     "ovhip_output_bytes", "ovhip_output_rows", "ovhip_output_pack_launch", "ovhip_output_row_md5_launch", "ovhip_output_bands", "ovhip_output_tree_md5_launch", "ovhip_pic_output", "ovhip_pic_digest",
     "ovhip_md5_init", "ovhip_md5_update", "ovhip_md5_final", "ovhip_tmvp_cells_launch", "ovhip_job_tmvp_cells", "ovhip_intra_flow_untag_launch", "ovhip_lmcs_inverse_untag_launch", "ovhip_lmcs_scale_prepare_launch",
-    "ovhip_host_alloc", "ovhip_host_free", "ovhip_d2d", "ovhip_job_test_abort_next_flow",
+    "ovhip_host_alloc", "ovhip_host_free", "ovhip_d2d", "ovhip_job_test_abort_next_flow", "ovhip_job_test_scales",
     "ovhip_dpb_create", "ovhip_dpb_create_ex", "ovhip_dpb_destroy", "ovhip_dpb_n_devices", "ovhip_dpb_device", "ovhip_dpb_begin", "ovhip_dpb_want",
     "ovhip_dpb_publish", "ovhip_dpb_acquire", "ovhip_dpb_wait_copy", "ovhip_dpb_poll_tag", "ovhip_frame_refs_ready", "ovhip_dpb_set_unknown_key_timeout", "ovhip_dpb_unpin", "ovhip_dpb_release", "ovhip_dpb_lookup", "ovhip_dpb_shutdown",
     "ovhip_dpb_get_stats", "ovhip_dpb_begin_tag", "ovhip_dpb_want_tag", "ovhip_dpb_acquire_tag", "ovhip_frame_begin_tag", "ovhip_frame_ref_tag", "ovhip_frame_set_trace",
diff --git a/openvvc_amd/csrc/kernels_itx.hip b/openvvc_amd/csrc/kernels_itx.hip
--- a/openvvc_amd/csrc/kernels_itx.hip
+++ b/openvvc_amd/csrc/kernels_itx.hip
@@ -1,4 +1,6 @@
 #include "ovvc_common.hip.h"
+#include "flow_state.hip.h"
+#include "lmcs_wnd.hip.h"
 #include <stdlib.h>
 #define OVT_ATTR __device__
 #include "vvc_tables.h"
@@ -184,6 +186,43 @@
 #define ITX_LDS_BIG   8064
 #define ITX_LDS_SLICE 2048
 
+
+struct ScaleTable { static constexpr bool on = false; };
+struct ScaleInline {
+    static constexpr bool on = true;
+    const ovhip_lmcs_region *regs;
+    LmcsWnd wnd;
+    int16_t *scales; uint32_t reg0, n_reg;
+    const ovhip_itask *tasks; uint32_t n_tasks; FlowState fs; unsigned epoch;
+};
+#define SCALE_WG_REGIONS 4
+#define SCALE_WG_TASKS   16
+
+template <int G> struct BlockScale { LmcsNbr<G> nb; ovhip_lmcs_region g; bool on; };
+template <int G, class SC>
+__device__ __forceinline__ void block_scale_begin(const ovhip_pic &pic, const ovhip_tb_cmd &c, const SC &sc, int lane, BlockScale<G> &b)
+{
+    b = BlockScale<G>{};
+    if constexpr (SC::on) {
+        if ((c.res_mode & (OVHIP_RES_SCALE_IDX | OVHIP_RES_STORE)) == OVHIP_RES_SCALE_IDX) {
+            b.g = sc.regs[c.c_scale];
+            b.on = !b.g.ordered;
+            if (b.on) lmcs_nbr_load<G>(pic, b.g, lane, b.nb);
+        }
+    }
+}
+
+template <int G>
+__device__ __forceinline__ int block_scale_end(const ovhip_tb_cmd &c, const int16_t *__restrict__ lmcs_scales, const ScaleInline &sc,
+                                               const BlockScale<G> &bs, bool all_lanes = false)
+{
+    int derived = 0;
+    if (all_lanes || bs.on) derived = lmcs_nbr_scale<G>(sc.wnd, bs.g, bs.nb);
+    const bool table = (c.res_mode & (OVHIP_RES_SCALE_IDX | OVHIP_RES_STORE)) == OVHIP_RES_SCALE_IDX && !bs.on;
+    return bs.on ? derived : table ? lmcs_scales[c.c_scale] : c.c_scale;
+}
+
+template <class SC>
 __device__ __forceinline__ ResidualSink make_sink(const ovhip_pic &pic, const ResDelta &rd, const ovhip_tb_cmd &c, const int16_t *__restrict__ lmcs_scales)
 {
     ResidualSink sink;
@@ -199,6 +238,8 @@
             sink.dst2 = reinterpret_cast<uint16_t *>(reinterpret_cast<char *>(sink.dst2) + d2);
         }
     }
+    if constexpr (SC::on) sink.scale = 0;
+    else
     sink.scale = (c.res_mode & OVHIP_RES_SCALE_IDX) ? lmcs_scales[c.c_scale] : c.c_scale;
     return sink;
 }
@@ -213,10 +254,12 @@
     } else __syncthreads();
 }
 
-template <int NT, int LW = -1, int LH = -1, bool PLAIN = false>
+template <int NT, int LW = -1, int LH = -1, bool PLAIN = false, class SC = ScaleTable>
 __device__ __forceinline__ void itx_block(const ovhip_pic &pic, const ResDelta &rd, const ovhip_tb_cmd &c, bool valid, const int16_t *__restrict__ arena,
-                                          const int16_t *__restrict__ lmcs_scales, int ablate, int lane, int16_t *lds)
-{
+                                          const int16_t *__restrict__ lmcs_scales, int ablate, int lane, int16_t *lds, const SC &sc)
+{
+    BlockScale<64> bsc;
+    block_scale_begin<64>(pic, c, sc, lane & 63, bsc);
     const int log2_w = LW >= 0 ? LW : c.log2_w, log2_h = LH >= 0 ? LH : c.log2_h;
     const int tb_w = 1 << log2_w, tb_h = 1 << log2_h;
     const int kind = PLAIN ? (int)OVHIP_TB_TR : (c.kind & 0x3f);
@@ -231,7 +274,8 @@
         const int lvl = have ? (int)src[0] : 0;
         const int c0 = (!have || bdpcm) ? lvl : dequant1(lvl, c.dq_scale, c.dq_shift, c.dq_neg);
         const int flat_val = ov_clip16(((((int)(int16_t)c0 + 1) >> 1) + (1 << (14 - OV_BD - 1))) >> (14 - OV_BD));
-        const ResidualSink sink = make_sink(pic, rd, c, lmcs_scales);
+        ResidualSink sink = make_sink<SC>(pic, rd, c, lmcs_scales);
+        if constexpr (SC::on) sink.scale = block_scale_end<64>(c, lmcs_scales, sc, bsc);
         for (int i0 = lane; i0 < tb_w * tb_h; i0 += 4 * NT) {
             int old[4], old2[4];
 #pragma unroll
@@ -332,7 +376,7 @@
     }
     block_sync<NT>();
 
-    const ResidualSink sink = make_sink(pic, rd, c, lmcs_scales);
+    ResidualSink sink = make_sink<SC>(pic, rd, c, lmcs_scales);
 
     if (ablate & 4) valid = false;
     const bool tr = valid && is_tr, lf = !PLAIN && tr && (c.lfnst & 1), bd = valid && !is_tr && bdpcm;
@@ -409,6 +453,7 @@
         }
     }
     block_sync<NT>();
+    if constexpr (SC::on) sink.scale = block_scale_end<64>(c, lmcs_scales, sc, bsc);
     if (tr) {
         const int k2 = min(nb_row, kh);
         tr_pass_lds<true, NT>(s_tmp, ts, s_mh, msh, log2_w, k2, tb_h, 20 - OV_BD, nullptr, 0, lane, sink);
@@ -465,13 +510,16 @@
     return acc;
 }
 
-template <int LW, int LH>
+template <int LW, int LH, class SC>
 __device__ __forceinline__ void itx_tiny(const ovhip_pic &pic, const ResDelta &rd, const ovhip_tb_cmd *__restrict__ cmds, uint32_t i, bool valid,
-                                         const int16_t *__restrict__ arena, const int16_t *__restrict__ lmcs_scales, int16_t *s , int l)
+                                         const int16_t *__restrict__ arena, const int16_t *__restrict__ lmcs_scales, int16_t *s , int l,
+                                         const SC &sc)
 {
     constexpr int W = 1 << LW, H = 1 << LH, N = W * H;
     static_assert(N <= 64 && W <= 8 && H <= 8, "a block is at most one wave: its fences are the wave's (tried with 16-point shapes behind workgroup barriers: slower)");
     const ovhip_tb_cmd c = cmds[valid ? i : 0];
+    BlockScale<N> bsc;
+    block_scale_begin<N>(pic, c, sc, l, bsc);
     const int r = l >> LW, q = l & (W - 1);
     const int bit = (r >> 2) * 8 + (q >> 2);
     const bool sig = (c.sig_sb_map >> bit) & 1;
@@ -488,8 +536,9 @@
     if (c.kind == OVHIP_TB_DC) {
         res = ov_clip16(((((int)s[0] + 1) >> 1) + (1 << (14 - OV_BD - 1))) >> (14 - OV_BD));
     }
+    ResidualSink sink = make_sink<SC>(pic, rd, c, lmcs_scales);
+    if constexpr (SC::on) sink.scale = block_scale_end<N>(c, lmcs_scales, sc, bsc, true);
     if (!valid) return;
-    const ResidualSink sink = make_sink(pic, rd, c, lmcs_scales);
     const int old = sink.dst[r * sink.stride + q];
     const int old2 = sink.dst2 ? (int)sink.dst2[r * sink.stride2 + q] : 0;
     sink.dst[r * sink.stride + q] = (uint16_t)residual1(old, res, sink.mode, sink.scale);
@@ -498,18 +547,38 @@
 
 struct TinyCounts { uint32_t n[4]; };
 
+template <class SC>
 __global__ __launch_bounds__(256) OV_OCC_ITX void k_itx_all(ovhip_pic pic, const ovhip_tb_cmd *__restrict__ cmds, uint32_t n_large,
                                                   uint32_t n_small, const int16_t *__restrict__ arena,
                                                   const int16_t *__restrict__ lmcs_scales, int ablate,
-                                                  const uint16_t *__restrict__ lmcs_inv_lut, uint32_t n_extra, ResDelta rd, TinyCounts tc)
+                                                  const uint16_t *__restrict__ lmcs_inv_lut, uint32_t n_extra, ResDelta rd, TinyCounts tc, SC sc)
 {
     __shared__ __attribute__((aligned(16))) int16_t lds[ITX_LDS_BIG > 4 * ITX_LDS_SLICE ? ITX_LDS_BIG : 4 * ITX_LDS_SLICE];
     const uint32_t n_tiny = tc.n[0] + tc.n[1] + tc.n[2] + tc.n[3];
     const uint32_t gq = (tc.n[0] + 3) >> 2, g0 = (tc.n[1] + 7) >> 3, g1 = (tc.n[2] + 7) >> 3, g2 = (tc.n[3] + 15) >> 4, n_tg = gq + g0 + g1 + g2;
     const uint32_t n_wave = n_small - n_tiny;
-    const uint32_t b = blockIdx.x, n_quads = (n_wave + 3) >> 2;
+    if constexpr (SC::on) {
+        const uint32_t e = blockIdx.x, n_rwg = (sc.n_reg + SCALE_WG_REGIONS - 1) / SCALE_WG_REGIONS;
+        if (e < n_rwg) {
+            const uint32_t ri = e * SCALE_WG_REGIONS + (threadIdx.x >> 6);
+            if (ri >= sc.n_reg) return;
+            const ovhip_lmcs_region g = sc.regs[sc.reg0 + ri];
+            if (g.ordered) return;
+            LmcsNbr<64> nb;
+            lmcs_nbr_load<64>(pic, g, (int)(threadIdx.x & 63), nb);
+            const int scale = lmcs_nbr_scale<64>(sc.wnd, g, nb);
+            if ((threadIdx.x & 63) == 0) sc.scales[sc.reg0 + ri] = (int16_t)scale;
+            return;
+        }
+        if (e < n_extra) {
+            const uint32_t ti = (e - n_rwg) * SCALE_WG_TASKS + (threadIdx.x >> 4);
+            if (ti < sc.n_tasks) flow_prepare_task(sc.tasks[ti], sc.fs, sc.epoch, threadIdx.x & 15);
+            return;
+        }
+    }
+    const uint32_t b = blockIdx.x - (SC::on ? n_extra : 0u), n_quads = (n_wave + 3) >> 2;
     if (b < n_large) {
-        itx_block<256>(pic, rd, cmds[ov_xcd_slot(b, n_large)], true, arena, lmcs_scales, ablate, threadIdx.x, lds);
+        itx_block<256>(pic, rd, cmds[ov_xcd_slot(b, n_large)], true, arena, lmcs_scales, ablate, threadIdx.x, lds, sc);
     } else if (b < n_large + n_quads) {
         const int w = __builtin_amdgcn_readfirstlane(threadIdx.x >> 6);
         const uint32_t i = ov_xcd_slot(b - n_large, n_quads) * 4 + w;
@@ -519,11 +588,11 @@
         const int lane = threadIdx.x & 63;
         const bool plain = valid && !ablate && (c.kind & 0x3f) == OVHIP_TB_TR && !(c.kind & (OVHIP_TB_FLAG_RASTER | OVHIP_TB_FLAG_BDPCM)) && !(c.lfnst & 1);
         const int shape = plain ? (c.log2_w << 3 | c.log2_h) : -1;
-#define ITX_SHAPE(lw, lh) case (lw) << 3 | (lh): itx_block<64, lw, lh, true>(pic, rd, c, true, arena, lmcs_scales, 0, lane, slice); break;
+#define ITX_SHAPE(lw, lh) case (lw) << 3 | (lh): itx_block<64, lw, lh, true>(pic, rd, c, true, arena, lmcs_scales, 0, lane, slice, sc); break;
         switch (shape) {
         ITX_SHAPE(2, 2) ITX_SHAPE(3, 2) ITX_SHAPE(2, 3) ITX_SHAPE(3, 3) ITX_SHAPE(4, 2) ITX_SHAPE(2, 4) ITX_SHAPE(4, 3) ITX_SHAPE(3, 4)
         ITX_SHAPE(4, 4) ITX_SHAPE(5, 2) ITX_SHAPE(2, 5) ITX_SHAPE(5, 3) ITX_SHAPE(3, 5)
-        default: itx_block<64>(pic, rd, c, valid, arena, lmcs_scales, ablate, lane, slice);
+        default: itx_block<64>(pic, rd, c, valid, arena, lmcs_scales, ablate, lane, slice, sc);
         }
 #undef ITX_SHAPE
     } else if (b < n_large + n_quads + n_tg) {
@@ -531,19 +600,19 @@
         const ovhip_tb_cmd *base = cmds + n_large + n_wave;
         if (g < gq) {
             const uint32_t blk = threadIdx.x >> 6, i = ov_xcd_slot(g, gq) * 4 + blk;
-            itx_tiny<3, 3>(pic, rd, base, i, i < tc.n[0], arena, lmcs_scales, lds + 128 * blk, (int)(threadIdx.x & 63));
+            itx_tiny<3, 3>(pic, rd, base, i, i < tc.n[0], arena, lmcs_scales, lds + 128 * blk, (int)(threadIdx.x & 63), sc);
         } else if ((g -= gq) < g0) {
             const uint32_t blk = threadIdx.x >> 5, i = ov_xcd_slot(g, g0) * 8 + blk;
-            itx_tiny<2, 3>(pic, rd, base + tc.n[0], i, i < tc.n[1], arena, lmcs_scales, lds + 64 * blk, (int)(threadIdx.x & 31));
+            itx_tiny<2, 3>(pic, rd, base + tc.n[0], i, i < tc.n[1], arena, lmcs_scales, lds + 64 * blk, (int)(threadIdx.x & 31), sc);
         } else if ((g -= g0) < g1) {
             const uint32_t blk = threadIdx.x >> 5, i = ov_xcd_slot(g, g1) * 8 + blk;
-            itx_tiny<3, 2>(pic, rd, base + tc.n[0] + tc.n[1], i, i < tc.n[2], arena, lmcs_scales, lds + 64 * blk, (int)(threadIdx.x & 31));
+            itx_tiny<3, 2>(pic, rd, base + tc.n[0] + tc.n[1], i, i < tc.n[2], arena, lmcs_scales, lds + 64 * blk, (int)(threadIdx.x & 31), sc);
         } else {
             g -= g1;
             const uint32_t blk = threadIdx.x >> 4, i = ov_xcd_slot(g, g2) * 16 + blk;
-            itx_tiny<2, 2>(pic, rd, base + tc.n[0] + tc.n[1] + tc.n[2], i, i < tc.n[3], arena, lmcs_scales, lds + 32 * blk, (int)(threadIdx.x & 15));
-        }
-    } else {
+            itx_tiny<2, 2>(pic, rd, base + tc.n[0] + tc.n[1] + tc.n[2], i, i < tc.n[3], arena, lmcs_scales, lds + 32 * blk, (int)(threadIdx.x & 15), sc);
+        }
+    } else if constexpr (!SC::on) {
         lmcs_inverse_rows<256>(pic, lmcs_inv_lut, b - n_large - n_quads - n_tg, n_extra, reinterpret_cast<uint16_t *>(lds));
     }
 }
@@ -563,7 +632,7 @@
 
 static int itx_launch(ovhip_ctx *ctx, const ovhip_pic *dst, const ovhip_tb_cmd *d_cmds, uint32_t n_large, uint32_t n_small,
                       const int16_t *d_coefs, const int16_t *d_lmcs_scales, const uint16_t *d_bwd_lut, const ovhip_pic *res = nullptr,
-                      const uint32_t *tiny3 = nullptr)
+                      const uint32_t *tiny3 = nullptr, const ScaleInline *inl = nullptr)
 {
     TinyCounts tc = { { tiny3 ? tiny3[0] : 0u, tiny3 ? tiny3[1] : 0u, tiny3 ? tiny3[2] : 0u, tiny3 ? tiny3[3] : 0u } };
     if ((uint64_t)tc.n[0] + tc.n[1] + tc.n[2] + tc.n[3] > n_small) return ov_fail(ctx, OVHIP_EINVAL, "itx launch: more tiny blocks than small ones", hipSuccess);
@@ -573,13 +642,21 @@
             return ov_fail(ctx, OVHIP_EINVAL, "itx launch: the residual picture must have the picture's geometry", hipSuccess);
         rd.d[0] = (char *)res->y - (char *)dst->y; rd.d[1] = (char *)res->cb - (char *)dst->cb; rd.d[2] = (char *)res->cr - (char *)dst->cr;
     }
-    const uint32_t n_extra = d_bwd_lut ? (uint32_t)(dst->h + 3) / 4 : 0;
+    if (inl && d_bwd_lut) return ov_fail(ctx, OVHIP_EINVAL, "itx launch: inline chroma scales read the luma the inverse mapping rewrites", hipSuccess);
+    const uint32_t n_extra = inl ? (inl->n_reg + SCALE_WG_REGIONS - 1) / SCALE_WG_REGIONS + (inl->n_tasks + SCALE_WG_TASKS - 1) / SCALE_WG_TASKS
+                           : d_bwd_lut ? (uint32_t)(dst->h + 3) / 4 : 0;
     if (itx_ablate()) tc.n[0] = tc.n[1] = tc.n[2] = tc.n[3] = 0;
     const uint32_t n_tiny = tc.n[0] + tc.n[1] + tc.n[2] + tc.n[3];
     const uint32_t grid = n_large + (n_small - n_tiny + 3) / 4 + (tc.n[0] + 3) / 4 + (tc.n[1] + 7) / 8 + (tc.n[2] + 7) / 8 + (tc.n[3] + 15) / 16 + n_extra;
     if (!grid) return OVHIP_OK;
-    hipLaunchKernelGGL(k_itx_all, dim3(grid), dim3(256), 0, ctx->stream, *dst, d_cmds, n_large, n_small, d_coefs,
-                       d_lmcs_scales, itx_ablate(), d_bwd_lut, n_extra, rd, tc);
+    if (inl) {
+        hipLaunchKernelGGL(k_itx_all<ScaleInline>, dim3(grid), dim3(256), 0, ctx->stream, *dst, d_cmds, n_large, n_small, d_coefs,
+                           d_lmcs_scales, itx_ablate(), d_bwd_lut, n_extra, rd, tc, *inl);
+        OV_LAUNCH_CHECK(ctx, "k_itx_all (+ chroma scales)");
+        return OVHIP_OK;
+    }
+    hipLaunchKernelGGL(k_itx_all<ScaleTable>, dim3(grid), dim3(256), 0, ctx->stream, *dst, d_cmds, n_large, n_small, d_coefs,
+                       d_lmcs_scales, itx_ablate(), d_bwd_lut, n_extra, rd, tc, ScaleTable{});
     OV_LAUNCH_CHECK(ctx, "k_itx_all");
     return OVHIP_OK;
 }
@@ -631,6 +708,24 @@
     return itx_launch(ctx, dst, d_cmds, n_large, n_small, d_coefs, d_lmcs_scales, d_bwd_lut, res, tiny3);
 }
 
+extern "C" int ovhip_itx_launch_scale_(ovhip_ctx *ctx, const ovhip_pic *dst, const ovhip_pic *res, const ovhip_tb_cmd *d_cmds,
+                                       uint32_t n_large, uint32_t n_small, const uint32_t tiny3[4], const int16_t *d_coefs,
+                                       const ovhip_lmcs_region *d_regions, uint32_t reg0, uint32_t n_reg, const ovhip_lmcs_luts *luts,
+                                       int16_t *d_scales, const ovhip_itask *d_tasks, uint32_t n_tasks, uint32_t *d_state, uint32_t epoch)
+{
+    if (!ctx || !dst || !luts) return OVHIP_EINVAL;
+    OV_DEVICE(ctx);
+    if (!d_cmds || !d_coefs || !(n_large + n_small) || !d_regions || !d_scales || !n_reg)
+        return ov_fail(ctx, OVHIP_EINVAL, "ovhip_itx_launch_scale_: null buffer", hipSuccess);
+    if (n_tasks && (!d_tasks || !d_state || !epoch)) return ov_fail(ctx, OVHIP_EINVAL, "ovhip_itx_launch_scale_: bad flow arguments", hipSuccess);
+    ScaleInline inl;
+    memset(&inl, 0, sizeof(inl));
+    inl.regs = d_regions; inl.wnd = lmcs_wnd_of(luts); inl.scales = d_scales; inl.reg0 = reg0; inl.n_reg = n_reg;
+    inl.tasks = d_tasks; inl.n_tasks = n_tasks; inl.epoch = epoch;
+    if (n_tasks) inl.fs = flow_state_of(d_state, dst->w, dst->h);
+    return itx_launch(ctx, dst, d_cmds, n_large, n_small, d_coefs, d_scales, nullptr, res, tiny3, &inl);
+}
+
 extern "C" int ovhip_itx_launch(ovhip_ctx *ctx, const ovhip_pic *dst, const ovhip_tb_cmd *d_cmds,
                                 uint32_t n_cmds, const int16_t *d_coefs, const int16_t *d_lmcs_scales)
 {
diff --git a/openvvc_amd/csrc/kernels_lmcs.hip b/openvvc_amd/csrc/kernels_lmcs.hip
--- a/openvvc_amd/csrc/kernels_lmcs.hip
+++ b/openvvc_amd/csrc/kernels_lmcs.hip
@@ -20,16 +20,10 @@
     }
     const ovhip_lmcs_region g = regs[bid];
     if (g.ordered) return;
-    const int lane = threadIdx.x;
-    const uint16_t *src = pic.y + (size_t)g.y * pic.stride_y + g.x;
-    const int na = 4 * g.n_abv, nl = 4 * g.n_lft;
-    const long oa = g.n_abv ? (long)min(lane, na - 1) - pic.stride_y : 0;
-    const long ol = g.n_lft ? (long)min(lane, nl - 1) * pic.stride_y - 1 : 0;
-    const int va = src[oa], vl = src[ol];
-    int sum = (g.n_abv ? va : 0) + (g.n_lft ? vl : 0);
-#pragma unroll
-    for (int m = 32; m; m >>= 1) sum += __shfl_xor(sum, m);
-    if (lane == 0) scales[bid] = (int16_t)lmcs_scale_of_sum(wnd, sum, g.n_abv, g.n_lft);
+    LmcsNbr<64> nb;
+    lmcs_nbr_load<64>(pic, g, (int)threadIdx.x, nb);
+    const int scale = lmcs_nbr_scale<64>(wnd, g, nb);
+    if (threadIdx.x == 0) scales[bid] = (int16_t)scale;
 }
 
 typedef uint32_t lm_u2 __attribute__((ext_vector_type(2), aligned(4)));
diff --git a/openvvc_amd/csrc/lmcs_wnd.hip.h b/openvvc_amd/csrc/lmcs_wnd.hip.h
--- a/openvvc_amd/csrc/lmcs_wnd.hip.h
+++ b/openvvc_amd/csrc/lmcs_wnd.hip.h
@@ -11,6 +11,7 @@
     return wnd;
 }
 
+template <bool IN_REGS = false>
 __device__ __forceinline__ int lmcs_scale_of_sum(const LmcsWnd &wnd, int sum, bool has_abv, bool has_lft)
 {
     const int nb_units = (has_abv ? 16 : 0) + (has_lft ? 16 : 0);
@@ -18,9 +19,50 @@
     for (int v = nb_units; v; v >>= 1) ++log2_nb;
     const int avg = log2_nb ? (sum + (1 << log2_nb)) >> (log2_nb + 1) : 512;
     int idx = wnd.min_idx;
-    for (; idx < wnd.max_idx; ++idx)
-        if (avg < wnd.bnd[idx + 1]) break;
-    idx = min(idx, 15);
-    const int wnd_sz = (int)wnd.bnd[idx + 1] - (int)wnd.bnd[idx];
+    int wnd_sz;
+    if (IN_REGS) {
+#pragma unroll
+        for (int i = 0; i < 16; ++i)
+            if (idx == i && i < wnd.max_idx && !(avg < wnd.bnd[i + 1])) idx = i + 1;
+        idx = min(idx, 15);
+        int lo = wnd.bnd[0], hi = wnd.bnd[1];
+#pragma unroll
+        for (int i = 1; i < 16; ++i)
+            if (idx == i) { lo = wnd.bnd[i]; hi = wnd.bnd[i + 1]; }
+        wnd_sz = hi - lo;
+    } else {
+        for (; idx < wnd.max_idx; ++idx)
+            if (avg < wnd.bnd[idx + 1]) break;
+        idx = min(idx, 15);
+        wnd_sz = (int)wnd.bnd[idx + 1] - (int)wnd.bnd[idx];
+    }
     return wnd_sz == 0 ? 1 << 11 : (1 << (OV_BD - 4 + 11)) / (wnd_sz + wnd.crs_offset);
 }
+
+template <int G> struct LmcsNbr { int abv[64 / G], lft[64 / G]; };
+
+template <int G>
+__device__ __forceinline__ void lmcs_nbr_load(const ovhip_pic &pic, const ovhip_lmcs_region &g, int lane, LmcsNbr<G> &v)
+{
+    const uint16_t *src = pic.y + (size_t)g.y * pic.stride_y + g.x;
+    const int na = 4 * g.n_abv, nl = 4 * g.n_lft;
+#pragma unroll
+    for (int i = 0; i < 64 / G; ++i) {
+        const int k = lane + G * i;
+        const long oa = g.n_abv ? (long)min(k, na - 1) - pic.stride_y : 0;
+        const long ol = g.n_lft ? (long)min(k, nl - 1) * pic.stride_y - 1 : 0;
+        v.abv[i] = src[oa]; v.lft[i] = src[ol];
+    }
+}
+
+template <int G>
+__device__ __forceinline__ int lmcs_nbr_scale(const LmcsWnd &wnd, const ovhip_lmcs_region &g, const LmcsNbr<G> &v)
+{
+    int sum = 0;
+#pragma unroll
+    for (int i = 0; i < 64 / G; ++i) sum += (g.n_abv ? v.abv[i] : 0) + (g.n_lft ? v.lft[i] : 0);
+#pragma unroll
+    for (int m = G / 2; m; m >>= 1) sum += __shfl_xor(sum, m);
+    if (G == 64) sum = __builtin_amdgcn_readfirstlane(sum);
+    return lmcs_scale_of_sum<true>(wnd, sum, g.n_abv, g.n_lft);
+}
diff --git a/openvvc_amd/csrc/ovvc_picture.hip b/openvvc_amd/csrc/ovvc_picture.hip
--- a/openvvc_amd/csrc/ovvc_picture.hip
+++ b/openvvc_amd/csrc/ovvc_picture.hip
@@ -55,6 +55,10 @@
 extern "C" const ovhip_tb_cmd *ovhip_rec_tb_cmds_split_tiny_(ovhip_recorder *r, size_t counts[4], size_t tiny[4][4], size_t *n);
 extern "C" int ovhip_itx_launch_ex_(ovhip_ctx *ctx, const ovhip_pic *dst, const ovhip_pic *res, const ovhip_tb_cmd *d_cmds, uint32_t n_large,
                                     uint32_t n_small, const uint32_t tiny3[4], const int16_t *d_coefs, const int16_t *d_lmcs_scales, const uint16_t *d_bwd_lut);
+extern "C" int ovhip_itx_launch_scale_(ovhip_ctx *ctx, const ovhip_pic *dst, const ovhip_pic *res, const ovhip_tb_cmd *d_cmds, uint32_t n_large,
+                                       uint32_t n_small, const uint32_t tiny3[4], const int16_t *d_coefs, const ovhip_lmcs_region *d_regions,
+                                       uint32_t reg0, uint32_t n_reg, const ovhip_lmcs_luts *luts, int16_t *d_scales, const ovhip_itask *d_tasks,
+                                       uint32_t n_tasks, uint32_t *d_state, uint32_t epoch);
 
 extern "C" int ovhip_sao_launch_rows(ovhip_ctx *ctx, const ovhip_pic *dst, const ovhip_pic *src, const ovhip_sao_ctu *d_params, int32_t log2_ctu_s, int32_t row0, int32_t row1);
 extern "C" int ovhip_alf_launch_rows(ovhip_ctx *ctx, const ovhip_pic *dst, const ovhip_pic *src, const ovhip_alf_pic *alf, int32_t row0, int32_t row1);
@@ -346,8 +350,10 @@
         CHK(ovhip_itx_launch_ex_(ctx, c.dst, c.res, c.d_tb, (uint32_t)c.cls[0], (uint32_t)c.cls[1], t_luma, c.d_coef, nullptr, nullptr));
         j->st.n_launches++;
     }
-    if (c.n_reg) {
-        if (!c.luts) return ov_fail(ctx, OVHIP_EINVAL, "chroma-scale regions recorded without LMCS tables", hipSuccess);
+    const bool unmap_rider = d_bwd && c.cls[3];
+    const bool inline_scales = c.n_reg && (c.cls[2] + c.cls[3]) && !unmap_rider;
+    if (c.n_reg && !c.luts) return ov_fail(ctx, OVHIP_EINVAL, "chroma-scale regions recorded without LMCS tables", hipSuccess);
+    if (c.n_reg && !inline_scales) {
         StageTimer t_(c.timer, OVHIP_TIME_LMCS_SCALE);
         if (c.n_items) {
             CHK(ovhip_lmcs_scale_prepare_launch(ctx, c.dst, c.d_reg + c.reg0, c.n_reg, c.luts, c.d_scales + c.reg0, c.d_it, c.n_it, j->d_flow, j->epoch));
@@ -357,12 +363,17 @@
     }
     const ovhip_tb_cmd *d_tbc = c.d_tb + c.cls[0] + c.cls[1];
     StageTimer t_(c.timer, OVHIP_TIME_ITX_CHROMA);
-    if (d_bwd && c.cls[3]) {
+    if (unmap_rider) {
         CHK(ovhip_itx_launch_ex_(ctx, c.dst, nullptr, d_tbc, (uint32_t)c.cls[2], (uint32_t)c.cls[3], t_chroma, c.d_coef, c.d_scales, d_bwd));
         j->st.n_launches++;
         return OVHIP_OK;
     }
-    if (c.cls[2] + c.cls[3]) {
+    if (inline_scales) {
+        CHK(ovhip_itx_launch_scale_(ctx, c.dst, c.res, d_tbc, (uint32_t)c.cls[2], (uint32_t)c.cls[3], t_chroma, c.d_coef, c.d_reg, c.reg0, c.n_reg,
+                                    c.luts, c.d_scales, c.n_items ? c.d_it : nullptr, c.n_items ? c.n_it : 0u, j->d_flow, j->epoch));
+        if (c.n_items) c.prepared = 1;
+        j->st.n_launches++;
+    } else if (c.cls[2] + c.cls[3]) {
         CHK(ovhip_itx_launch_ex_(ctx, c.dst, c.res, d_tbc, (uint32_t)c.cls[2], (uint32_t)c.cls[3], t_chroma, c.d_coef, c.d_scales, nullptr));
         j->st.n_launches++;
     }
@@ -955,6 +966,15 @@
     return OVHIP_OK;
 }
 
+int ovhip_job_test_scales(ovhip_job *j, int16_t *out, size_t n)
+{
+    if (!j || !out || j->dev[B_SCALE].cap < n * sizeof(int16_t)) return OVHIP_EINVAL;
+    OV_DEVICE(j->ctx);
+    if (ov_sync_stream(j->ctx) != hipSuccess) return ov_fail(j->ctx, OVHIP_ELAUNCH, "ovhip_job_test_scales", hipGetLastError());
+    OV_HIP(j->ctx, hipMemcpy(out, j->dev[B_SCALE].p, n * sizeof(int16_t), hipMemcpyDeviceToHost));
+    return OVHIP_OK;
+}
+
 static int job_flush_impl(ovhip_job *j, const ovhip_pic *dst, const ovhip_pic *refs, uint32_t n_refs, const ovhip_pic *intra,
                           const ovhip_job_params *pr)
 {
diff --git a/openvvc_amd/engine.py b/openvvc_amd/engine.py
--- a/openvvc_amd/engine.py
+++ b/openvvc_amd/engine.py
@@ -777,6 +777,11 @@
     def test_abort_next_flow(self):
         self.ctx._chk(self.lib.ovhip_job_test_abort_next_flow(self.j), "job_test_abort_next_flow")
 
+    def test_scales(self, n: int) -> np.ndarray:
+        out = np.zeros(n, np.int16)
+        self.ctx._chk(self.lib.ovhip_job_test_scales(self.j, out.ctypes.data, n), "job_test_scales")
+        return out
+
     def stats(self) -> "capi.JobStats":
         s = capi.JobStats()
         self.lib.ovhip_job_last_stats(self.j, C.byref(s))
```
